# pollen-robotics/reachy2_symbolic_ik

Hardware: AMD Instinct MI355X
Metric: IK solves/sec (7-DoF r_arm, batched poses) (higher is better)
Workload: dtype f64

## Files before the change

### reachy2_symbolic_ik_amd/csrc/rsik_device.hpp

```cpp
#pragma once

#include <hip/hip_runtime.h>
#include <stdint.h>

#include "../../include/rsik.h"
#include "rsik_math.hpp"

namespace rsik {

#ifdef RSIK_HOT_ONLY
#define RSIK_RARE(c) (false)
#else
#define RSIK_RARE(c) (__builtin_expect(!!(c), 0))
#endif


#ifdef RSIK_ISA_MARKS
#define RSIK_MARK(name) asm volatile("; RSIK_MARK " name)
#else
#define RSIK_MARK(name)
#endif

constexpr double kPi = 3.141592653589793;
constexpr double kTwoPi = 2 * kPi;

struct ArmC {
    double v[RSIK_ARM_CONSTS_COUNT];
};

struct V3 {
    double x, y, z;
};
__device__ __forceinline__ V3 operator+(V3 a, V3 b) { return {a.x + b.x, a.y + b.y, a.z + b.z}; }
__device__ __forceinline__ V3 operator-(V3 a, V3 b) { return {a.x - b.x, a.y - b.y, a.z - b.z}; }
__device__ __forceinline__ V3 operator*(V3 a, double s) { return {a.x * s, a.y * s, a.z * s}; }
__device__ __forceinline__ double dot(V3 a, V3 b) { return fma(a.x, b.x, fma(a.y, b.y, a.z * b.z)); }
__device__ __forceinline__ V3 cross(V3 a, V3 b) {
    return {fma(a.y, b.z, -(a.z * b.y)), fma(a.z, b.x, -(a.x * b.z)), fma(a.x, b.y, -(a.y * b.x))};
}
__device__ __forceinline__ V3 madd(V3 a, double s, V3 b) { return {fma(a.x, s, b.x), fma(a.y, s, b.y), fma(a.z, s, b.z)}; }
__device__ __forceinline__ double dot_d(V3 a, V3 b) { return a.x * b.x + a.y * b.y + a.z * b.z; }
__device__ __forceinline__ double norm(V3 a) { return sqrt_cr(dot_d(a, a)); }
__device__ __forceinline__ V3 normalized(V3 a, double& len) {
    double rs;
    sqrt_rsqrt(dot(a, a), len, rs);
    return a * rs;
}
__device__ __forceinline__ V3 normalized(V3 a) {
    return a * rsqrt_fast(dot(a, a));
}

__device__ __forceinline__ bool np_isclose(double a, double b) { return fabs(a - b) <= (1e-8 + 1e-5 * fabs(b)); }
template <int N>
__device__ __forceinline__ bool all_finite(const double (&v)[N]) {
    bool ok = true;
#pragma unroll
    for (int k = 0; k < N; k++) ok = ok && (fabs(v[k]) < __builtin_inf());
    return ok;
}

__device__ __forceinline__ double pymod_2pi(double a) {
    double q = floor(a * 0.15915494309189535);
    double m = fma(-q, kTwoPi, a);
    if (RSIK_RARE(!(m >= 0 && m < kTwoPi))) {
        if (m < 0) m += kTwoPi;
        if (m >= kTwoPi) m -= kTwoPi;
    }
    return m;
// ... 180 lines not shown
    return g;
}
template <class Acc>
__device__ __forceinline__ Goal goal_from_euler_tipz(const Acc& A, double roll, double pitch, double yaw) {
    const double ang[3] = {roll, pitch, yaw};
    double sn[3], cs[3];
    fast_sincos_n<3>(ang, sn, cs);
    const double sa = sn[0], ca = cs[0], sb = sn[1], cb = cs[1], sc = sn[2], cc = cs[2];
    const double tz = A(RSIK_C_TIPL + 2);
    Goal g;
    g.woff = {fma(cc * sb, ca, sc * sa) * tz, fma(sc * sb, ca, -(cc * sa)) * tz, (cb * ca) * tz};
    g.toff = {0.0, 0.0, 0.0};
    g.xg = {cc * cb, sc * cb, -sb};
    g.tw = {-g.woff.x, -g.woff.y, -g.woff.z};
    return g;
}
__device__ __forceinline__ V3 wrist_position(const V3& woff, V3 pos) { return woff + pos; }

template <bool V>
struct BoolC {
    __device__ __forceinline__ constexpr operator bool() const { return V; }
};
template <bool KEEP, bool GEOM_ONLY, class NL, class Acc>
__device__ Reach reach_impl(const Acc& A, V3 pos_in, const V3 woff, const NL no_limits_v) {
    const bool NO_LIMITS = no_limits_v;
    Reach r;
    r.ok = false;
    r.i0 = r.i1 = __builtin_nan("");
    const V3 s = cvec(A, RSIK_C_SHOULDER);
    const double u = A(RSIK_C_UPPER_ARM), f = A(RSIK_C_FOREARM);
    const double bl = A(RSIK_C_BACKWARD), pm = A(RSIK_C_PROJ_MARGIN), upf = A(RSIK_C_UPF);

    V3 gp = pos_in;
    V3 dv = gp - s;
    const double ss0 = dot_d(dv, dv);
    int st = RSIK_STATE_REACHABLE;
    if (RSIK_RARE(ss0 > A(RSIK_C_MAX_LEN_SQ))) {
        double nd = sqrt_cr(ss0) + pm;
        gp = madd(dv * fast_rcp(nd), A(RSIK_C_MAX_LEN), s);
        st = RSIK_STATE_POSE_OUT_OF_REACH;
    }
    if (RSIK_RARE(gp.x < bl)) {
        gp.x = bl;
        st = RSIK_STATE_BACKWARD_POSE;
    }
    r.state = st;
    r.stage = 0;
    if (KEEP) { r.pos = gp; r.w = gp; r.c2 = gp; r.n2 = gp; r.a1 = gp; r.a2 = gp; r.r2 = 0.0; r.ct0 = 1.0; r.st0 = 0.0; r.ct1 = 1.0; r.st1 = 0.0; }
    if (!NO_LIMITS && st != RSIK_STATE_REACHABLE) return r;
    r.stage = 1;

    RSIK_MARK("reach_wrist");
    V3 w = wrist_position(woff, gp);
    if (RSIK_RARE(w.x < bl)) {
        double diff = bl - w.x;
        gp.x = gp.x + diff;
        if (NO_LIMITS) w = wrist_position(woff, gp);
        else w.x = w.x + diff;
    }
    V3 P = w - s;
    double dsw, inv_d;
    sqrt_rsqrt(dot_d(P, P), dsw, inv_d);
    double d = dsw;
    V3 self_pos = gp;
    if (NO_LIMITS) {
        if (RSIK_RARE(dsw > upf)) {
            double nd = fabs(dsw) + pm;
            V3 nw = madd((w - s) * fast_rcp(nd), upf, s);
            self_pos = gp + (nw - w);
            w = nw;
            P = w - s;
            sqrt_rsqrt(dot_d(P, P), d, inv_d);
        }
    } else {
        if (RSIK_RARE(dsw > upf)) {
            r.state = RSIK_STATE_WRIST_OUT_OF_RANGE;
            if (KEEP) { r.pos = gp; r.w = w; }
            return r;
        }
    }
    if (RSIK_RARE(dsw < A(RSIK_C_MIN_DIST))) {
        const double t = fabs(dsw) + pm;
        const double k = A(RSIK_C_MIN_DIST) * fast_rcp(t);
        const double km1 = k - 1.0;
        gp = madd(P, km1, gp);
        w = madd(P, km1, w);
        self_pos = gp;
        P = P * k;
        d = dsw * k;
        inv_d = inv_d * (t * A(RSIK_C_INV_MIN_DIST));
    }

    RSIK_MARK("reach_circle");
    if (RSIK_RARE(d > upf)) {
        r.state = RSIK_STATE_SHOULD_NOT_HAPPEN;
        if (KEEP) { r.pos = self_pos; r.w = w; }
        return r;
    }
    r.pos = self_pos;
    r.w = w;
    V3 n2 = P * inv_d;
    double r2, ir2;
    double kk;
    double fh;
    V3 c2;
    {
        double d2 = d * d, k = d2 - f * f + u * u;
        double rad = 4 * d2 * (u * u) - k * k;
        const double m = d + P.x;
        const double g = rad * (m * m);
        double irad, srad;
        if (RSIK_RARE(!(g > 0.0))) {
            irad = (rad != 0.0) ? rsqrt_fast(rad) : 0.0;
            srad = rad * irad;
            fh = fast_rcp(1.0 + n2.x);
        } else {
            const double z = rsqrt_fast(g);
            irad = z * m;
            srad = rad * irad;
            fh = d * (z * srad);
        }
        const double hid = 0.5 * inv_d;
        r2 = hid * srad;
        ir2 = (d + d) * irad;
        kk = k * hid;
        c2 = s + n2 * kk;
    }
    RSIK_MARK("reach_frame");
    Frame F2 = frame_from_unit(n2, fh);
    r.c2 = c2; r.r2 = r2; r.n2 = n2; r.a1 = F2.c1; r.a2 = F2.c2;
    r.stage = 2;
    if (NO_LIMITS || GEOM_ONLY) {
        r.ok = true; r.state = RSIK_STATE_REACHABLE; r.i0 = -kPi; r.i1 = kPi;
        r.ct0 = -1.0; r.st0 = -1.2246467991473532e-16;
// ... 130 lines not shown
    const bool inside = fma(r2, fma(cm, fa1, sm * fa2), side_val) > 0;
    const bool first = inside != (ang2 < ang1);
    r.i0 = first ? ang1 : ang2;
    r.i1 = first ? ang2 : ang1;
    r.ct0 = first ? ly1 : ly2;
    r.st0 = first ? lz1 : lz2;
    r.ct1 = first ? ly2 : ly1;
    r.st1 = first ? lz2 : lz1;
    return r;
}

template <bool NO_LIMITS, bool KEEP = true, class Acc>
__device__ __forceinline__ Reach reach_g(const Acc& A, V3 pos_in, const V3 woff) {
    return reach_impl<KEEP, false>(A, pos_in, woff, BoolC<NO_LIMITS>{});
}

template <bool NO_LIMITS, bool KEEP = true, class Acc>
__device__ __forceinline__ Reach reach(const Acc& A, V3 pos_in, const Rot& Rg) {
    return reach_g<NO_LIMITS, KEEP>(A, pos_in, make_goal(A, Rg).woff);
}

__device__ __forceinline__ V3 elbow_on_circle(const Reach& r, double ct, double st) {
    double y = r.r2 * ct, z = r.r2 * st;
    return madd(r.a1, y, madd(r.a2, z, r.c2));
}

template <bool EXACT = true, class Acc>
__device__ __forceinline__ bool above_singularity_plane(const Acc& A, V3 e) {
    if constexpr (EXACT) return e.z > (e.x - A(RSIK_C_ES)) * A(RSIK_C_SING_COEFF) + A(RSIK_C_ES + 2) - A(RSIK_C_SING_OFFSET);
    else return e.z > fma(e.x, A(RSIK_C_SING_COEFF), A(RSIK_C_PLANE_K));
}
template <bool PLANE = true, class Acc>
__device__ __forceinline__ bool is_elbow_ok(const Acc& A, V3 e) {
    bool ok = e.y * A(RSIK_C_SIDE) < -0.2;
    if constexpr (PLANE) ok = ok && (e.z < (e.x - A(RSIK_C_ES)) * A(RSIK_C_SING_COEFF) + A(RSIK_C_ES + 2) - A(RSIK_C_SING_OFFSET));
    return ok;
}

struct JointsOut {
    double j[7];
    V3 elbow;
    bool projected;
    bool sing;
    double c4, s4, c5, s5, c6, s6;
};

typedef const __attribute__((address_space(1))) double* GConst;
template <bool FRESH, bool TIPZ = false, class Acc, class Prev = const double*>
__device__ JointsOut joints_from_theta_g(const Acc& A, Reach& r, const Goal& G, double ct, double st, Prev prev) {
    RSIK_MARK("joints_elbow");
    JointsOut o;
    V3 e = elbow_on_circle(r, ct, st);
    o.projected = false;
    if (RSIK_RARE(above_singularity_plane<!FRESH>(A, e))) {
        const V3 v3 = cvec(A, RSIK_C_PLANE_N), pc = cvec(A, RSIK_C_PROJ_CENTER);
        const V3 d1 = e - pc;
        const V3 V = madd(v3, -dot(d1, v3), d1);
        const V3 ne = madd(V, A(RSIK_C_PROJ_RADIUS) * rsqrt_fast(dot(V, V)), pc);
        const V3 shift = ne - e;
        e = ne;
        if constexpr (FRESH) {
            r.w = r.w + shift;
        } else {
            r.pos = r.pos + shift;
            r.w = wrist_position(G.woff, r.pos);
        }
        o.projected = true;
    }
    RSIK_MARK("joints_shoulder");
    o.elbow = e;
    const double u = A(RSIK_C_UPPER_ARM), f = A(RSIK_C_FOREARM);
    auto to_shoulder = [&](V3 p) -> V3 {
        return {fma(A(RSIK_C_MST + 0), p.x, fma(A(RSIK_C_MST + 1), p.y, fma(A(RSIK_C_MST + 2), p.z, A(RSIK_C_TSH + 0)))),
                fma(A(RSIK_C_MST + 3), p.x, fma(A(RSIK_C_MST + 4), p.y, fma(A(RSIK_C_MST + 5), p.z, A(RSIK_C_TSH + 1)))),
                fma(A(RSIK_C_MST + 6), p.x, fma(A(RSIK_C_MST + 7), p.y, fma(A(RSIK_C_MST + 8), p.z, A(RSIK_C_TSH + 2))))};
    };
    V3 q = to_shoulder(e);
    double cphi, sphi, rho;
    const bool sing_sp = RSIK_RARE(q.x == 0 && q.z == 0);
    if (sing_sp) {
        double s_, c_;
        fast_sincos(prev[0], &s_, &c_);
        cphi = c_; sphi = -s_; rho = 0.0;
    } else {
        const double rho2 = fma(q.x, q.x, q.z * q.z);
        const double irho = rsqrt_fast(rho2);
        rho = rho2 * irho;
        cphi = q.x * irho; sphi = q.z * irho;
    }
    const double iL = A(RSIK_C_INV_U);
    double cr = rho * iL, srs = q.y * iL;
    V3 g0 = {cr * cphi, srs, cr * sphi};
    V3 g1 = {-srs * cphi, cr, -srs * sphi};
    V3 g2 = {-sphi, 0.0, cphi};
    auto rot_g = [&](V3 a) -> V3 { return {dot(g0, a), dot(g1, a), fma(g2.x, a.x, g2.z * a.z)}; };
    auto to_elbow = [&](V3 p) -> V3 {
        V3 a = rot_g(to_shoulder(p));
        a.x -= u;
        return a;
    };
    RSIK_MARK("joints_elbow_angles");
    V3 pw = to_elbow(r.w);
    double sigma, ca, sa;
    const bool sing_ey = RSIK_RARE(pw.y == 0 && pw.z == 0);
    if (sing_ey) {
        fast_sincos(prev[2], &sa, &ca);
        sigma = 0.0;
// ... 482 lines not shown
```

### reachy2_symbolic_ik_amd/csrc/rsik_kernel_continuous.hpp

```cpp
#pragma once

namespace rsik {

struct ContinuousArgs {
    int64_t n;
    const double* in[12];
    const double* cur_pose[12];
    const uint8_t* arm;
    const uint8_t* timed_out;
    int euler_roundtrip;
    int first_timed_out;
    double pref_arg[2];
    double pref_self[2];
    double pref_self_cs[2], pref_self_sn[2];
    double lim[2][2];
    double d_theta_max;
    const double* current_joints;
    double max_angle, cos_max, sin_max;
    double* st;
    double* joints;
    uint8_t* reachable;
    uint8_t* state;
    unsigned* started_word;
    unsigned started_seq;
// ... 21 lines not shown
    return disc;
}

struct ThetaTarget {
    bool ok_limits;
    bool found;
    double theta;
    int code;
};
template <bool PLANE, bool FALLBACK_GEOMETRY = true, class Acc>
__device__ __forceinline__ ThetaTarget continuous_target(const Acc& A, V3 pos, const V3 woff, double pref_self, double pref_cs,
                                                         double pref_sn, Reach& r) {
    ThetaTarget T;
    r = reach_g<false, false>(A, pos, woff);
    T.ok_limits = r.ok;
    T.found = false;
    T.theta = 0.0;
    T.code = RSIK_STATE_EMPTY;
    if (r.ok) {
        T.found = best_discrete_theta_lane<PLANE>(A, r, 10, pref_self, pref_cs, pref_sn, T.theta);
        if (!T.found) T.code = RSIK_STATE_LIMITED_BY_SHOULDER;
    } else {
        T.code = r.state;
        if constexpr (FALLBACK_GEOMETRY) r = reach_g<true>(A, pos, woff);
    }
    return T;
}
__device__ __forceinline__ double continuous_next_theta_goal(double goal, double prev_theta, double d_theta_max, double l0,
                                                            double l1, double dmax_v, double l1v) {
    const double ad = angle_diff_straight(goal, prev_theta);
    const double theta = (fabs(ad) < d_theta_max) ? goal : (prev_theta + copysign(dmax_v, ad));
    return limit_theta_to_interval_straight(theta, l0, l1, l1v);
}
__device__ __forceinline__ double continuous_next_theta_goal(double goal, double prev_theta, double d_theta_max, double l0,
                                                            double l1) {
    return continuous_next_theta_goal(goal, prev_theta, d_theta_max, l0, l1, d_theta_max, l1);
}
__device__ __forceinline__ double continuous_next_theta(bool ok_limits, bool found, double target, double pref_arg,
                                                        double prev_theta, double d_theta_max, double l0, double l1) {
    const double goal = ok_limits ? (found ? target : prev_theta) : pref_arg;
    return continuous_next_theta_goal(goal, prev_theta, d_theta_max, l0, l1);
}
template <bool MIXED, bool PLANE>
__global__ __launch_bounds__(kBlock) void control_continuous_kernel(const ContinuousArgs K) {
    __shared__ double lds_out[kBlock / 64][64 * 7];
    const int lane = threadIdx.x & 63;
    const int wave = threadIdx.x >> 6;
    const int64_t i = (int64_t)blockIdx.x * kBlock + threadIdx.x;
    const int64_t wave_base = (int64_t)blockIdx.x * kBlock + wave * 64;
    const bool live = i < K.n;
    const int64_t ii = live ? i : (K.n - 1);
    const int64_t n = K.n;

    __shared__ SharedTables lds_tab;
        stage_tables<MIXED, (int)offsetof(ContinuousArgs, arms) + (MIXED ? 0 : (int)sizeof(ArmC))>(lds_tab, K.arms);
    const Acc<MIXED> A = make_acc<MIXED>(K.arms, MIXED ? (K.arm[ii] != 0) : false, lds_tab);
    const int slot = MIXED ? (A.isl ? 1 : 0) : 0;

    double prev_theta = K.st[0 * n + ii];
    double prev_sol[7];
#pragma unroll
    for (int k = 0; k < 7; k++) prev_sol[k] = K.st[(1 + k) * n + ii];
    bool init = K.st[8 * n + ii] != 0.0;
    bool emergency = K.st[9 * n + ii] != 0.0;
    bool has_prev = K.st[10 * n + ii] != 0.0;

    double jv[7], rejected[7];
    int st_code = RSIK_STATE_EMPTY;
    int cause = 0;
    bool ok = false;
    if (emergency) {
#pragma unroll
        for (int k = 0; k < 7; k++) jv[k] = prev_sol[k];
        st_code = RSIK_STATE_EMERGENCY;
    } else {
        Rot Rg;
        V3 pos;
        double m[12];
#pragma unroll
        for (int k = 0; k < 12; k++) m[k] = K.in[k][ii];
        const bool invalid = !all_finite(m);
        goal_from_m12(m, Rg, pos, K.euler_roundtrip);
        if (K.first_timed_out || (K.timed_out && K.timed_out[ii])) { has_prev = false; init = true; }
        if (!has_prev) {
            has_prev = true;
            continuous_reinit(A, K, ii, K.pref_arg[slot], prev_theta, prev_sol);
        }
        const Goal G = make_goal(A, Rg);
        Reach r;
        const ThetaTarget T = continuous_target<PLANE>(A, pos, G.woff, K.pref_self[slot], K.pref_self_cs[slot], K.pref_self_sn[slot], r);
        if (RSIK_RARE(invalid)) {
#pragma unroll
            for (int k = 0; k < 7; k++) jv[k] = __builtin_nan("");
            st_code = RSIK_STATE_INVALID_INPUT;
            prev_theta = continuous_next_theta(true, false, 0.0, K.pref_arg[slot], prev_theta, K.d_theta_max, K.lim[slot][0], K.lim[slot][1]);
        } else if (RSIK_RARE(!T.ok_limits && !r.ok)) {
#pragma unroll
            for (int k = 0; k < 7; k++) jv[k] = __builtin_nan("");
            st_code = RSIK_STATE_NOT_REACHABLE_NO_LIMITS;
        } else {
        ok = T.ok_limits && T.found;
        st_code = T.code;
        const double theta = continuous_next_theta(T.ok_limits, T.found, T.theta, K.pref_arg[slot], prev_theta, K.d_theta_max,
                                                   K.lim[slot][0], K.lim[slot][1]);
        prev_theta = theta;
        double sn, cs;
        fast_sincos(theta, &sn, &cs);
        JointsOut o = joints_from_theta_g<true>(A, r, G, cs, sn, prev_sol);
#pragma unroll
        for (int k = 0; k < 7; k++) jv[k] = o.j[k];
        cause = safety_checks(A.utab, jv, o.c4, o.s4, o.c5, o.s5, o.c6, o.s6, prev_sol, K.max_angle, K.cos_max, K.sin_max);
        emergency = cause != 0;
        if (!init && joints_discontinuous(jv, prev_sol)) {
            cause |= RSIK_EMERGENCY_CONTINUITY;
            emergency = true;
#pragma unroll
            for (int k = 0; k < 7; k++) { rejected[k] = jv[k]; jv[k] = prev_sol[k]; }
        }
        init = false;
        if (!emergency) {
#pragma unroll
            for (int k = 0; k < 7; k++) prev_sol[k] = jv[k];
        }
        }
    }
    store_rows<7>(K.joints, wave_base, K.n, lane, lds_out[wave], jv);
    if (live) {
        if (K.reachable) K.reachable[i] = ok ? 1 : 0;
        if (K.state) K.state[i] = (uint8_t)st_code;
        K.st[0 * n + i] = prev_theta;
#pragma unroll
        for (int k = 0; k < 7; k++) K.st[(1 + k) * n + i] = prev_sol[k];
        K.st[8 * n + i] = init ? 1.0 : 0.0;
        K.st[9 * n + i] = emergency ? 1.0 : 0.0;
        K.st[10 * n + i] = has_prev ? 1.0 : 0.0;
        if (cause != 0) {
            K.st[11 * n + i] = (double)cause;
            if (cause & RSIK_EMERGENCY_CONTINUITY) {
#pragma unroll
                for (int k = 0; k < 7; k++) K.st[(12 + k) * n + i] = rejected[k];
            }
        }
    }
}

template <bool MIXED, bool PAIR>
__global__ __launch_bounds__(kBlock) void cont_init_kernel(const ContinuousArgs K) {
    __builtin_amdgcn_s_setprio(3);
    if (K.started_word != nullptr && blockIdx.x == gridDim.x - 1 && threadIdx.x == 0)
        __hip_atomic_store(K.started_word, K.started_seq, __ATOMIC_RELAXED, __HIP_MEMORY_SCOPE_SYSTEM);
    const int64_t gid = (int64_t)blockIdx.x * kBlock + threadIdx.x;
    const int64_t i = PAIR ? (gid >> 1) : gid;
    const int half = PAIR ? (int)(gid & 1) : 0;
    const bool live = i < K.n;
    const int64_t ii = live ? i : (K.n - 1);
    __shared__ SharedTables lds_tab;
        stage_tables<MIXED, (int)offsetof(ContinuousArgs, arms) + (MIXED ? 0 : (int)sizeof(ArmC))>(lds_tab, K.arms);
    const Acc<MIXED> A = make_acc<MIXED>(K.arms, MIXED ? (K.arm[ii] != 0) : false, lds_tab);
    const int slot = MIXED ? (A.isl ? 1 : 0) : 0;
    const int64_t n = K.n;
    if (!live || K.st[9 * n + i] != 0.0) return;
    const bool timed_out = K.first_timed_out || (K.timed_out && K.timed_out[i]);
    if (!timed_out && K.st[10 * n + i] != 0.0) return;
    double prev_theta = K.st[0 * n + i];
    double prev_sol[7];
#pragma unroll
    for (int k = 0; k < 7; k++) prev_sol[k] = K.st[(1 + k) * n + i];
    continuous_reinit<PAIR>(A, K, i, K.pref_arg[slot], prev_theta, prev_sol, half);
    if (half != 0) return;
    K.st[0 * n + i] = prev_theta;
#pragma unroll
    for (int k = 0; k < 7; k++) K.st[(1 + k) * n + i] = prev_sol[k];
    K.st[8 * n + i] = 1.0;
    K.st[10 * n + i] = 1.0;
}

}
```

### reachy2_symbolic_ik_amd/csrc/rsik_kernel_discrete.hpp

```cpp
#pragma once

namespace rsik {

struct DiscreteArgs {
    int64_t n;
    const double* in[12];
    const uint8_t* arm;
    int nb;
    int log2p;
    int sweep_mode;
    int euler_roundtrip;
    int stagger;
    double pref[2];
    double pref_cs[2], pref_sn[2];
    double lim[2][2];
    union {
        double prev_sol[2][7];
        const double* prev_rows;
    };
    double prev_cs[2][3], prev_sn[2][3];
    const double* current_joints;
    double max_angle, cos_max, sin_max;
    double* joints;
    uint8_t* reachable;
// ... 64 lines not shown
            double od = __shfl_xor(best_d, off);
            int ok = __shfl_xor(best_k, off);
            if (od < best_d || (od == best_d && ok < best_k)) { best_d = od; best_k = ok; }
        }
        if (p >= 0 && k0 == 0) {
            double th = __builtin_nan("");
            if (best_k != 0x7fffffff) th = (best_k == K.nb - 1) ? gb : ((double)best_k * gstep + ga);
            res[p] = th;
        }
    }
}

#ifndef RSIK_DISC_ATTR
#define RSIK_DISC_ATTR
#endif
#ifndef RSIK_DISC_MIN_WAVES
#define RSIK_DISC_MIN_WAVES 3
#endif
#define RSIK_DISC_PRIO(p) do { if (K.stagger) __builtin_amdgcn_s_setprio(p); } while (0)
#ifndef RSIK_DISC_BLOCK
#define RSIK_DISC_BLOCK 256
#endif
constexpr int kDiscBlock = RSIK_DISC_BLOCK;
struct PrevRowRegs { double v[7]; };
struct NoPrevRow {};
__device__ __forceinline__ const double* safety_prev(const PrevRowRegs& p, const double*) { return p.v; }
__device__ __forceinline__ const double* safety_prev(const NoPrevRow&, const double* uniform) { return uniform; }
template <bool MIXED, bool PLANE, bool PREV_ROWS = false>
__global__ __launch_bounds__(kDiscBlock, RSIK_DISC_MIN_WAVES) RSIK_DISC_ATTR void control_discrete_kernel(const DiscreteArgs K) {
    __shared__ double lds_slab[kDiscBlock / 64][kDiscRows][64];
    const int lane = threadIdx.x & 63;
    const int wave = threadIdx.x >> 6;
    const int64_t i = (int64_t)blockIdx.x * kDiscBlock + threadIdx.x;
    const int64_t wave_base = (int64_t)blockIdx.x * kDiscBlock + wave * 64;
    const bool live = i < K.n;
    const int64_t ii = live ? i : (K.n - 1);

#ifdef RSIK_TIMELINE_PROBE
    uint64_t probe_t[7];
    probe_t[0] = __builtin_amdgcn_s_memrealtime();
#define RSIK_DISC_PROBE(k) do { __builtin_amdgcn_sched_barrier(0); probe_t[k] = __builtin_amdgcn_s_memrealtime(); __builtin_amdgcn_sched_barrier(0); } while (0)
#else
#define RSIK_DISC_PROBE(k) do { } while (0)
#endif
    double m12[12];
#pragma unroll
    for (int k = 0; k < 12; k++) m12[k] = K.in[k][ii];
    const bool lane_isl = MIXED ? (K.arm[ii] != 0) : false;
    [[maybe_unused]] std::conditional_t<PREV_ROWS, PrevRowRegs, NoPrevRow> prow;
    if constexpr (PREV_ROWS) {
#pragma unroll
        for (int k = 0; k < 7; k++) prow.v[k] = K.prev_rows[ii * 7 + k];
    }
        __shared__ SharedTables lds_tab;
    stage_tables<MIXED, (int)offsetof(DiscreteArgs, arms) + (MIXED ? 0 : (int)sizeof(ArmC)), kDiscBlock>(lds_tab, K.arms);
#ifdef RSIK_TIMELINE_PROBE
    asm volatile("s_waitcnt vmcnt(0)" ::: "memory");
#endif
    RSIK_DISC_PROBE(1);
    const Acc<MIXED> A = make_acc<MIXED>(K.arms, lane_isl, lds_tab);
    const int slot = MIXED ? (A.isl ? 1 : 0) : 0;

    const bool invalid = !all_finite(m12);
    Rot Rg;
    V3 pos;
    goal_from_m12(m12, Rg, pos, K.euler_roundtrip);

    Goal G = make_goal(A, Rg);
    {
        const double pk[6] = {G.tw.x, G.tw.y, G.tw.z, G.xg.x, G.xg.y, G.xg.z};
#pragma unroll
        for (int k = 0; k < 6; k++) lds_slab[wave][k][lane] = pk[k];
    }
    RSIK_MARK("disc_reach");
    RSIK_DISC_PRIO(3);
    Reach r = reach_g<false, false>(A, pos, G.woff);
    if (RSIK_RARE(invalid)) { r.ok = false; r.state = RSIK_STATE_INVALID_INPUT; }
    RSIK_MARK("disc_shortcut");
    const double pref = K.pref[slot];
    bool found = false;
    double theta = 0.0;
    bool need = false;
    bool pref_valid = false;
    if (r.ok) {
        pref_valid = is_valid_angle(pref, r.i0, r.i1);
        if (pref_valid) {
            const double st = K.pref_sn[slot], ct = K.pref_cs[slot];
            if (is_elbow_ok<PLANE>(A, elbow_on_circle(r, ct, st))) { found = true; theta = pref; }
        }
        need = !found;
    }
    double ca = 1.0, sa = 0.0, cb = 1.0, sb = 0.0;
    bool pref_free = need && !pref_valid && fabs(pref) > kPi;
    if (need) {
        double a, b;
        if (fabs(fabs(r.i0) + fabs(r.i1) - kTwoPi) < 0.00001) {
            a = kPi / 2; b = kPi / 2 + kTwoPi;
            ca = 6.123233995736766e-17; sa = 1.0; cb = 3.061616997868383e-16; sb = 1.0;
            pref_free = pref_free || !pref_valid;
        } else {
            a = r.i0; b = (r.i0 < r.i1) ? r.i1 : r.i1 + kTwoPi;
            ca = r.ct0; sa = r.st0; cb = r.ct1; sb = r.st1;
        }
        double (*g)[64] = &lds_slab[wave][kGeoRow0];
        g[0][lane] = r.c2.x; g[1][lane] = r.c2.y; g[2][lane] = r.c2.z;
        g[3][lane] = r.r2 * r.a1.x; g[4][lane] = r.r2 * r.a1.y; g[5][lane] = r.r2 * r.a1.z;
        g[6][lane] = r.r2 * r.a2.x; g[7][lane] = r.r2 * r.a2.y; g[8][lane] = r.r2 * r.a2.z;
// ... 131 lines not shown
```

### reachy2_symbolic_ik_amd/csrc/rsik_kernel_nearest.hpp

```cpp
#pragma once

namespace rsik {

struct NearestArgs {
    int64_t n;
    const double* in[6];
    const uint8_t* arm;
    int theta_policy;
    int n_theta;
    int theta_per_pose;
    int skip_projected;
    const double* theta_in;
    union {
        double prev[7];
        const double* prev_rows;
    };
    const double* seed;
    double weights[7];
    int32_t* index;
    double* theta;
    double* joints;
    double* elbow;
    double* cost;
    uint8_t* projected;
    double* interval;
    uint8_t* reachable;
    uint8_t* state;
    ArmC arms[2];
};

template <int MIXED>
struct AccNearest : AccK<MIXED> {};

constexpr int kNoSample = 0x7fffffff;

__device__ __forceinline__ bool nearer(double c, int k, double bc, int bk) { return c < bc || (c == bc && k < bk); }

template <int L>
__device__ __forceinline__ void nearest_of_group(double& c, int& k) {
#pragma unroll
    for (int off = L / 2; off >= 1; off >>= 1) {
        const double oc = __shfl_xor(c, off, 64);
        const int ok = __shfl_xor(k, off, 64);
        if (nearer(oc, ok, c, k)) { c = oc; k = ok; }
    }
}

template <int W, int PW>
__device__ __forceinline__ void flush_pose_rows(double* __restrict__ out, int64_t wave_base, int nrows, int lane,
                                                const double* __restrict__ lds_rows) {
    __builtin_amdgcn_s_waitcnt(0xC07F);
    __builtin_amdgcn_wave_barrier();
    const int total = nrows * W;
    double* dst = out + wave_base * W;
#pragma unroll
    for (int k = 0; k < W; k++) {
        if (k * 64 < PW * W) {
            const int idx = k * 64 + lane;
            if (idx < total) st_stream(dst + idx, lds_rows[idx]);
        }
    }
    __builtin_amdgcn_wave_barrier();
}

#ifndef RSIK_NEAREST_MIN_WAVES
#define RSIK_NEAREST_MIN_WAVES 1
#endif
template <int MIXED, bool TIPZ, bool PREV_ROWS, int L>
__global__ __launch_bounds__(kBlock, RSIK_NEAREST_MIN_WAVES) void solve_nearest_kernel(const NearestArgs K) {
    static_assert(L == 1 || L == 8 || L == 64, "lanes per pose");
    constexpr int PW = 64 / L;
    constexpr int PB = kBlock / L;
    __shared__ SharedTables lds_tab;
    __shared__ double lds[kBlock / 64][64 * 10];
    const int lane = threadIdx.x & 63;
    const int wave = __builtin_amdgcn_readfirstlane(threadIdx.x >> 6);
    const int64_t tile0 = (int64_t)blockIdx.x * PB;
    const int64_t left = K.n - tile0;
    const unsigned rows = left < PB ? (unsigned)left : (unsigned)PB;
    const unsigned sub = (unsigned)lane & (L - 1);
    const unsigned pw = (unsigned)lane / L;
    const unsigned t = (unsigned)wave * PW + pw;
    const unsigned tt = (t < rows ? t : rows - 1) & (PB - 1);
    const bool lead = sub == 0;
    const bool live = t < rows && lead;

    double in[6];
#pragma unroll
    for (int k = 0; k < 6; k++) in[k] = ld_stream(K.in[k] + tile0 + tt);
    warm_and_stage_tables<MIXED>(K, lds_tab);
    const AccNearest<MIXED> A = kernarg_acc<AccNearest<MIXED>, NearestArgs>(lds_tab, (MIXED != 0 && K.arm[tile0 + tt] != 0) ? 1 : 0);
    double* lds_wave = lds[wave];

    const bool invalid = !all_finite(in);
    const V3 pos = {in[0], in[1], in[2]};
    Goal G;
    if constexpr (TIPZ) {
        G = goal_from_euler_tipz(A, in[3], in[4], in[5]);
    } else {
        const Rot Rg = rot_from_euler(in[3], in[4], in[5]);
        G = make_goal(A, Rg);
    }
    Reach r = reach_g<false, false>(A, pos, G.woff);
    if (RSIK_RARE(invalid)) reach_invalid_input(r);
    store_reach(K, live, tile0, t, r);
    if (rows <= (unsigned)(wave * PW)) return;

    const int wave_rows = rows - wave * PW < PW ? (int)(rows - wave * PW) : PW;
    const int64_t wave_base = tile0 + wave * PW;
    {
        const double* src = K.seed + wave_base * 7;
#pragma unroll
        for (int k = 0; k < 7; k++) {
            if (k * 64 < PW * 7) {
                const int idx = k * 64 + lane;
                if (idx < wave_rows * 7) lds_wave[idx] = ld_stream(src + idx);
            }
        }
        __builtin_amdgcn_s_waitcnt(0xC07F);
        __builtin_amdgcn_wave_barrier();
    }
    const double* seed = lds_wave + (tt - wave * PW) * 7;
    double* jrow = lds_wave + pw * 7;
    double* erow = lds_wave + 64 * 7 + pw * 3;

    const bool want_elbow = K.elbow != nullptr;
// ... 77 lines not shown
```

### reachy2_symbolic_ik_amd/csrc/rsik_kernel_pipeline.hpp

```cpp
#pragma once

namespace rsik {

#ifndef RSIK_THETA_BATCH
#define RSIK_THETA_BATCH 16
#endif
#ifndef RSIK_CHAIN_BATCH
#define RSIK_CHAIN_BATCH 16
#endif
constexpr int kThetaBatch = RSIK_THETA_BATCH, kChainBatch = RSIK_CHAIN_BATCH;
#ifdef RSIK_PHASED_OCC
#define RSIK_PHASED_OCC_ATTR __attribute__((amdgpu_waves_per_eu(RSIK_PHASED_OCC, RSIK_PHASED_OCC)))
#else
#define RSIK_PHASED_OCC_ATTR
#endif
#ifndef RSIK_JOINT_CHUNK
#define RSIK_JOINT_CHUNK 8
#endif
constexpr int kJointChunk = RSIK_JOINT_CHUNK;

#ifndef RSIK_THETA_BLOCK
#define RSIK_THETA_BLOCK 64
#endif
constexpr int kThetaBlock = RSIK_THETA_BLOCK;
// ... 48 lines not shown
    unsigned* run_turn_hint;
    uint8_t* slot_turn_hint;
    int first_block, last_block;
    unsigned* started_word;
    unsigned started_seq;
    const unsigned* wait_word;
    unsigned wait_seq;
    unsigned* timeout_word;
    unsigned* chain_started_word;
    double* st;
    double* joints;
    uint8_t* reachable;
    uint8_t* state;
    ArmC arms[2];
};
#define RSIK_WS(K, t, i) (K).ws[(int64_t)(t) * (K).n + (i)]
constexpr int kRowStoreAux = 17;
template <class T>
__device__ __forceinline__ void pipe_store(T* p, T v) { st_stream<kStoreThrough>(p, v); }

template <bool MIXED, bool PLANE>
__device__ __forceinline__ void cont_prepare_step(const ContRunArgs& K, const Acc<MIXED>& A, int slot, const double (&m)[12], int64_t t,
                                                  int64_t t_abs, int64_t i, bool live) {
    const bool invalid = !all_finite(m);
    Rot Rg;
    V3 pos;
    bool special;
    goal_from_m12(m, Rg, pos, K.euler_roundtrip, &special);
    const Goal G = make_goal(A, Rg);
    Reach r;
    ThetaTarget T = continuous_target<PLANE, false>(A, pos, G.woff, K.pref_self[slot], K.pref_self_cs[slot], K.pref_self_sn[slot], r);
    if (!live) return;
    if (RSIK_RARE(invalid)) { T.ok_limits = true; T.found = false; T.code = RSIK_STATE_INVALID_INPUT; }
    const double goal = T.ok_limits ? (T.found ? T.theta : __builtin_nan("")) : K.pref_arg[slot];
    pipe_store(&RSIK_WS(K, t, i), goal);
    pipe_store(&K.gw[t * K.n + i], wrap_theta_to_pi(goal));
    pipe_store(&K.flags[t * K.n + i], (uint8_t)((T.ok_limits ? 1 : 0) | (T.found ? 2 : 0) | (special ? 8 : 0) | (invalid ? 16 : 0)));
    if (K.state) pipe_store(&K.state[t_abs * K.n + i], (uint8_t)T.code);
    if (K.reachable) pipe_store(&K.reachable[t_abs * K.n + i], (uint8_t)((T.ok_limits && T.found) ? 1 : 0));
}

template <bool MIXED, bool PLANE>
__global__ __launch_bounds__(kBlock) RSIK_PHASED_OCC_ATTR void cont_prepare_kernel(const ContRunArgs K) {
    RSIK_PIPE_STAMP(K, 0);
    const int64_t i = (int64_t)blockIdx.x * kBlock + threadIdx.x;
    const int64_t t = blockIdx.y;
    const bool live = i < K.n;
    const int64_t ii = live ? i : (K.n - 1);
    double m[12];
    const double* src = K.m12_steps + (K.t0 + t) * 12 * K.n + ii;
#pragma unroll
    for (int k = 0; k < 12; k++) m[k] = src[k * K.n];
    const bool lane_isl = MIXED ? (K.arm[ii] != 0) : false;
    __shared__ SharedTables lds_tab;
        stage_tables<MIXED, (int)offsetof(ContRunArgs, arms) + (MIXED ? 0 : (int)sizeof(ArmC))>(lds_tab, K.arms);
    const Acc<MIXED> A = make_acc<MIXED>(K.arms, lane_isl, lds_tab);
    const int slot = MIXED ? (A.isl ? 1 : 0) : 0;
    cont_prepare_step<MIXED, PLANE>(K, A, slot, m, t, K.t0 + t, i, live);
}

typedef unsigned RowWords2 __attribute__((ext_vector_type(2)));
__device__ __forceinline__ __amdgpu_buffer_rsrc_t row_buffer(const void* base) {
    return __builtin_amdgcn_make_buffer_rsrc(const_cast<void*>(base), 0, 0x7fffffff, 0x00020000);
}
__device__ __forceinline__ double ld_row_f64(__amdgpu_buffer_rsrc_t buf, unsigned lane, unsigned row) {
    return __builtin_bit_cast(double, __builtin_amdgcn_raw_buffer_load_b64(buf, lane, row, 0));
}
__device__ __forceinline__ void st_row_f64(__amdgpu_buffer_rsrc_t buf, unsigned lane, unsigned row, double v) {
    __builtin_amdgcn_raw_buffer_store_b64(__builtin_bit_cast(RowWords2, v), buf, lane, row, kRowStoreAux);
}
__device__ __forceinline__ int ld_row_u8(__amdgpu_buffer_rsrc_t buf, unsigned lane, unsigned row) {
    return (int)__builtin_amdgcn_raw_buffer_load_b8(buf, lane, row, 0);
}

template <int KIND, int BATCH>
__device__ __forceinline__ double cont_theta_walk(const ContRunArgs& K, int64_t i, double l0, double l1, double* ws, double* gw, int64_t T,
                                                  bool first_generic, double prev_theta, double* scratch) {
    const int64_t n = K.n;
    const __amdgpu_buffer_rsrc_t wbuf = row_buffer(ws), gbuf = row_buffer(gw);
    const unsigned off = (unsigned)(i * sizeof(double)), stride = (unsigned)(n * sizeof(double));
    unsigned row = 0;
    const double dmax_v = opaque(K.d_theta_max), l0v = opaque(l0), l1v = opaque(l1), tdag_v = opaque(K.snap_tdag);
    auto generic = [&](double g) {
        return continuous_next_theta_goal((g != g) ? prev_theta : g, prev_theta, K.d_theta_max, l0, l1, dmax_v, l1v);
    };
    auto one = [&](double g, double gw_) {
        if constexpr (KIND == kSnapGeneric) prev_theta = generic(g);
        else prev_theta = continuous_next_theta_lean<KIND>(g, gw_, prev_theta, dmax_v, l0v, l1v, tdag_v);
        return prev_theta;
    };
    int64_t left = T;
    if (KIND != kSnapGeneric && first_generic && left > 0) {
        prev_theta = generic(ld_row_f64(wbuf, off, row));
        st_row_f64(wbuf, off, row, prev_theta);
        row += stride; left -= 1;
    }
    struct Operands { double g[BATCH], gw[BATCH]; };
    auto fetch = [&](Operands& o, int ahead, int valid) {
#pragma unroll
        for (int u = 0; u < BATCH; u++) {
            const unsigned at = row + (unsigned)(ahead + (u < valid ? u : valid - 1)) * stride;
            o.g[u] = ld_row_f64(wbuf, off, at);
            if constexpr (KIND != kSnapGeneric) o.gw[u] = ld_row_f64(gbuf, off, at);
        }
    };
    auto compute = [&](const Operands& o, auto partial, int valid) {
        constexpr bool kPartial = decltype(partial)::value;
// ... 178 lines not shown
            packed = fma(packed, 256.0, 8.0 - r);
        }
        if (k < 4) worst_a = __builtin_fmax(worst_a, fabs(x));
        else worst_b = __builtin_fmax(worst_b, fabs(x));
    }
    const unsigned long long sing_mask = __ballot(dead);
    const bool sing_below = sl > 0 && ((sing_mask >> (lane - 8)) & 1ull) != 0;
    const bool ev = dead || sing_below || !(worst_a <= 0.5 - 1e-9) || !(worst_b <= 1.0 - 1e-9) || !(fabs(packed) < 4.0e9);
    unsigned word = (unsigned)packed;
#pragma unroll
    for (int step = 1; step < 8; step *= 2) {
        const unsigned w = (unsigned)__builtin_amdgcn_ds_bpermute((lane - 8 * step) << 2, (int)word);
        if (sl >= step) word += w;
    }
#pragma unroll
    for (int k = 0; k < 7; k++) turn[k] = 0.0;
    {
        const int bias = 8 * (sl + 1) + 128;
        turn[0] = (double)((int)(word & 0xffu) + (int)(hint & 0xffu) - bias);
        turn[2] = (double)((int)((word >> 8) & 0xffu) + (int)((hint >> 8) & 0xffu) - bias);
        turn[4] = (double)((int)((word >> 16) & 0xffu) + (int)((hint >> 16) & 0xffu) - bias);
        turn[6] = (double)((int)(word >> 24) + (int)(hint >> 24) - bias);
    }
    double out[7];
#pragma unroll
    for (int k = 0; k < 7; k++) out[k] = (k == 0 || k == 2 || k == 4 || k == 6) ? fma(turn[k], kTwoPi, jv[k]) : jv[k];
    if (RSIK_RARE(sing_mask != 0)) {
#pragma unroll
        for (int k = 0; k < 7; k++) out[k] = dead ? __builtin_nan("") : out[k];
    }
    if (live && sing) K.flags[t * n + i] = (uint8_t)(flag | 4);
    const unsigned long long evm = __ballot(ev && live);
    if (live && sl == 0) pipe_store(&K.chunk_event[c * n + i], (uint8_t)(((evm >> tl) & 0x0101010101010101ull) != 0 ? 1 : 0));
#pragma unroll
    for (int k = 0; k < 7; k++) lw[lane * 7 + k] = out[k];
    __builtin_amdgcn_s_waitcnt(0xC07F);
    __builtin_amdgcn_wave_barrier();
    const int traj_left = (int)((n - grp * 8) < 8 ? (n - grp * 8) : 8);
    const int steps_left = (int)((K.T - c * kJointChunk) < kJointChunk ? (K.T - c * kJointChunk) : kJointChunk);
    const __amdgpu_buffer_rsrc_t obuf = row_buffer(K.joints + ((K.t0 + c * kJointChunk) * n + grp * 8) * 7);
    const unsigned row_bytes = (unsigned)(n * 7 * sizeof(double));
    if (lane < traj_left * 7) {
#pragma unroll
        for (int s_ = 0; s_ < kJointChunk; s_++)
            if (s_ < steps_left) st_row_f64(obuf, (unsigned)lane * 8u, (unsigned)s_ * row_bytes, lw[s_ * 56 + lane]);
    }
    __builtin_amdgcn_wave_barrier();
}

template <bool MIXED>
__global__ __launch_bounds__(kBlock) RSIK_PHASED_OCC_ATTR void cont_joints_kernel(const ContRunArgs K) {
    RSIK_PIPE_STAMP(K, 2);
    __shared__ double lds_out[kBlock / 64][64 * 7];
    __shared__ SharedTables lds_tab;
    const int wave = threadIdx.x >> 6;
    cont_joints_chunk<MIXED>(K, lds_tab, lds_out[wave], (int64_t)blockIdx.x * (kBlock / 64) + wave, (int64_t)blockIdx.y);
}

template <bool MIXED, int BATCH>
__device__ __forceinline__ void cont_chain_walk(const ContRunArgs& K, SharedTables& lds_tab, int64_t i, int j, int64_t tw0, int64_t t_abs0,
                                                int64_t T, bool last) {
    auto theta_at = [&](int64_t t_ws, int64_t ix) { return RSIK_WS(K, t_ws, ix); };
    const int lane = threadIdx.x & 63;
    const int gshift = lane & ~7;
    const bool live = i < K.n;
    const int64_t ii = live ? i : (K.n - 1);
    const int jj = j < 7 ? j : 6;
    const bool owner = live && j < 7;
    const Acc<MIXED> A = make_acc<MIXED>(K.arms, MIXED ? (K.arm[ii] != 0) : false, lds_tab);
    const int64_t n = K.n;
    const int64_t tm0 = t_abs0 - K.t0;
    double prev = K.st[(1 + jj) * n + ii];
    bool init = K.st[8 * n + ii] != 0.0;
    bool emergency = K.st[9 * n + ii] != 0.0;
    bool filled = false;
    const double thr = jj < 4 ? 0.5 : 1.0;
    const double lim = (jj == 0 || jj == 2 || jj == 6) ? 6 * kPi : __builtin_inf();
    const int hit_bit = jj == 0 ? RSIK_EMERGENCY_SHOULDER_PITCH : (jj == 2 ? RSIK_EMERGENCY_ELBOW_YAW : RSIK_EMERGENCY_WRIST_YAW);
    auto group_or = [](int v) -> int {
        v |= __builtin_amdgcn_update_dpp(0, v, 0xB1, 0xf, 0xf, true);
        v |= __builtin_amdgcn_update_dpp(0, v, 0x4E, 0xf, 0xf, true);
        v |= __builtin_amdgcn_update_dpp(0, v, 0x141, 0xf, 0xf, true);
        return v;
    };
    const __amdgpu_buffer_rsrc_t jbuf = row_buffer(K.joints + t_abs0 * n * 7), fbuf = row_buffer(K.flags + tw0 * n);
    const unsigned joff = (unsigned)((ii * 7 + jj) * sizeof(double)), foff = (unsigned)ii;
    const unsigned jstride = (unsigned)(n * 7 * sizeof(double)), fstride = (unsigned)n;
    int64_t t_abs = t_abs0;
    auto one = [&](double cur, int f, int64_t t, unsigned jrow) {
        const bool inv = (f & 16) != 0;
        if (RSIK_RARE((f & 4) != 0 && !emergency && !inv)) {
            double pv[7];
#pragma unroll
            for (int k = 0; k < 7; k++) pv[k] = __shfl(prev, gshift + k);
            Reach r;
            Goal G;
            double m[12];
            load_step_m12(K, tm0 + t, ii, m);
            step_geometry(A, m, K.euler_roundtrip, (f & 1) == 0, r, G);
            double jv[7];
            bool sing;
            step_joints(A, K, r, G, theta_at(tw0 + t, ii), pv, jv, sing);
            cur = jv[0];
#pragma unroll
            for (int k = 1; k < 7; k++) cur = (jj == k) ? jv[k] : cur;
        }
        const double turned = allow_multiturn_one_straight(cur, prev);
// ... 109 lines not shown
                                          (!limited || fabs(f2) <= clear_of_limit));
            const bool inside = c0 + u < n_chunks;
            const bool stands = !__any(!quiet) && inside;
            const bool taken = stop == BATCH && stands;
            if (stop == BATCH && !stands) stop = u;
            if (taken && !filled) prev = o.last[u] + sh;
            if (RSIK_RARE(taken && turns != 0.0 && !filled) && owner) add_turns(c0 + u, sh);
        }
        return stop;
    };
    {
        Operands oa, ob;
        int64_t c0 = 0;
        if (RSIK_RARE(__any(emergency && !filled))) fill_rest(0);
        fetch(oa, 0);
#pragma unroll 1
        while (c0 < n_chunks) {
            fetch(ob, c0 + BATCH);
            const int stop = walk(oa, c0);
            if (RSIK_RARE(c0 + stop < n_chunks && stop < BATCH)) {
                double sh, last_row;
                if (stands_alone(c0 + stop, sh, last_row)) {
                    if (!filled) prev = last_row + sh;
                    if (RSIK_RARE(sh != 0.0 && !filled) && owner) add_turns(c0 + stop, sh);
                } else {
                    stepwise((c0 + stop) * kJointChunk, chunk_len(c0 + stop));
                    if (RSIK_RARE(__any(emergency && !filled))) fill_rest((c0 + stop + 1) * kJointChunk);
                }
                c0 += stop + 1;
                if (c0 < n_chunks) fetch(oa, c0);
            } else {
                c0 += BATCH;
                oa = ob;
            }
        }
    }
    if (owner) K.st[(1 + j) * n + i] = prev;
    if (owner && (j & 1) == 0)
        K.slot_turn_hint[4 * i + (j >> 1)] = (uint8_t)((int)((fabs(prev) < 600.0 && !K.no_turn_hint) ? rint(prev * 0.15915494309189535) : 0.0) + 128);
    if (live && j == 7) {
        K.st[8 * n + i] = init ? 1.0 : 0.0;
        K.st[9 * n + i] = emergency ? 1.0 : 0.0;
        if (last && !emergency) K.st[0 * n + i] = theta_at(tw0 + T - 1, i);
    }
}

template <bool MIXED>
__global__ __launch_bounds__(kChainBlock) __attribute__((amdgpu_waves_per_eu(1, 1))) void cont_chain_kernel(const ContRunArgs K) {
    RSIK_PIPE_STAMP(K, 3);
    if (K.chain_started_word != nullptr && blockIdx.x == gridDim.x - 1 && threadIdx.x == 0)
        __hip_atomic_store(K.chain_started_word, K.started_seq, __ATOMIC_RELAXED, __HIP_MEMORY_SCOPE_SYSTEM);
    __builtin_amdgcn_s_setprio(2);
    const int64_t gid = (int64_t)blockIdx.x * kChainBlock + threadIdx.x;
    __shared__ SharedTables lds_tab;
        stage_tables<MIXED, (int)offsetof(ContRunArgs, arms) + (MIXED ? 0 : (int)sizeof(ArmC)), kChainBlock>(lds_tab, K.arms);
    cont_chain_walk<MIXED, kChainBatch>(K, lds_tab, gid >> 3, (int)(gid & 7), 0, K.t0, K.T, K.last_block != 0);
}

}
```

### reachy2_symbolic_ik_amd/csrc/rsik_kernel_solve.hpp

```cpp
#pragma once

namespace rsik {

#ifndef RSIK_BLOCK
#define RSIK_BLOCK 256
#endif
constexpr int kBlock = RSIK_BLOCK;

struct SolveArgs {
    int64_t n;
    const double* in[6];
    const uint8_t* arm;
    int theta_policy;
    const double* theta_in;
    union {
        double prev[7];
        const double* prev_rows;
    };
    double* joints;
    double* interval;
    double* elbow;
    uint8_t* reachable;
    uint8_t* state;
    ArmC arms[2];
};

typedef const __attribute__((address_space(3))) double* LdsConst;
template <bool MIXED>
struct Acc {
    const ArmC* a;
    bool isl;
    LdsConst lds;
    UnitAtanTab utab;
    __device__ __forceinline__ double operator()(int i) const {
        if constexpr (MIXED) return lds[i];
        else return a[0].v[i];
    }
};
typedef const __attribute__((address_space(4))) double* KConst;
__host__ __device__ constexpr bool arm_const_is_sided(int i) {
    return i == RSIK_C_SHOULDER + 1 || i == RSIK_C_TIPL + 1 || (i >= RSIK_C_MST && i < RSIK_C_TSH + 3) || i == RSIK_C_ES + 1 ||
           i == RSIK_C_SIDE || (i >= RSIK_C_PLANE_P && i < RSIK_C_PROJ_CENTER + 3);
}
template <int MIXED>
struct AccK {
    KConst k;
    LdsConst lds;
    UnitAtanTab utab;
    __device__ __forceinline__ double operator()(int i) const {
        if constexpr (MIXED == 1) return lds[i];
        else if constexpr (MIXED == 2) return arm_const_is_sided(i) ? lds[i] : k[i];
        else return k[i];
    }
};
struct SharedTables {
    double arm[2][RSIK_ARM_CONSTS_COUNT];
    double utab[3][kUnitAtanRows];
};
#ifndef RSIK_WARM_KERNARG
#define RSIK_WARM_KERNARG 1
#endif
template <int BYTES>
__device__ __forceinline__ void warm_kernarg() {
#if RSIK_WARM_KERNARG
    const unsigned long long ka = (unsigned long long)__builtin_amdgcn_kernarg_segment_ptr();
#define RSIK_TOUCH(off) if constexpr (BYTES > (off)) asm volatile("s_load_dword s90, %0, " #off ::"s"(ka) : "s90", "memory")
    RSIK_TOUCH(0x40); RSIK_TOUCH(0x80); RSIK_TOUCH(0xc0); RSIK_TOUCH(0x100); RSIK_TOUCH(0x140); RSIK_TOUCH(0x180);
    RSIK_TOUCH(0x1c0); RSIK_TOUCH(0x200); RSIK_TOUCH(0x240); RSIK_TOUCH(0x280); RSIK_TOUCH(0x2c0); RSIK_TOUCH(0x300);
    RSIK_TOUCH(0x340); RSIK_TOUCH(0x380); RSIK_TOUCH(0x3c0); RSIK_TOUCH(0x400); RSIK_TOUCH(0x440); RSIK_TOUCH(0x480);
    RSIK_TOUCH(0x4c0); RSIK_TOUCH(0x500); RSIK_TOUCH(0x540); RSIK_TOUCH(0x580); RSIK_TOUCH(0x5c0); RSIK_TOUCH(0x600);
#undef RSIK_TOUCH
    asm volatile("s_waitcnt lgkmcnt(0)" ::: "s90", "memory");
#endif
}

template <bool MIXED, int WARM = 0, int NB = kBlock>
__device__ __forceinline__ void stage_tables(SharedTables& S, const ArmC* arms) {
    constexpr int NA = kUnitAtanRows * 3, NS = kSinCosRows * 2, NC = 2 * RSIK_ARM_CONSTS_COUNT;
    constexpr int RA = (NA + NB - 1) / NB, RS = (NS + NB - 1) / NB, RC = (NC + NB - 1) / NB;
    const unsigned t = threadIdx.x & (NB - 1);
    const double* ga = &c_unit_atan_tab[0][0];
    const double* gs = &c_sincos_tab[0][0];
    double va[RA], vs[RS], vc[RC];
#pragma unroll
    for (int r = 0; r < RA; r++) va[r] = ((r + 1) * NB <= NA || t + r * NB < NA) ? ga[t + r * NB] : 0.0;
#pragma unroll
    for (int r = 0; r < RS; r++) vs[r] = ((r + 1) * NB <= NS || t + r * NB < NS) ? gs[t + r * NB] : 0.0;
    if constexpr (MIXED) {
#pragma unroll
        for (int r = 0; r < RC; r++) {
            const unsigned k = t + r * NB;
            vc[r] = ((r + 1) * NB <= NC || k < NC) ? arms[k / RSIK_ARM_CONSTS_COUNT].v[k % RSIK_ARM_CONSTS_COUNT] : 0.0;
        }
    }
    double* la = &S.utab[0][0];
    double* ls = &g_sincos_tab[0][0];
#pragma unroll
    for (int r = 0; r < RA; r++)
        if ((r + 1) * NB <= NA || t + r * NB < NA) la[t + r * NB] = va[r];
#pragma unroll
    for (int r = 0; r < RS; r++)
        if ((r + 1) * NB <= NS || t + r * NB < NS) ls[t + r * NB] = vs[r];
    if constexpr (MIXED) {
        double* lc = &S.arm[0][0];
#pragma unroll
        for (int r = 0; r < RC; r++)
            if ((r + 1) * NB <= NC || t + r * NB < NC) lc[t + r * NB] = vc[r];
    }
    __syncthreads();
}
template <bool MIXED>
__device__ __forceinline__ Acc<MIXED> make_acc(const ArmC* arms, bool isl, SharedTables& S) {
    Acc<MIXED> A{arms, isl, (LdsConst)S.arm[isl ? 1 : 0], (UnitAtanTab)&S.utab[0][0]};
    return A;
}

#ifndef RSIK_NT_STORE
#define RSIK_NT_STORE 1
#endif
#ifndef RSIK_NT_LOAD
#define RSIK_NT_LOAD 0
#endif
typedef double f64x2 __attribute__((ext_vector_type(2)));
constexpr int kStoreStream = 1, kStoreThrough = 2;
template <int POLICY = kStoreStream, class T>
__device__ __forceinline__ void st_stream(T* p, T v) {
#if RSIK_NT_STORE
    if constexpr (POLICY == kStoreThrough && sizeof(T) <= 8) __hip_atomic_store(p, v, __ATOMIC_RELAXED, __HIP_MEMORY_SCOPE_SYSTEM);
    else __builtin_nontemporal_store(v, p);
#else
    *p = v;
#endif
}
template <class T>
__device__ __forceinline__ T ld_stream(const T* p) {
#if RSIK_NT_LOAD
    return __builtin_nontemporal_load(p);
#else
    return *p;
#endif
}

template <int W, int POLICY = kStoreStream>
__device__ __forceinline__ void store_rows(double* __restrict__ out, int64_t wave_base, int64_t n, int lane,
                                           double* __restrict__ lds_wave, const double (&vals)[W]) {
#pragma unroll
    for (int k = 0; k < W; k++) lds_wave[lane * W + k] = vals[k];
    __builtin_amdgcn_s_waitcnt(0xC07F);
    __builtin_amdgcn_wave_barrier();
    int64_t rows = n - wave_base;
    if (rows > 64) rows = 64;
    double* dst = out + wave_base * W;
    if (__builtin_amdgcn_readfirstlane((int)rows) == 64) {
        double v[W];
#pragma unroll
        for (int k = 0; k < W; k++) v[k] = lds_wave[k * 64 + lane];
#pragma unroll
        for (int k = 0; k < W; k++) st_stream<POLICY>(dst + k * 64 + lane, v[k]);
    } else {
        const int64_t total = rows * W;
#pragma unroll
        for (int k = 0; k < W; k++) {
            int idx = k * 64 + lane;
            if (idx < total) st_stream<POLICY>(dst + idx, lds_wave[idx]);
        }
    }
    __builtin_amdgcn_wave_barrier();
}

template <int W>
__device__ __forceinline__ void flush_rows_full(double* __restrict__ out, int64_t wave_base, int lane,
                                                const double* __restrict__ lds_rows) {
    __builtin_amdgcn_s_waitcnt(0xC07F);
    __builtin_amdgcn_wave_barrier();
    double v[W];
#pragma unroll
    for (int k = 0; k < W; k++) v[k] = lds_rows[k * 64 + lane];
    double* dst = out + wave_base * W + lane;
#pragma unroll
    for (int k = 0; k < W; k++) st_stream(dst + k * 64, v[k]);
    __builtin_amdgcn_wave_barrier();
}

template <int W>
__device__ __forceinline__ void flush_rows(double* __restrict__ out, int64_t wave_base, int64_t n, int lane,
                                           const double* __restrict__ lds_rows) {
    __builtin_amdgcn_s_waitcnt(0xC07F);
    __builtin_amdgcn_wave_barrier();
    int64_t rows = n - wave_base;
    if (rows > 64) rows = 64;
    const int64_t total = rows * W;
    double* dst = out + wave_base * W;
#pragma unroll
    for (int k = 0; k < W; k++) {
        int idx = k * 64 + lane;
        if (idx < total) st_stream(dst + idx, lds_rows[idx]);
    }
    __builtin_amdgcn_wave_barrier();
}

__device__ __forceinline__ void branch_stores_stay() { asm volatile("" ::: "memory"); }

#ifndef RSIK_SOLVE_MIN_WAVES
#define RSIK_SOLVE_MIN_WAVES 1
#endif

template <int MIXED, class ARGS>
__device__ __forceinline__ void warm_and_stage_tables(const ARGS& K, SharedTables& S) {
    warm_kernarg<(MIXED == 1 ? 0 : (int)offsetof(ARGS, arms) + (int)sizeof(ArmC))>();
    stage_tables<(MIXED != 0)>(S, K.arms);
}
template <class ACC, class ARGS>
__device__ __forceinline__ ACC kernarg_acc(SharedTables& S, int slot) {
    ACC A;
    A.k = (KConst)&((const __attribute__((address_space(4))) ARGS*)__builtin_amdgcn_kernarg_segment_ptr())->arms[0].v[0];
    A.lds = (LdsConst)S.arm[slot]; A.utab = (UnitAtanTab)&S.utab[0][0];
    return A;
}
__device__ __forceinline__ void reach_invalid_input(Reach& r) {
    r.ok = false; r.state = RSIK_STATE_INVALID_INPUT; r.i0 = r.i1 = __builtin_nan("");
}
template <class ARGS>
__device__ __forceinline__ void store_reach(const ARGS& K, bool live, int64_t tile0, unsigned t, const Reach& r) {
    if (!live) return;
    if (K.interval) {
        const f64x2 iv = {r.i0, r.i1};
        st_stream(reinterpret_cast<f64x2*>(K.interval + 2 * tile0) + t, iv);
    }
    if (K.reachable) st_stream(K.reachable + tile0 + t, (uint8_t)(r.ok ? 1 : 0));
    if (K.state) st_stream(K.state + tile0 + t, (uint8_t)r.state);
}

template <int MIXED, bool TIPZ, bool PREV_ROWS = false>
__global__ __launch_bounds__(kBlock, RSIK_SOLVE_MIN_WAVES) void solve_kernel(const SolveArgs K) {
    __shared__ SharedTables lds_tab;
    __shared__ double lds[kBlock / 64][64 * 10];
    const int lane = threadIdx.x & 63;
    const int wave = __builtin_amdgcn_readfirstlane(threadIdx.x >> 6);
    const int64_t tile0 = (int64_t)blockIdx.x * kBlock;
    const int64_t left = K.n - tile0;
    const unsigned rows = left < kBlock ? (unsigned)left : (unsigned)kBlock;
    const unsigned t = threadIdx.x & (kBlock - 1);
    const unsigned tt = (t < rows ? t : rows - 1) & (kBlock - 1);
    const bool live = t < rows;

#ifdef RSIK_CLOCK_PROBE
    const uint64_t probe_c0 = __builtin_readcyclecounter(), probe_r0 = __builtin_amdgcn_s_memrealtime();
#endif
#ifdef RSIK_TIMELINE_PROBE
    const uint64_t probe_t0 = __builtin_amdgcn_s_memrealtime();
#endif
    double in[6];
#pragma unroll
    for (int k = 0; k < 6; k++) in[k] = ld_stream(K.in[k] + tile0 + tt);
    warm_and_stage_tables<MIXED>(K, lds_tab);
#ifdef RSIK_TIMELINE_PROBE
    const uint64_t probe_t1 = __builtin_amdgcn_s_memrealtime();
    uint64_t probe_mid = 0, probe_goal = 0, probe_reach = 0;
#define RSIK_SOLVE_PROBE(v) do { __builtin_amdgcn_sched_barrier(0); v = __builtin_amdgcn_s_memrealtime(); __builtin_amdgcn_sched_barrier(0); } while (0)
#else
#define RSIK_SOLVE_PROBE(v) do { } while (0)
#endif
    const AccK<MIXED> A = kernarg_acc<AccK<MIXED>, SolveArgs>(lds_tab, (MIXED != 0 && K.arm[tile0 + tt] != 0) ? 1 : 0);
    double* lds_wave = lds[wave];

    const bool invalid = !all_finite(in);
    const V3 pos = {in[0], in[1], in[2]};
    Goal G;
    if constexpr (TIPZ) {
        G = goal_from_euler_tipz(A, in[3], in[4], in[5]);
    } else {
        RSIK_MARK("euler");
        const Rot Rg = rot_from_euler(in[3], in[4], in[5]);
        RSIK_MARK("goal");
        G = make_goal(A, Rg);
    }
    RSIK_MARK("reach_start");
    RSIK_SOLVE_PROBE(probe_goal);
    Reach r = reach_g<false, false>(A, pos, G.woff);
    RSIK_SOLVE_PROBE(probe_reach);
    if (RSIK_RARE(invalid)) reach_invalid_input(r);
    RSIK_MARK("after_reach");

    const bool want_elbow = K.elbow != nullptr;
    if (K.theta_policy != RSIK_THETA_NONE) {
        double* jrow = lds_wave + lane * 7;
        double* erow = lds_wave + 64 * 7 + lane * 3;
        if (r.ok) {
// ... 127 lines not shown
```

### reachy2_symbolic_ik_amd/csrc/rsik_kernel_stages.hpp

```cpp
#pragma once

namespace rsik {

struct StageArgs {
    int64_t n;
    int op;
    const double* in;
    double* out;
    int in_stride, out_stride;
    ArmC arms[2];
};

__device__ __forceinline__ V3 cross_d(V3 a, V3 b) {
    return {a.y * b.z - a.z * b.y, a.z * b.x - a.x * b.z, a.x * b.y - a.y * b.x};
}
__device__ __forceinline__ V3 div_d(V3 a, double s) { return {a.x / s, a.y / s, a.z / s}; }

__device__ inline void rotation_from_vector_ref(V3 vect, double (&R)[9]) {
    const V3 u = div_d(vect, sqrt(dot_d(vect, vect)));
    if (np_isclose(1.0, u.x) && np_isclose(0.0, u.y) && np_isclose(0.0, u.z)) {
        R[0] = 1; R[1] = 0; R[2] = 0; R[3] = 0; R[4] = 1; R[5] = 0; R[6] = 0; R[7] = 0; R[8] = 1;
        return;
    }
    if (np_isclose(1.0, -u.x) && np_isclose(0.0, -u.y) && np_isclose(0.0, -u.z)) {
// ... 98 lines not shown
    const double sq = sqrt(disc);
    const double t1 = (-b + sq) / (2 * a), t2 = (-b - sq) / (2 * a);
    pa = {point.x + t1 * dir.x, point.y + t1 * dir.y, point.z + t1 * dir.z};
    pb = {point.x + t2 * dir.x, point.y + t2 * dir.y, point.z + t2 * dir.z};
    return 2;
}

__device__ inline int circles_linked_ref(double normal_margin, V3 wrist, V3 c2, double r2, V3 n2, V3 c1, double r1, V3 n1, double& i0, double& i1) {
    i0 = i1 = __builtin_nan("");
    const V3 p1 = c1 - wrist, p2 = c2 - wrist;
    double R2[9], R1[9];
    rotation_from_vector_ref(n2, R2);
    rotation_from_vector_ref(n1, R1);
    auto colT = [](const double (&R)[9], int k, V3 a) { return R[k] * a.x + R[3 + k] * a.y + R[6 + k] * a.z; };
    auto lim_x = [&](V3 p) { return colT(R1, 0, p) + (-colT(R1, 0, p1)); };
    const bool side = lim_x(p2) > 0;
    auto whole_or_nothing = [&]() -> int {
        if (!side) return 0;
        i0 = -kPi; i1 = kPi;
        return 2;
    };
    V3 N1 = n1, N2 = n2;
    if (N1.x != 0 || N1.y != 0 || N1.z != 0) N1 = div_d(N1, sqrt(dot_d(N1, N1)));
    if (N2.x != 0 || N2.y != 0 || N2.z != 0) N2 = div_d(N2, sqrt(dot_d(N2, N2)));
    const double mg = normal_margin;
    if ((fabs(N2.x - N1.x) < mg && fabs(N2.y - N1.y) < mg && fabs(N2.z - N1.z) < mg) ||
        (fabs(N2.x + N1.x) < mg && fabs(N2.y + N1.y) < mg && fabs(N2.z + N1.z) < mg))
        return whole_or_nothing();
    V3 q, v;
    if (!nearest_approach_ref(p1, N1, p2, N2, q, v)) return whole_or_nothing();
    V3 pa, pb;
    const int np_ = circle_line_ref(p1, r1, v, q, pa, pb);
    if (np_ == 0) return whole_or_nothing();
    auto angle_of = [&](V3 p) {
        const double y = colT(R2, 1, p) + (-colT(R2, 1, p2)), z = colT(R2, 2, p) + (-colT(R2, 2, p2));
        return atan2(z, y);
    };
    if (np_ == 1) {
        i0 = i1 = angle_of(pa);
        return 2;
    }
    double a1 = angle_of(pa), a2 = angle_of(pb);
    if (a2 < a1) { const double t = a1; a1 = a2; a2 = t; }
    const double at = (a1 + a2) / 2;
    const double ly = cos(at) * r2, lz = sin(at) * r2;
    const V3 tp = {R2[1] * ly + R2[2] * lz + p2.x, R2[4] * ly + R2[5] * lz + p2.y, R2[7] * ly + R2[8] * lz + p2.z};
    if (lim_x(tp) > 0) { i0 = a1; i1 = a2; }
    else { i0 = a2; i1 = a1; }
    return 2;
}

__global__ __launch_bounds__(kBlock) void stage_kernel(const StageArgs K) {
    const int64_t i = (int64_t)blockIdx.x * kBlock + threadIdx.x;
    __shared__ SharedTables lds_tab;
        stage_tables<false, (int)offsetof(StageArgs, arms) + (int)sizeof(ArmC)>(lds_tab, K.arms);
    if (i >= K.n) return;
    const Acc<false> A = make_acc<false>(K.arms, false, lds_tab);
    const double* x = K.in + i * K.in_stride;
    double* o = K.out + i * K.out_stride;
    const V3 s = cvec(A, RSIK_C_SHOULDER);
    const double u = A(RSIK_C_UPPER_ARM), f = A(RSIK_C_FOREARM);
    auto put = [&](int at, V3 a) { o[at] = a.x; o[at + 1] = a.y; o[at + 2] = a.z; };
    switch (K.op) {
    case RSIK_STAGE_POSE_IN_REACH: {
        V3 gp = {x[0], x[1], x[2]};
        const V3 dv = gp - s;
        const double d = sqrt(dot_d(dv, dv));
        int st = RSIK_STATE_EMPTY;
        if (d > A(RSIK_C_MAX_LEN)) {
            const V3 dir = div_d(dv, d + A(RSIK_C_PROJ_MARGIN));
            gp = {s.x + dir.x * A(RSIK_C_MAX_LEN), s.y + dir.y * A(RSIK_C_MAX_LEN), s.z + dir.z * A(RSIK_C_MAX_LEN)};
            st = RSIK_STATE_POSE_OUT_OF_REACH;
        }
        if (gp.x < A(RSIK_C_BACKWARD)) { gp.x = A(RSIK_C_BACKWARD); st = RSIK_STATE_BACKWARD_POSE; }
        o[0] = st == RSIK_STATE_EMPTY ? 1.0 : 0.0;
        put(1, gp);
        o[4] = (double)st;
        break;
    }
    case RSIK_STAGE_WRIST_POSITION: {
        const Rot Rg = rot_from_euler(x[3], x[4], x[5]);
        put(0, wrist_position(make_goal(A, Rg).woff, V3{x[0], x[1], x[2]}));
        break;
    }
    case RSIK_STAGE_LIMITATION_CIRCLE: {
        const V3 w = {x[0], x[1], x[2]};
        const V3 nv = w - V3{x[3], x[4], x[5]};
        const V3 vec = div_d(nv, sqrt(dot_d(nv, nv))) * A(RSIK_C_WRIST_AX);
        put(0, w + vec);
        o[3] = A(RSIK_C_WRIST_R);
        put(4, nv);
        break;
    }
    case RSIK_STAGE_INTERSECTION_CIRCLE: {
        const V3 P = V3{x[0], x[1], x[2]} - s;
        const double d = sqrt(P.x * P.x + P.y * P.y + P.z * P.z);
        if (d > u + f) {
            o[0] = 0.0;
            for (int k = 1; k < 8; k++) o[k] = __builtin_nan("");
            break;
        }
        const V3 dir = div_d(P, d);
        const double kq = d * d - f * f + u * u;
        o[0] = 1.0;
        put(1, s + dir * (kq / (2 * d)));
        o[4] = 1 / (2 * d) * sqrt(4 * (d * d) * (u * u) - kq * kq);
        put(5, dir);
// ... 91 lines not shown
```

### reachy2_symbolic_ik_amd/csrc/rsik_kernel_state.hpp

```cpp
#pragma once

namespace rsik {

struct StateArgs {
    int64_t n;
    const double* in[6];
    const uint8_t* arm;
    int no_limits;
    double* solver_state;
    const double* theta;
    const double* prev;
    double* joints;
    double* interval;
    double* elbow;
    uint8_t* reachable;
    uint8_t* state;
    ArmC arms[2];
};

template <bool MIXED>
__global__ __launch_bounds__(kBlock) void reach_state_kernel(const StateArgs K) {
    const int64_t i = (int64_t)blockIdx.x * kBlock + threadIdx.x;
    __shared__ SharedTables lds_tab;
    stage_tables<MIXED, (int)offsetof(StateArgs, arms) + (MIXED ? 0 : (int)sizeof(ArmC))>(lds_tab, K.arms);
    if (i >= K.n) return;
    const Acc<MIXED> A = make_acc<MIXED>(K.arms, MIXED ? (K.arm[i] != 0) : false, lds_tab);
    V3 pos = {K.in[0][i], K.in[1][i], K.in[2][i]};
    double e0 = K.in[3][i], e1 = K.in[4][i], e2 = K.in[5][i];
    const double in6[6] = {pos.x, pos.y, pos.z, e0, e1, e2};
    const bool invalid = !all_finite(in6);
    Rot Rg = rot_from_euler(e0, e1, e2);
    Reach r = K.no_limits ? reach<true>(A, pos, Rg) : reach<false>(A, pos, Rg);
    if (RSIK_RARE(invalid)) { reach_invalid_input(r); r.stage = 0; }
    double* S = K.solver_state + i * RSIK_SOLVER_STATE_STRIDE;
    if (r.stage >= 1) {
        S[0] = r.pos.x; S[1] = r.pos.y; S[2] = r.pos.z; S[3] = e0; S[4] = e1; S[5] = e2;
        S[6] = r.w.x; S[7] = r.w.y; S[8] = r.w.z;
    }
    if (r.stage >= 2) {
        S[9] = r.c2.x; S[10] = r.c2.y; S[11] = r.c2.z; S[12] = r.r2;
        S[13] = r.n2.x; S[14] = r.n2.y; S[15] = r.n2.z;
    }
    S[20] = r.i0; S[21] = r.i1; S[22] = r.ok ? 1.0 : 0.0; S[23] = (double)r.state;
    if (K.interval) { K.interval[2 * i] = r.i0; K.interval[2 * i + 1] = r.i1; }
    if (K.reachable) K.reachable[i] = r.ok ? 1 : 0;
    if (K.state) K.state[i] = (uint8_t)r.state;
}

__device__ __forceinline__ Reach reach_from_state(const double* S) {
    Reach r;
    r.ok = true; r.state = RSIK_STATE_REACHABLE; r.stage = 2; r.i0 = -kPi; r.i1 = kPi;
    r.pos = {S[0], S[1], S[2]};
    r.w = {S[6], S[7], S[8]};
    r.c2 = {S[9], S[10], S[11]};
    r.r2 = S[12];
    r.n2 = {S[13], S[14], S[15]};
    Frame F = frame_from_unit(normalized(r.n2));
    r.a1 = F.c1; r.a2 = F.c2;
    return r;
}

template <bool MIXED>
__global__ __launch_bounds__(kBlock) void joints_state_kernel(const StateArgs K) {
    const int64_t i = (int64_t)blockIdx.x * kBlock + threadIdx.x;
    __shared__ SharedTables lds_tab;
    stage_tables<MIXED, (int)offsetof(StateArgs, arms) + (MIXED ? 0 : (int)sizeof(ArmC))>(lds_tab, K.arms);
    if (i >= K.n) return;
    const Acc<MIXED> A = make_acc<MIXED>(K.arms, MIXED ? (K.arm[i] != 0) : false, lds_tab);
    double* S = K.solver_state + i * RSIK_SOLVER_STATE_STRIDE;
    Reach r = reach_from_state(S);
    Rot Rg = rot_from_euler(S[3], S[4], S[5]);
    double prev[7];
#pragma unroll
    for (int k = 0; k < 7; k++) prev[k] = K.prev ? K.prev[i * 7 + k] : 0.0;
    double st, ct;
    fast_sincos(K.theta[i], &st, &ct);
    JointsOut o = joints_from_theta<false>(A, r, Rg, ct, st, prev);
    if (K.joints) {
#pragma unroll
        for (int k = 0; k < 7; k++) K.joints[i * 7 + k] = o.j[k];
    }
#pragma unroll
    for (int k = 0; k < 7; k++) S[24 + k] = o.j[k];
    S[0] = r.pos.x; S[1] = r.pos.y; S[2] = r.pos.z;
    S[6] = r.w.x; S[7] = r.w.y; S[8] = r.w.z;
    S[16] = o.elbow.x; S[17] = o.elbow.y; S[18] = o.elbow.z;
    S[19] = o.projected ? 1.0 : 0.0;
    if (K.elbow) { K.elbow[3 * i] = o.elbow.x; K.elbow[3 * i + 1] = o.elbow.y; K.elbow[3 * i + 2] = o.elbow.z; }
}

__global__ __launch_bounds__(kBlock) void elbow_state_kernel(const StateArgs K) {
    const int64_t i = (int64_t)blockIdx.x * kBlock + threadIdx.x;
    stage_sincos_tab();
    __syncthreads();
    if (i >= K.n) return;
    const double* S = K.solver_state + i * RSIK_SOLVER_STATE_STRIDE;
    Reach r = reach_from_state(S);
    double st, ct;
    fast_sincos(K.theta[i], &st, &ct);
    V3 e = elbow_on_circle(r, ct, st);
    K.elbow[3 * i] = e.x; K.elbow[3 * i + 1] = e.y; K.elbow[3 * i + 2] = e.z;
}

struct FkArgs {
    int64_t n;
    const double* joints;
    const uint8_t* arm;
    int goal_kind;
    const double* goal[12];
    double* pos;
    double* rot;
    double* err;
    ArmC arms[2];
};

template <bool MIXED>
__global__ __launch_bounds__(kBlock) void fk_kernel(const FkArgs K) {
    const int64_t i = (int64_t)blockIdx.x * kBlock + threadIdx.x;
    __shared__ SharedTables lds_tab;
    stage_tables<MIXED>(lds_tab, K.arms);
    if (i >= K.n) return;
    const Acc<MIXED> A = make_acc<MIXED>(K.arms, MIXED ? (K.arm[i] != 0) : false, lds_tab);
    double j[7];
#pragma unroll
    for (int k = 0; k < 7; k++) j[k] = K.joints[i * 7 + k];
    const FkOut o = forward_kinematics(A, j);
    if (K.pos) { K.pos[3 * i] = o.pos.x; K.pos[3 * i + 1] = o.pos.y; K.pos[3 * i + 2] = o.pos.z; }
    if (K.rot) {
#pragma unroll
        for (int k = 0; k < 9; k++) K.rot[9 * i + k] = o.R[k];
    }
    if (K.err) {
        V3 gp;
        Rot Rg;
        if (K.goal_kind == RSIK_GOAL_M12) {
#pragma unroll
            for (int k = 0; k < 9; k++) Rg.m[k] = K.goal[k][i];
            gp = {K.goal[9][i], K.goal[10][i], K.goal[11][i]};
        } else {
            gp = {K.goal[0][i], K.goal[1][i], K.goal[2][i]};
            Rg = rot_from_euler(K.goal[3][i], K.goal[4][i], K.goal[5][i]);
        }
        const V3 d = o.pos - gp;
        double fro = 0.0;
#pragma unroll
        for (int k = 0; k < 9; k++) { const double e = o.R[k] - Rg.m[k]; fro = fma(e, e, fro); }
        K.err[2 * i] = sqrt(dot(d, d));
        K.err[2 * i + 1] = sqrt(0.5 * fro);
    }
}

__global__ void debug_math_kernel(int op, int64_t n, const double* a, const double* b, double* o0, double* o1) {
    const int64_t i = (int64_t)blockIdx.x * blockDim.x + threadIdx.x;
    __shared__ double utab[3][kUnitAtanRows];
    stage_sincos_tab();
    stage_unit_atan_tab(utab);
    __syncthreads();
    if (i >= n) return;
    double x = a[i], r0 = 0.0, r1 = 0.0;
    switch (op) {
        case 7: {
            const double ss[1] = {x}, cc[1] = {b[i]};
            double o[1];
            unit_atan2_n<1>((UnitAtanTab)&utab[0][0], ss, cc, o);
            r0 = o[0];
            break;
        }
        case 0: r0 = fast_rcp(x); break;
        case 1: sqrt_rsqrt(x, r0, r1); r1 = sqrt_cr(x); break;
        case 2: r0 = rsqrt_fast(x); break;
        case 3: r0 = fast_atan2(x, b[i]); break;
        case 4: fast_sincos(x, &r0, &r1); break;
        case 5: r0 = pymod_2pi(x); r1 = angle_diff(x, b[i]); break;
        case 6: {
            double c[8];
#pragma unroll
            for (int k = 0; k < 8; k++) c[k] = x + k;
            const double m = b[i];
#pragma unroll 1
            for (int it = 0; it < 2048; ++it) {
#pragma unroll
                for (int k = 0; k < 8; k++) c[k] = fma(c[k], m, x);
            }
            r0 = ((c[0] + c[1]) + (c[2] + c[3])) + ((c[4] + c[5]) + (c[6] + c[7]));
            break;
        }
        default: break;
    }
    o0[i] = r0;
    if (o1) o1[i] = r1;
}

__global__ void clock_monitor_kernel(const double* ticks, int64_t n_waves, double* core_ticks, double* real_ticks) {
    const int64_t w = ((int64_t)blockIdx.x * blockDim.x + threadIdx.x) >> 6;
    if (w >= n_waves) return;
    double want = ticks[0];
    want = want < 0.0 ? 0.0 : (want > 5.0e8 ? 5.0e8 : want);
    const uint64_t dur = (uint64_t)want;
    const uint64_t r0 = __builtin_amdgcn_s_memrealtime(), c0 = __builtin_readcyclecounter();
    uint64_t r = r0;
    for (int guard = 0; guard < 4000000 && r - r0 < dur; ++guard) {
        __builtin_amdgcn_s_sleep(127);
        r = __builtin_amdgcn_s_memrealtime();
    }
    const uint64_t c1 = __builtin_readcyclecounter();
    if ((threadIdx.x & 63) == 0) {
        core_ticks[w] = (double)(c1 - c0);
        real_ticks[w] = (double)(r - r0);
    }
}

}
```

### reachy2_symbolic_ik_amd/csrc/rsik_kernel_sweep.hpp

```cpp
#pragma once

namespace rsik {

struct SweepArgs {
    int64_t n;
    const double* in[6];
    const uint8_t* arm;
    int theta_policy;
    int n_theta;
    int theta_per_pose;
    const double* theta_in;
    union {
        double prev[7];
        const double* prev_rows;
    };
    double* joints;
    double* elbow;
    uint8_t* projected;
    double* theta;
    double* interval;
    uint8_t* reachable;
    uint8_t* state;
    ArmC arms[2];
};

template <int MIXED>
struct AccSweep : AccK<MIXED> {};

#ifndef RSIK_SWEEP_MIN_WAVES
#define RSIK_SWEEP_MIN_WAVES 1
#endif
template <int MIXED, bool TIPZ, bool PREV_ROWS>
__global__ __launch_bounds__(kBlock, RSIK_SWEEP_MIN_WAVES) void solve_sweep_kernel(const SweepArgs K) {
    __shared__ SharedTables lds_tab;
    __shared__ double lds[kBlock / 64][64 * 10];
    const int lane = threadIdx.x & 63;
    const int wave = __builtin_amdgcn_readfirstlane(threadIdx.x >> 6);
    const int64_t tile0 = (int64_t)blockIdx.x * kBlock;
    const int64_t left = K.n - tile0;
    const unsigned rows = left < kBlock ? (unsigned)left : (unsigned)kBlock;
    const unsigned t = threadIdx.x & (kBlock - 1);
    const unsigned tt = (t < rows ? t : rows - 1) & (kBlock - 1);
    const bool live = t < rows;

    double in[6];
#pragma unroll
    for (int k = 0; k < 6; k++) in[k] = ld_stream(K.in[k] + tile0 + tt);
    warm_and_stage_tables<MIXED>(K, lds_tab);
    const AccSweep<MIXED> A = kernarg_acc<AccSweep<MIXED>, SweepArgs>(lds_tab, (MIXED != 0 && K.arm[tile0 + tt] != 0) ? 1 : 0);
    double* lds_wave = lds[wave];

    const bool invalid = !all_finite(in);
    const V3 pos = {in[0], in[1], in[2]};
    Goal G;
    if constexpr (TIPZ) {
        G = goal_from_euler_tipz(A, in[3], in[4], in[5]);
    } else {
        const Rot Rg = rot_from_euler(in[3], in[4], in[5]);
        G = make_goal(A, Rg);
    }
    Reach r = reach_g<false, false>(A, pos, G.woff);
    if (RSIK_RARE(invalid)) reach_invalid_input(r);
    store_reach(K, live, tile0, t, r);
    if (rows <= (unsigned)(wave * 64)) return;

    const bool want_elbow = K.elbow != nullptr;
    const bool full = rows >= (unsigned)(wave * 64 + 64);
    const bool fraction = K.theta_policy != RSIK_THETA_EXPLICIT;
    const bool per_pose = K.theta_per_pose != 0;
    const int64_t wave_base = tile0 + wave * 64;
    double* jrow = lds_wave + lane * 7;
    double* erow = lds_wave + 64 * 7 + lane * 3;
    const double fa = r.i0;
    double fb = r.i1;
    if (fa > fb) fb += kTwoPi;
    const double fspan = fb - fa;
    const V3 wrist = r.w;
    if (!r.ok) {
        const double nan = opaque(__builtin_nan(""));
#pragma unroll
        for (int k = 0; k < 7; k++) jrow[k] = nan;
        erow[0] = nan; erow[1] = nan; erow[2] = nan;
        branch_stores_stay();
    }
    const __attribute__((address_space(4))) double* grid = (const __attribute__((address_space(4))) double*)K.theta_in;
    const double* th_col = K.theta_in + tile0 + tt;
    double* jout = K.joints;
// ... 52 lines not shown
```

### reachy2_symbolic_ik_amd/csrc/rsik_kernel_theta_from_joints.hpp

```cpp
#pragma once

namespace rsik {

struct ThetaSearchOut {
    double theta, low, high, distance;
    double j[7];
    V3 elbow;
    bool projected;
};

template <class Acc>
__device__ __forceinline__ ThetaSearchOut theta_search(const Acc& A, Reach& r, const Goal& G, const double* cur, bool n14, double pref) {
    const double zeros[7] = {0, 0, 0, 0, 0, 0, 0};
    const double tolerance = 0.01;
    ThetaSearchOut S;
    auto eval = [&](double th, bool keep) -> double {
        double st, ct;
        fast_sincos(th, &st, &ct);
        const JointsOut o = joints_from_theta_g<false>(A, r, G, ct, st, zeros);
        double acc = 0.0;
        if (RSIK_RARE(n14)) {
#pragma unroll
            for (int q = 0; q < 2; q++)
#pragma unroll
// ... 3 lines not shown
            for (int k = 0; k < 7; k++) { const double d = angle_diff(o.j[k], cur[k]); acc += d * d; }
        }
        const double dist = sqrt(acc);
        if (keep) {
#pragma unroll
            for (int k = 0; k < 7; k++) S.j[k] = o.j[k];
            S.elbow = o.elbow; S.projected = o.projected; S.distance = dist; S.theta = th;
        }
        return dist;
    };
    double low = -kPi, high = kPi;
    if (A(RSIK_C_SIDE) < 0) { low = 0; high = kTwoPi; }
    S.low = S.high = __builtin_nan("");
    if (eval(pref, true) < tolerance) return S;
    while ((high - low) > tolerance) {
        const double mid1 = low + (high - low) / 3;
        const double mid2 = high - (high - low) / 3;
        const double f1 = eval(mid1, false);
        const double f2 = eval(mid2, false);
        if (f1 < f2) high = mid2; else low = mid1;
    }
    (void)eval((low + high) / 2, true);
    S.low = low; S.high = high;
    return S;
}

struct ThetaFromJointsArgs {
    int64_t n;
    const double* goal[12];
    const uint8_t* arm;
    int euler_roundtrip;
    const double* current_joints;
    int n_current;
    double pref[2];
    double* solver_state;
    double* theta;
    double* joints;
    double* bracket;
    double* distance;
    uint8_t* state;
    ArmC arms[2];
};

template <int MIXED, bool M12>
__global__ __launch_bounds__(kBlock) void theta_from_joints_kernel(const ThetaFromJointsArgs K) {
    __shared__ double lds_out[kBlock / 64][64 * 7];
    const int lane = threadIdx.x & 63;
    const int wave = threadIdx.x >> 6;
    const int64_t i = (int64_t)blockIdx.x * kBlock + threadIdx.x;
    const int64_t wave_base = (int64_t)blockIdx.x * kBlock + wave * 64;
    const bool live = i < K.n;
    const int64_t ii = live ? i : (K.n - 1);

    __shared__ SharedTables lds_tab;
    stage_tables<(MIXED != 0), (MIXED == 1 ? 0 : (int)offsetof(ThetaFromJointsArgs, arms) + (int)sizeof(ArmC))>(lds_tab, K.arms);
    const int slot = (MIXED != 0 && K.arm[ii] != 0) ? 1 : 0;
    const AccK<MIXED> A = kernarg_acc<AccK<MIXED>, ThetaFromJointsArgs>(lds_tab, slot);

    double cur[7];
#pragma unroll
    for (int k = 0; k < 7; k++) cur[k] = K.current_joints[ii * 7 + k];
    Rot Rg;
    V3 pos;
    bool invalid = !all_finite(cur);
    if constexpr (M12) {
        double m[12];
#pragma unroll
        for (int k = 0; k < 12; k++) m[k] = K.goal[k][ii];
        invalid = invalid || !all_finite(m);
        goal_from_m12(m, Rg, pos, K.euler_roundtrip);
    } else {
        double p[6];
#pragma unroll
        for (int k = 0; k < 6; k++) p[k] = K.goal[k][ii];
        invalid = invalid || !all_finite(p);
        pos = {p[0], p[1], p[2]};
        Rg = rot_from_euler(p[3], p[4], p[5]);
    }
    const Goal G = make_goal(A, Rg);
    Reach r = reach_g<true>(A, pos, G.woff);
    ThetaSearchOut S = theta_search(A, r, G, cur, false, K.pref[slot]);
    int code = RSIK_STATE_REACHABLE;
    if (RSIK_RARE(invalid || !r.ok)) {
        code = invalid ? RSIK_STATE_INVALID_INPUT : RSIK_STATE_NOT_REACHABLE_NO_LIMITS;
        const double nan = __builtin_nan("");
        S.theta = S.low = S.high = S.distance = nan;
#pragma unroll
        for (int k = 0; k < 7; k++) S.j[k] = nan;
    }
    if (K.joints) store_rows<7>(K.joints, wave_base, K.n, lane, lds_out[wave], S.j);
    if (live) {
        K.theta[i] = S.theta;
        if (K.bracket) { K.bracket[2 * i] = S.low; K.bracket[2 * i + 1] = S.high; }
        if (K.distance) K.distance[i] = S.distance;
        if (K.state) K.state[i] = (uint8_t)code;
    }
}

template <bool MIXED>
__global__ __launch_bounds__(kBlock) void theta_from_joints_state_kernel(const ThetaFromJointsArgs K) {
    const int64_t i = (int64_t)blockIdx.x * kBlock + threadIdx.x;
    __shared__ SharedTables lds_tab;
    stage_tables<MIXED, (int)offsetof(ThetaFromJointsArgs, arms) + (MIXED ? 0 : (int)sizeof(ArmC))>(lds_tab, K.arms);
    if (i >= K.n) return;
    const Acc<MIXED> A = make_acc<MIXED>(K.arms, MIXED ? (K.arm[i] != 0) : false, lds_tab);
    const int slot = MIXED ? (A.isl ? 1 : 0) : 0;
    double* Sr = K.solver_state + i * RSIK_SOLVER_STATE_STRIDE;
    Reach r = reach_from_state(Sr);
    const Goal G = make_goal(A, rot_from_euler(Sr[3], Sr[4], Sr[5]));
    const bool n14 = K.n_current == 14;
    double cur[14];
#pragma unroll
    for (int k = 0; k < 14; k++) cur[k] = (k < 7 || n14) ? K.current_joints[i * K.n_current + k] : 0.0;
    const ThetaSearchOut S = theta_search(A, r, G, cur, n14, K.pref[slot]);
    K.theta[i] = S.theta;
    if (K.bracket) { K.bracket[2 * i] = S.low; K.bracket[2 * i + 1] = S.high; }
#pragma unroll
    for (int k = 0; k < 7; k++) Sr[24 + k] = S.j[k];
    Sr[0] = r.pos.x; Sr[1] = r.pos.y; Sr[2] = r.pos.z;
    Sr[6] = r.w.x; Sr[7] = r.w.y; Sr[8] = r.w.z;
    Sr[16] = S.elbow.x; Sr[17] = S.elbow.y; Sr[18] = S.elbow.z;
    Sr[19] = S.projected ? 1.0 : 0.0;
}

__device__ __forceinline__ bool tend_to_theta_ref(double previous_theta, double d_theta_max, double goal, double& theta) {
    const double ad = angle_diff(goal, previous_theta);
    if (fabs(ad) < d_theta_max) { theta = goal; return true; }
    const double sign = ad / fabs(ad);
    theta = previous_theta + sign * d_theta_max;
    return false;
}
__global__ __launch_bounds__(kBlock) void stage_limiter_kernel(const StageArgs K) {
    const int64_t i = (int64_t)blockIdx.x * kBlock + threadIdx.x;
    if (i >= K.n) return;
    const double* x = K.in + i * K.in_stride;
    double* o = K.out + i * K.out_stride;
    if (K.op == RSIK_STAGE_TEND_TO_PREFERRED_THETA) {
        double th;
        const bool reached = tend_to_theta_ref(x[0], x[1], x[2], th);
        o[0] = reached ? 1.0 : 0.0; o[1] = th;
    } else {
        double in[19];
        for (int k = 0; k < 19; k++) in[k] = x[k];
        double goal = in[0], th = in[0];
        bool worked = false;
        const int nb = (in[3] >= 0.0 && in[3] <= 1048576.0) ? (int)in[3] : 0;
        const bool found = best_discrete_theta_ref(in[0], in[1], in[2], nb, in[4], in[5], in[6], in[7], V3{in[8], in[9], in[10]},
                                                   V3{in[11], in[12], in[13]}, in[14], V3{in[15], in[16], in[17]}, goal, worked);
        double which = 0.0;
        if (found) which = tend_to_theta_ref(in[0], in[18], goal, th) ? 1.0 : 2.0;
        o[0] = found ? 1.0 : 0.0; o[1] = found ? th : in[0]; o[2] = which; o[3] = worked ? 1.0 : 0.0;
    }
}

}
// ... 1 lines not shown
```

### reachy2_symbolic_ik_amd/csrc/rsik_math.hpp

```cpp
#pragma once

#include <hip/hip_runtime.h>

namespace rsik {

__device__ __forceinline__ double fast_rcp(double d) {
    double r = __builtin_amdgcn_rcp(d);
    double e = fma(-d, r, 1.0);
    double p = fma(e, e, e);
    return fma(r, p, r);
}

__device__ __forceinline__ double sqrt_cr(double x) {
    double y = __builtin_amdgcn_rsq(x);
    double g = x * y, h = 0.5 * y;
    double r = fma(-h, g, 0.5);
    g = fma(g, r, g);
    h = fma(h, r, h);
    double d = fma(-g, g, x);
    g = fma(d, h, g);
    d = fma(-g, g, x);
    g = fma(d, h, g);
    return g;
}
// ... 4 lines not shown
    double r = fma(-h, g, 0.5);
    g = fma(g, r, g);
    h = fma(h, r, h);
    double d = fma(-g, g, x);
    g = fma(d, h, g);
    r = fma(-h, g, 0.5);
    h = fma(h, r, h);
    d = fma(-g, g, x);
    g = fma(d, h, g);
    s = g;
    rs = h + h;
}

__device__ __forceinline__ double rsqrt_fast(double x) {
    double y = __builtin_amdgcn_rsq(x);
    double e = fma(-(x * y), y, 1.0);
    double p = fma(0.375, e, 0.5);
    return fma(y, e * p, y);
}

#include "rsik_poly_gen.hpp"

template <int N>
__device__ __forceinline__ void fast_atan2_n(const double (&y)[N], const double (&x)[N], double (&out)[N]) {
    double a[N], s[N], q[N];
    unsigned oct[N];
#pragma unroll
    for (int i = 0; i < N; i++) {
        const double ax = fabs(x[i]), ay = fabs(y[i]);
        const double mx = fmax(ax, ay), mn = fmin(ax, ay);
        double t = mn * fast_rcp(mx);
        a[i] = (mx == 0.0) ? 0.0 : t;
        s[i] = a[i] * a[i];
        oct[i] = (ay > ax ? 1u : 0u) | (__builtin_signbit(x[i]) ? 2u : 0u) |
                 ((unsigned)(__builtin_bit_cast(unsigned long long, y[i]) >> 32) & 0x80000000u);
    }
    horner_atan_q<N>(q, s);
#pragma unroll
    for (int i = 0; i < N; i++) {
        double r = fma(a[i] * s[i], q[i], a[i]);
        r = (oct[i] & 1u) ? (1.5707963267948966 - r) : r;
        r = (oct[i] & 2u) ? (3.141592653589793 - r) : r;
        unsigned long long bits = __builtin_bit_cast(unsigned long long, r) | ((unsigned long long)(oct[i] & 0x80000000u) << 32);
        out[i] = __builtin_bit_cast(double, bits);
    }
}
__device__ __forceinline__ double fast_atan2(double y, double x) {
    const double yy[1] = {y}, xx[1] = {x};
    double o[1];
    fast_atan2_n<1>(yy, xx, o);
    return o[0];
}

typedef const __attribute__((address_space(3))) double* UnitAtanTab;
__device__ __forceinline__ void stage_unit_atan_tab(double (*lds_tab)[kUnitAtanRows]) {
    for (int k = threadIdx.x; k < kUnitAtanRows * 3; k += blockDim.x) (&lds_tab[0][0])[k] = (&c_unit_atan_tab[0][0])[k];
}
template <int N>
__device__ __forceinline__ void unit_atan2_n(UnitAtanTab T, const double (&s)[N], const double (&c)[N], double (&out)[N]) {
    double x[N], x2[N], p[N], phi[N];
#pragma unroll
    for (int i = 0; i < N; i++) {
        const double ac = fabs(c[i]), as = fabs(s[i]);
        const double mx = fmax(ac, as), mn = fmin(ac, as);
        const unsigned idx = (unsigned)(int)fma(mn, (double)kUnitAtanSteps, 0.5);
        const unsigned cneg = (unsigned)(__builtin_bit_cast(unsigned long long, c[i]) >> 63);
        typedef const __attribute__((address_space(3))) char* LdsBytes;
        const unsigned tb = (unsigned)(size_t)(LdsBytes)T;
        const unsigned addr = ((idx + (unsigned)kUnitAtanHalf * cneg) << 4) + (as > ac ? tb + 8u : tb);
        const LdsBytes Tb = (LdsBytes)(size_t)addr;
        const double ci = *(UnitAtanTab)Tb, si = *(UnitAtanTab)(Tb + kUnitAtanRows * 8);
        phi[i] = *(UnitAtanTab)(Tb + 2 * kUnitAtanRows * 8);
        x[i] = fma(mn, ci, -(mx * si));
        x2[i] = x[i] * x[i];
    }
    horner_asin_p<N>(p, x2);
#pragma unroll
    for (int i = 0; i < N; i++) {
        const double r = phi[i] + fma(x[i] * x2[i], p[i], x[i]);
        out[i] = __builtin_copysign(r, s[i]);
    }
}

__shared__ __attribute__((aligned(512))) double g_sincos_tab[2][kSinCosRows];
__device__ __forceinline__ void stage_sincos_tab() {
    for (int k = threadIdx.x; k < kSinCosRows * 2; k += blockDim.x) (&g_sincos_tab[0][0])[k] = (&c_sincos_tab[0][0])[k];
}
template <int N>
__device__ __forceinline__ void fast_sincos_n(const double (&x)[N], double (&sn)[N], double (&cs)[N]) {
    double r[N], z[N], ps[N], pc[N], ck[N], sk[N];
#pragma unroll
    for (int i = 0; i < N; i++) {
        const double k = __builtin_rint(x[i] * 10.185916357881302);
        const double t = fma(-k, 0.09817477042088285, x[i]);
        r[i] = fma(-k, 3.79818781656637e-12, t);
        const int idx = (int)k & (kSinCosRows - 1);
        ck[i] = g_sincos_tab[0][idx]; sk[i] = g_sincos_tab[1][idx];
        z[i] = r[i] * r[i];
    }
    horner_sin3<N>(ps, z);
    horner_cos4<N>(pc, z);
#pragma unroll
    for (int i = 0; i < N; i++) {
        const double sr = fma(r[i] * z[i], ps[i], r[i]);
        const double cm1 = z[i] * pc[i];
        sn[i] = sk[i] + fma(sk[i], cm1, ck[i] * sr);
        cs[i] = ck[i] + fma(ck[i], cm1, -(sk[i] * sr));
    }
}
__device__ __forceinline__ void fast_sincos(double x, double* sn, double* cs) {
    const double xx[1] = {x};
    double s[1], c[1];
    fast_sincos_n<1>(xx, s, c);
    *sn = s[0];
    *cs = c[0];
}

}
```

### reachy2_symbolic_ik_amd/csrc/rsik_poly_gen.hpp

```cpp
template <int N> __device__ __forceinline__ void horner_atan_q(double (&q)[N], const double (&s)[N]);
template <int N> __device__ __forceinline__ void horner_sin_s(double (&q)[N], const double (&s)[N]);
template <int N> __device__ __forceinline__ void horner_cos_c(double (&q)[N], const double (&s)[N]);
template <> __device__ __forceinline__ void horner_atan_q<1>(double (&q)[1], const double (&s)[1]) {
    asm("s_mov_b32 s94, 0xf1d17f2c\n\ts_mov_b32 s95, 0x3eea7d4f\n\tv_mov_b64 %0, s[94:95]\n\ts_mov_b32 s94, 0x5000addb\n\ts_mov_b32 s95, 0xbf2328ae\n\tv_fma_f64 %0, %0, %1, s[94:95]\n\ts_mov_b32 s94, 0x5c884a6d\n\ts_mov_b32 s95, 0x3f4a5313\n\tv_fma_f64 %0, %0, %1, s[94:95]\n\ts_mov_b32 s94, 0x0a5cad37\n\ts_mov_b32 s95, 0xbf66fa05\n\tv_fma_f64 %0, %0, %1, s[94:95]\n\ts_mov_b32 s94, 0x33ffd1ae\n\ts_mov_b32 s95, 0x3f7cd48e\n\tv_fma_f64 %0, %0, %1, s[94:95]\n\ts_mov_b32 s94, 0xe85b6413\n\ts_mov_b32 s95, 0xbf8c012f\n\tv_fma_f64 %0, %0, %1, s[94:95]\n\ts_mov_b32 s94, 0x0da5054f\n\ts_mov_b32 s95, 0x3f964311\n\tv_fma_f64 %0, %0, %1, s[94:95]\n\ts_mov_b32 s94, 0x6d612131\n\ts_mov_b32 s95, 0xbf9e69dd\n\tv_fma_f64 %0, %0, %1, s[94:95]\n\ts_mov_b32 s94, 0x9c197546\n\ts_mov_b32 s95, 0x3fa2b18b\n\tv_fma_f64 %0, %0, %1, s[94:95]\n\ts_mov_b32 s94, 0xbd7d7b67\n\ts_mov_b32 s95, 0xbfa59180\n\tv_fma_f64 %0, %0, %1, s[94:95]\n\ts_mov_b32 s94, 0x93dd0230\n\ts_mov_b32 s95, 0x3fa82a3c\n\tv_fma_f64 %0, %0, %1, s[94:95]\n\ts_mov_b32 s94, 0x39abd8c9\n\ts_mov_b32 s95, 0xbfaae4da\n\tv_fma_f64 %0, %0, %1, s[94:95]\n\ts_mov_b32 s94, 0x5bcacd55\n\ts_mov_b32 s95, 0x3fae1b7b\n\tv_fma_f64 %0, %0, %1, s[94:95]\n\ts_mov_b32 s94, 0x7e57b3d8\n\ts_mov_b32 s95, 0xbfb110df\n\tv_fma_f64 %0, %0, %1, s[94:95]\n\ts_mov_b32 s94, 0xaf6a0e88\n\ts_mov_b32 s95, 0x3fb3b135\n\tv_fma_f64 %0, %0, %1, s[94:95]\n\ts_mov_b32 s94, 0x099f743e\n\ts_mov_b32 s95, 0xbfb745d1\n\tv_fma_f64 %0, %0, %1, s[94:95]\n\ts_mov_b32 s94, 0x16e724e1\n\ts_mov_b32 s95, 0x3fbc71c7\n\tv_fma_f64 %0, %0, %1, s[94:95]\n\ts_mov_b32 s94, 0x92327bf2\n\ts_mov_b32 s95, 0xbfc24924\n\tv_fma_f64 %0, %0, %1, s[94:95]\n\ts_mov_b32 s94, 0x99993702\n\ts_mov_b32 s95, 0x3fc99999\n\tv_fma_f64 %0, %0, %1, s[94:95]\n\ts_mov_b32 s94, 0x55555500\n\ts_mov_b32 s95, 0xbfd55555\n\tv_fma_f64 %0, %0, %1, s[94:95]"
        : "=&v"(q[0])
        : "v"(s[0])
        : "s94", "s95");
}
template <> __device__ __forceinline__ void horner_atan_q<2>(double (&q)[2], const double (&s)[2]) {
    asm("s_mov_b32 s94, 0xf1d17f2c\n\ts_mov_b32 s95, 0x3eea7d4f\n\tv_mov_b64 %0, s[94:95]\n\ts_mov_b32 s94, 0x5000addb\n\ts_mov_b32 s95, 0xbf2328ae\n\tv_fma_f64 %1, %0, %3, s[94:95]\n\tv_fma_f64 %0, %0, %2, s[94:95]\n\ts_mov_b32 s94, 0x5c884a6d\n\ts_mov_b32 s95, 0x3f4a5313\n\tv_fma_f64 %0, %0, %2, s[94:95]\n\tv_fma_f64 %1, %1, %3, s[94:95]\n\ts_mov_b32 s94, 0x0a5cad37\n\ts_mov_b32 s95, 0xbf66fa05\n\tv_fma_f64 %0, %0, %2, s[94:95]\n\tv_fma_f64 %1, %1, %3, s[94:95]\n\ts_mov_b32 s94, 0x33ffd1ae\n\ts_mov_b32 s95, 0x3f7cd48e\n\tv_fma_f64 %0, %0, %2, s[94:95]\n\tv_fma_f64 %1, %1, %3, s[94:95]\n\ts_mov_b32 s94, 0xe85b6413\n\ts_mov_b32 s95, 0xbf8c012f\n\tv_fma_f64 %0, %0, %2, s[94:95]\n\tv_fma_f64 %1, %1, %3, s[94:95]\n\ts_mov_b32 s94, 0x0da5054f\n\ts_mov_b32 s95, 0x3f964311\n\tv_fma_f64 %0, %0, %2, s[94:95]\n\tv_fma_f64 %1, %1, %3, s[94:95]\n\ts_mov_b32 s94, 0x6d612131\n\ts_mov_b32 s95, 0xbf9e69dd\n\tv_fma_f64 %0, %0, %2, s[94:95]\n\tv_fma_f64 %1, %1, %3, s[94:95]\n\ts_mov_b32 s94, 0x9c197546\n\ts_mov_b32 s95, 0x3fa2b18b\n\tv_fma_f64 %0, %0, %2, s[94:95]\n\tv_fma_f64 %1, %1, %3, s[94:95]\n\ts_mov_b32 s94, 0xbd7d7b67\n\ts_mov_b32 s95, 0xbfa59180\n\tv_fma_f64 %0, %0, %2, s[94:95]\n\tv_fma_f64 %1, %1, %3, s[94:95]\n\ts_mov_b32 s94, 0x93dd0230\n\ts_mov_b32 s95, 0x3fa82a3c\n\tv_fma_f64 %0, %0, %2, s[94:95]\n\tv_fma_f64 %1, %1, %3, s[94:95]\n\ts_mov_b32 s94, 0x39abd8c9\n\ts_mov_b32 s95, 0xbfaae4da\n\tv_fma_f64 %0, %0, %2, s[94:95]\n\tv_fma_f64 %1, %1, %3, s[94:95]\n\ts_mov_b32 s94, 0x5bcacd55\n\ts_mov_b32 s95, 0x3fae1b7b\n\tv_fma_f64 %0, %0, %2, s[94:95]\n\tv_fma_f64 %1, %1, %3, s[94:95]\n\ts_mov_b32 s94, 0x7e57b3d8\n\ts_mov_b32 s95, 0xbfb110df\n\tv_fma_f64 %0, %0, %2, s[94:95]\n\tv_fma_f64 %1, %1, %3, s[94:95]\n\ts_mov_b32 s94, 0xaf6a0e88\n\ts_mov_b32 s95, 0x3fb3b135\n\tv_fma_f64 %0, %0, %2, s[94:95]\n\tv_fma_f64 %1, %1, %3, s[94:95]\n\ts_mov_b32 s94, 0x099f743e\n\ts_mov_b32 s95, 0xbfb745d1\n\tv_fma_f64 %0, %0, %2, s[94:95]\n\tv_fma_f64 %1, %1, %3, s[94:95]\n\ts_mov_b32 s94, 0x16e724e1\n\ts_mov_b32 s95, 0x3fbc71c7\n\tv_fma_f64 %0, %0, %2, s[94:95]\n\tv_fma_f64 %1, %1, %3, s[94:95]\n\ts_mov_b32 s94, 0x92327bf2\n\ts_mov_b32 s95, 0xbfc24924\n\tv_fma_f64 %0, %0, %2, s[94:95]\n\tv_fma_f64 %1, %1, %3, s[94:95]\n\ts_mov_b32 s94, 0x99993702\n\ts_mov_b32 s95, 0x3fc99999\n\tv_fma_f64 %0, %0, %2, s[94:95]\n\tv_fma_f64 %1, %1, %3, s[94:95]\n\ts_mov_b32 s94, 0x55555500\n\ts_mov_b32 s95, 0xbfd55555\n\tv_fma_f64 %0, %0, %2, s[94:95]\n\tv_fma_f64 %1, %1, %3, s[94:95]"
        : "=&v"(q[0]), "=&v"(q[1])
        : "v"(s[0]), "v"(s[1])
        : "s94", "s95");
}
template <> __device__ __forceinline__ void horner_atan_q<3>(double (&q)[3], const double (&s)[3]) {
    asm("s_mov_b32 s94, 0xf1d17f2c\n\ts_mov_b32 s95, 0x3eea7d4f\n\tv_mov_b64 %0, s[94:95]\n\ts_mov_b32 s94, 0x5000addb\n\ts_mov_b32 s95, 0xbf2328ae\n\tv_fma_f64 %2, %0, %5, s[94:95]\n\tv_fma_f64 %1, %0, %4, s[94:95]\n\tv_fma_f64 %0, %0, %3, s[94:95]\n\ts_mov_b32 s94, 0x5c884a6d\n\ts_mov_b32 s95, 0x3f4a5313\n\tv_fma_f64 %0, %0, %3, s[94:95]\n\tv_fma_f64 %1, %1, %4, s[94:95]\n\tv_fma_f64 %2, %2, %5, s[94:95]\n\ts_mov_b32 s94, 0x0a5cad37\n\ts_mov_b32 s95, 0xbf66fa05\n\tv_fma_f64 %0, %0, %3, s[94:95]\n\tv_fma_f64 %1, %1, %4, s[94:95]\n\tv_fma_f64 %2, %2, %5, s[94:95]\n\ts_mov_b32 s94, 0x33ffd1ae\n\ts_mov_b32 s95, 0x3f7cd48e\n\tv_fma_f64 %0, %0, %3, s[94:95]\n\tv_fma_f64 %1, %1, %4, s[94:95]\n\tv_fma_f64 %2, %2, %5, s[94:95]\n\ts_mov_b32 s94, 0xe85b6413\n\ts_mov_b32 s95, 0xbf8c012f\n\tv_fma_f64 %0, %0, %3, s[94:95]\n\tv_fma_f64 %1, %1, %4, s[94:95]\n\tv_fma_f64 %2, %2, %5, s[94:95]\n\ts_mov_b32 s94, 0x0da5054f\n\ts_mov_b32 s95, 0x3f964311\n\tv_fma_f64 %0, %0, %3, s[94:95]\n\tv_fma_f64 %1, %1, %4, s[94:95]\n\tv_fma_f64 %2, %2, %5, s[94:95]\n\ts_mov_b32 s94, 0x6d612131\n\ts_mov_b32 s95, 0xbf9e69dd\n\tv_fma_f64 %0, %0, %3, s[94:95]\n\tv_fma_f64 %1, %1, %4, s[94:95]\n\tv_fma_f64 %2, %2, %5, s[94:95]\n\ts_mov_b32 s94, 0x9c197546\n\ts_mov_b32 s95, 0x3fa2b18b\n\tv_fma_f64 %0, %0, %3, s[94:95]\n\tv_fma_f64 %1, %1, %4, s[94:95]\n\tv_fma_f64 %2, %2, %5, s[94:95]\n\ts_mov_b32 s94, 0xbd7d7b67\n\ts_mov_b32 s95, 0xbfa59180\n\tv_fma_f64 %0, %0, %3, s[94:95]\n\tv_fma_f64 %1, %1, %4, s[94:95]\n\tv_fma_f64 %2, %2, %5, s[94:95]\n\ts_mov_b32 s94, 0x93dd0230\n\ts_mov_b32 s95, 0x3fa82a3c\n\tv_fma_f64 %0, %0, %3, s[94:95]\n\tv_fma_f64 %1, %1, %4, s[94:95]\n\tv_fma_f64 %2, %2, %5, s[94:95]\n\ts_mov_b32 s94, 0x39abd8c9\n\ts_mov_b32 s95, 0xbfaae4da\n\tv_fma_f64 %0, %0, %3, s[94:95]\n\tv_fma_f64 %1, %1, %4, s[94:95]\n\tv_fma_f64 %2, %2, %5, s[94:95]\n\ts_mov_b32 s94, 0x5bcacd55\n\ts_mov_b32 s95, 0x3fae1b7b\n\tv_fma_f64 %0, %0, %3, s[94:95]\n\tv_fma_f64 %1, %1, %4, s[94:95]\n\tv_fma_f64 %2, %2, %5, s[94:95]\n\ts_mov_b32 s94, 0x7e57b3d8\n\ts_mov_b32 s95, 0xbfb110df\n\tv_fma_f64 %0, %0, %3, s[94:95]\n\tv_fma_f64 %1, %1, %4, s[94:95]\n\tv_fma_f64 %2, %2, %5, s[94:95]\n\ts_mov_b32 s94, 0xaf6a0e88\n\ts_mov_b32 s95, 0x3fb3b135\n\tv_fma_f64 %0, %0, %3, s[94:95]\n\tv_fma_f64 %1, %1, %4, s[94:95]\n\tv_fma_f64 %2, %2, %5, s[94:95]\n\ts_mov_b32 s94, 0x099f743e\n\ts_mov_b32 s95, 0xbfb745d1\n\tv_fma_f64 %0, %0, %3, s[94:95]\n\tv_fma_f64 %1, %1, %4, s[94:95]\n\tv_fma_f64 %2, %2, %5, s[94:95]\n\ts_mov_b32 s94, 0x16e724e1\n\ts_mov_b32 s95, 0x3fbc71c7\n\tv_fma_f64 %0, %0, %3, s[94:95]\n\tv_fma_f64 %1, %1, %4, s[94:95]\n\tv_fma_f64 %2, %2, %5, s[94:95]\n\ts_mov_b32 s94, 0x92327bf2\n\ts_mov_b32 s95, 0xbfc24924\n\tv_fma_f64 %0, %0, %3, s[94:95]\n\tv_fma_f64 %1, %1, %4, s[94:95]\n\tv_fma_f64 %2, %2, %5, s[94:95]\n\ts_mov_b32 s94, 0x99993702\n\ts_mov_b32 s95, 0x3fc99999\n\tv_fma_f64 %0, %0, %3, s[94:95]\n\tv_fma_f64 %1, %1, %4, s[94:95]\n\tv_fma_f64 %2, %2, %5, s[94:95]\n\ts_mov_b32 s94, 0x55555500\n\ts_mov_b32 s95, 0xbfd55555\n\tv_fma_f64 %0, %0, %3, s[94:95]\n\tv_fma_f64 %1, %1, %4, s[94:95]\n\tv_fma_f64 %2, %2, %5, s[94:95]"
        : "=&v"(q[0]), "=&v"(q[1]), "=&v"(q[2])
        : "v"(s[0]), "v"(s[1]), "v"(s[2])
        : "s94", "s95");
}
template <> __device__ __forceinline__ void horner_atan_q<4>(double (&q)[4], const double (&s)[4]) {
    asm("s_mov_b32 s94, 0xf1d17f2c\n\ts_mov_b32 s95, 0x3eea7d4f\n\tv_mov_b64 %0, s[94:95]\n\ts_mov_b32 s94, 0x5000addb\n\ts_mov_b32 s95, 0xbf2328ae\n\tv_fma_f64 %3, %0, %7, s[94:95]\n\tv_fma_f64 %2, %0, %6, s[94:95]\n\tv_fma_f64 %1, %0, %5, s[94:95]\n\tv_fma_f64 %0, %0, %4, s[94:95]\n\ts_mov_b32 s94, 0x5c884a6d\n\ts_mov_b32 s95, 0x3f4a5313\n\tv_fma_f64 %0, %0, %4, s[94:95]\n\tv_fma_f64 %1, %1, %5, s[94:95]\n\tv_fma_f64 %2, %2, %6, s[94:95]\n\tv_fma_f64 %3, %3, %7, s[94:95]\n\ts_mov_b32 s94, 0x0a5cad37\n\ts_mov_b32 s95, 0xbf66fa05\n\tv_fma_f64 %0, %0, %4, s[94:95]\n\tv_fma_f64 %1, %1, %5, s[94:95]\n\tv_fma_f64 %2, %2, %6, s[94:95]\n\tv_fma_f64 %3, %3, %7, s[94:95]\n\ts_mov_b32 s94, 0x33ffd1ae\n\ts_mov_b32 s95, 0x3f7cd48e\n\tv_fma_f64 %0, %0, %4, s[94:95]\n\tv_fma_f64 %1, %1, %5, s[94:95]\n\tv_fma_f64 %2, %2, %6, s[94:95]\n\tv_fma_f64 %3, %3, %7, s[94:95]\n\ts_mov_b32 s94, 0xe85b6413\n\ts_mov_b32 s95, 0xbf8c012f\n\tv_fma_f64 %0, %0, %4, s[94:95]\n\tv_fma_f64 %1, %1, %5, s[94:95]\n\tv_fma_f64 %2, %2, %6, s[94:95]\n\tv_fma_f64 %3, %3, %7, s[94:95]\n\ts_mov_b32 s94, 0x0da5054f\n\ts_mov_b32 s95, 0x3f964311\n\tv_fma_f64 %0, %0, %4, s[94:95]\n\tv_fma_f64 %1, %1, %5, s[94:95]\n\tv_fma_f64 %2, %2, %6, s[94:95]\n\tv_fma_f64 %3, %3, %7, s[94:95]\n\ts_mov_b32 s94, 0x6d612131\n\ts_mov_b32 s95, 0xbf9e69dd\n\tv_fma_f64 %0, %0, %4, s[94:95]\n\tv_fma_f64 %1, %1, %5, s[94:95]\n\tv_fma_f64 %2, %2, %6, s[94:95]\n\tv_fma_f64 %3, %3, %7, s[94:95]\n\ts_mov_b32 s94, 0x9c197546\n\ts_mov_b32 s95, 0x3fa2b18b\n\tv_fma_f64 %0, %0, %4, s[94:95]\n\tv_fma_f64 %1, %1, %5, s[94:95]\n\tv_fma_f64 %2, %2, %6, s[94:95]\n\tv_fma_f64 %3, %3, %7, s[94:95]\n\ts_mov_b32 s94, 0xbd7d7b67\n\ts_mov_b32 s95, 0xbfa59180\n\tv_fma_f64 %0, %0, %4, s[94:95]\n\tv_fma_f64 %1, %1, %5, s[94:95]\n\tv_fma_f64 %2, %2, %6, s[94:95]\n\tv_fma_f64 %3, %3, %7, s[94:95]\n\ts_mov_b32 s94, 0x93dd0230\n\ts_mov_b32 s95, 0x3fa82a3c\n\tv_fma_f64 %0, %0, %4, s[94:95]\n\tv_fma_f64 %1, %1, %5, s[94:95]\n\tv_fma_f64 %2, %2, %6, s[94:95]\n\tv_fma_f64 %3, %3, %7, s[94:95]\n\ts_mov_b32 s94, 0x39abd8c9\n\ts_mov_b32 s95, 0xbfaae4da\n\tv_fma_f64 %0, %0, %4, s[94:95]\n\tv_fma_f64 %1, %1, %5, s[94:95]\n\tv_fma_f64 %2, %2, %6, s[94:95]\n\tv_fma_f64 %3, %3, %7, s[94:95]\n\ts_mov_b32 s94, 0x5bcacd55\n\ts_mov_b32 s95, 0x3fae1b7b\n\tv_fma_f64 %0, %0, %4, s[94:95]\n\tv_fma_f64 %1, %1, %5, s[94:95]\n\tv_fma_f64 %2, %2, %6, s[94:95]\n\tv_fma_f64 %3, %3, %7, s[94:95]\n\ts_mov_b32 s94, 0x7e57b3d8\n\ts_mov_b32 s95, 0xbfb110df\n\tv_fma_f64 %0, %0, %4, s[94:95]\n\tv_fma_f64 %1, %1, %5, s[94:95]\n\tv_fma_f64 %2, %2, %6, s[94:95]\n\tv_fma_f64 %3, %3, %7, s[94:95]\n\ts_mov_b32 s94, 0xaf6a0e88\n\ts_mov_b32 s95, 0x3fb3b135\n\tv_fma_f64 %0, %0, %4, s[94:95]\n\tv_fma_f64 %1, %1, %5, s[94:95]\n\tv_fma_f64 %2, %2, %6, s[94:95]\n\tv_fma_f64 %3, %3, %7, s[94:95]\n\ts_mov_b32 s94, 0x099f743e\n\ts_mov_b32 s95, 0xbfb745d1\n\tv_fma_f64 %0, %0, %4, s[94:95]\n\tv_fma_f64 %1, %1, %5, s[94:95]\n\tv_fma_f64 %2, %2, %6, s[94:95]\n\tv_fma_f64 %3, %3, %7, s[94:95]\n\ts_mov_b32 s94, 0x16e724e1\n\ts_mov_b32 s95, 0x3fbc71c7\n\tv_fma_f64 %0, %0, %4, s[94:95]\n\tv_fma_f64 %1, %1, %5, s[94:95]\n\tv_fma_f64 %2, %2, %6, s[94:95]\n\tv_fma_f64 %3, %3, %7, s[94:95]\n\ts_mov_b32 s94, 0x92327bf2\n\ts_mov_b32 s95, 0xbfc24924\n\tv_fma_f64 %0, %0, %4, s[94:95]\n\tv_fma_f64 %1, %1, %5, s[94:95]\n\tv_fma_f64 %2, %2, %6, s[94:95]\n\tv_fma_f64 %3, %3, %7, s[94:95]\n\ts_mov_b32 s94, 0x99993702\n\ts_mov_b32 s95, 0x3fc99999\n\tv_fma_f64 %0, %0, %4, s[94:95]\n\tv_fma_f64 %1, %1, %5, s[94:95]\n\tv_fma_f64 %2, %2, %6, s[94:95]\n\tv_fma_f64 %3, %3, %7, s[94:95]\n\ts_mov_b32 s94, 0x55555500\n\ts_mov_b32 s95, 0xbfd55555\n\tv_fma_f64 %0, %0, %4, s[94:95]\n\tv_fma_f64 %1, %1, %5, s[94:95]\n\tv_fma_f64 %2, %2, %6, s[94:95]\n\tv_fma_f64 %3, %3, %7, s[94:95]"
        : "=&v"(q[0]), "=&v"(q[1]), "=&v"(q[2]), "=&v"(q[3])
        : "v"(s[0]), "v"(s[1]), "v"(s[2]), "v"(s[3])
// ... 15 lines not shown
    asm("s_mov_b32 s94, 0x9f8b1451\n\ts_mov_b32 s95, 0x3de5e0b1\n\tv_mov_b64 %0, s[94:95]\n\ts_mov_b32 s94, 0xb02b6262\n\ts_mov_b32 s95, 0xbe5ae600\n\tv_fma_f64 %1, %0, %3, s[94:95]\n\tv_fma_f64 %0, %0, %2, s[94:95]\n\ts_mov_b32 s94, 0x7968a100\n\ts_mov_b32 s95, 0x3ec71de3\n\tv_fma_f64 %0, %0, %2, s[94:95]\n\tv_fma_f64 %1, %1, %3, s[94:95]\n\ts_mov_b32 s94, 0x19e83aae\n\ts_mov_b32 s95, 0xbf2a01a0\n\tv_fma_f64 %0, %0, %2, s[94:95]\n\tv_fma_f64 %1, %1, %3, s[94:95]\n\ts_mov_b32 s94, 0x11110bb2\n\ts_mov_b32 s95, 0x3f811111\n\tv_fma_f64 %0, %0, %2, s[94:95]\n\tv_fma_f64 %1, %1, %3, s[94:95]\n\ts_mov_b32 s94, 0x55555555\n\ts_mov_b32 s95, 0xbfc55555\n\tv_fma_f64 %0, %0, %2, s[94:95]\n\tv_fma_f64 %1, %1, %3, s[94:95]"
        : "=&v"(q[0]), "=&v"(q[1])
        : "v"(s[0]), "v"(s[1])
        : "s94", "s95");
}
template <> __device__ __forceinline__ void horner_sin_s<3>(double (&q)[3], const double (&s)[3]) {
    asm("s_mov_b32 s94, 0x9f8b1451\n\ts_mov_b32 s95, 0x3de5e0b1\n\tv_mov_b64 %0, s[94:95]\n\ts_mov_b32 s94, 0xb02b6262\n\ts_mov_b32 s95, 0xbe5ae600\n\tv_fma_f64 %2, %0, %5, s[94:95]\n\tv_fma_f64 %1, %0, %4, s[94:95]\n\tv_fma_f64 %0, %0, %3, s[94:95]\n\ts_mov_b32 s94, 0x7968a100\n\ts_mov_b32 s95, 0x3ec71de3\n\tv_fma_f64 %0, %0, %3, s[94:95]\n\tv_fma_f64 %1, %1, %4, s[94:95]\n\tv_fma_f64 %2, %2, %5, s[94:95]\n\ts_mov_b32 s94, 0x19e83aae\n\ts_mov_b32 s95, 0xbf2a01a0\n\tv_fma_f64 %0, %0, %3, s[94:95]\n\tv_fma_f64 %1, %1, %4, s[94:95]\n\tv_fma_f64 %2, %2, %5, s[94:95]\n\ts_mov_b32 s94, 0x11110bb2\n\ts_mov_b32 s95, 0x3f811111\n\tv_fma_f64 %0, %0, %3, s[94:95]\n\tv_fma_f64 %1, %1, %4, s[94:95]\n\tv_fma_f64 %2, %2, %5, s[94:95]\n\ts_mov_b32 s94, 0x55555555\n\ts_mov_b32 s95, 0xbfc55555\n\tv_fma_f64 %0, %0, %3, s[94:95]\n\tv_fma_f64 %1, %1, %4, s[94:95]\n\tv_fma_f64 %2, %2, %5, s[94:95]"
        : "=&v"(q[0]), "=&v"(q[1]), "=&v"(q[2])
        : "v"(s[0]), "v"(s[1]), "v"(s[2])
        : "s94", "s95");
}
template <> __device__ __forceinline__ void horner_sin_s<4>(double (&q)[4], const double (&s)[4]) {
    asm("s_mov_b32 s94, 0x9f8b1451\n\ts_mov_b32 s95, 0x3de5e0b1\n\tv_mov_b64 %0, s[94:95]\n\ts_mov_b32 s94, 0xb02b6262\n\ts_mov_b32 s95, 0xbe5ae600\n\tv_fma_f64 %3, %0, %7, s[94:95]\n\tv_fma_f64 %2, %0, %6, s[94:95]\n\tv_fma_f64 %1, %0, %5, s[94:95]\n\tv_fma_f64 %0, %0, %4, s[94:95]\n\ts_mov_b32 s94, 0x7968a100\n\ts_mov_b32 s95, 0x3ec71de3\n\tv_fma_f64 %0, %0, %4, s[94:95]\n\tv_fma_f64 %1, %1, %5, s[94:95]\n\tv_fma_f64 %2, %2, %6, s[94:95]\n\tv_fma_f64 %3, %3, %7, s[94:95]\n\ts_mov_b32 s94, 0x19e83aae\n\ts_mov_b32 s95, 0xbf2a01a0\n\tv_fma_f64 %0, %0, %4, s[94:95]\n\tv_fma_f64 %1, %1, %5, s[94:95]\n\tv_fma_f64 %2, %2, %6, s[94:95]\n\tv_fma_f64 %3, %3, %7, s[94:95]\n\ts_mov_b32 s94, 0x11110bb2\n\ts_mov_b32 s95, 0x3f811111\n\tv_fma_f64 %0, %0, %4, s[94:95]\n\tv_fma_f64 %1, %1, %5, s[94:95]\n\tv_fma_f64 %2, %2, %6, s[94:95]\n\tv_fma_f64 %3, %3, %7, s[94:95]\n\ts_mov_b32 s94, 0x55555555\n\ts_mov_b32 s95, 0xbfc55555\n\tv_fma_f64 %0, %0, %4, s[94:95]\n\tv_fma_f64 %1, %1, %5, s[94:95]\n\tv_fma_f64 %2, %2, %6, s[94:95]\n\tv_fma_f64 %3, %3, %7, s[94:95]"
        : "=&v"(q[0]), "=&v"(q[1]), "=&v"(q[2]), "=&v"(q[3])
        : "v"(s[0]), "v"(s[1]), "v"(s[2]), "v"(s[3])
        : "s94", "s95");
}
template <> __device__ __forceinline__ void horner_sin_s<7>(double (&q)[7], const double (&s)[7]) {
    asm("s_mov_b32 s94, 0x9f8b1451\n\ts_mov_b32 s95, 0x3de5e0b1\n\tv_mov_b64 %0, s[94:95]\n\ts_mov_b32 s94, 0xb02b6262\n\ts_mov_b32 s95, 0xbe5ae600\n\tv_fma_f64 %6, %0, %13, s[94:95]\n\tv_fma_f64 %5, %0, %12, s[94:95]\n\tv_fma_f64 %4, %0, %11, s[94:95]\n\tv_fma_f64 %3, %0, %10, s[94:95]\n\tv_fma_f64 %2, %0, %9, s[94:95]\n\tv_fma_f64 %1, %0, %8, s[94:95]\n\tv_fma_f64 %0, %0, %7, s[94:95]\n\ts_mov_b32 s94, 0x7968a100\n\ts_mov_b32 s95, 0x3ec71de3\n\tv_fma_f64 %0, %0, %7, s[94:95]\n\tv_fma_f64 %1, %1, %8, s[94:95]\n\tv_fma_f64 %2, %2, %9, s[94:95]\n\tv_fma_f64 %3, %3, %10, s[94:95]\n\tv_fma_f64 %4, %4, %11, s[94:95]\n\tv_fma_f64 %5, %5, %12, s[94:95]\n\tv_fma_f64 %6, %6, %13, s[94:95]\n\ts_mov_b32 s94, 0x19e83aae\n\ts_mov_b32 s95, 0xbf2a01a0\n\tv_fma_f64 %0, %0, %7, s[94:95]\n\tv_fma_f64 %1, %1, %8, s[94:95]\n\tv_fma_f64 %2, %2, %9, s[94:95]\n\tv_fma_f64 %3, %3, %10, s[94:95]\n\tv_fma_f64 %4, %4, %11, s[94:95]\n\tv_fma_f64 %5, %5, %12, s[94:95]\n\tv_fma_f64 %6, %6, %13, s[94:95]\n\ts_mov_b32 s94, 0x11110bb2\n\ts_mov_b32 s95, 0x3f811111\n\tv_fma_f64 %0, %0, %7, s[94:95]\n\tv_fma_f64 %1, %1, %8, s[94:95]\n\tv_fma_f64 %2, %2, %9, s[94:95]\n\tv_fma_f64 %3, %3, %10, s[94:95]\n\tv_fma_f64 %4, %4, %11, s[94:95]\n\tv_fma_f64 %5, %5, %12, s[94:95]\n\tv_fma_f64 %6, %6, %13, s[94:95]\n\ts_mov_b32 s94, 0x55555555\n\ts_mov_b32 s95, 0xbfc55555\n\tv_fma_f64 %0, %0, %7, s[94:95]\n\tv_fma_f64 %1, %1, %8, s[94:95]\n\tv_fma_f64 %2, %2, %9, s[94:95]\n\tv_fma_f64 %3, %3, %10, s[94:95]\n\tv_fma_f64 %4, %4, %11, s[94:95]\n\tv_fma_f64 %5, %5, %12, s[94:95]\n\tv_fma_f64 %6, %6, %13, s[94:95]"
        : "=&v"(q[0]), "=&v"(q[1]), "=&v"(q[2]), "=&v"(q[3]), "=&v"(q[4]), "=&v"(q[5]), "=&v"(q[6])
        : "v"(s[0]), "v"(s[1]), "v"(s[2]), "v"(s[3]), "v"(s[4]), "v"(s[5]), "v"(s[6])
        : "s94", "s95");
}
template <> __device__ __forceinline__ void horner_cos_c<1>(double (&q)[1], const double (&s)[1]) {
    asm("s_mov_b32 s94, 0x367a37cb\n\ts_mov_b32 s95, 0xbda907da\n\tv_mov_b64 %0, s[94:95]\n\ts_mov_b32 s94, 0x8e93b64c\n\ts_mov_b32 s95, 0x3e21eeb6\n\tv_fma_f64 %0, %0, %1, s[94:95]\n\ts_mov_b32 s94, 0xa17da09e\n\ts_mov_b32 s95, 0xbe927e4f\n\tv_fma_f64 %0, %0, %1, s[94:95]\n\ts_mov_b32 s94, 0x19f4eb01\n\ts_mov_b32 s95, 0x3efa01a0\n\tv_fma_f64 %0, %0, %1, s[94:95]\n\ts_mov_b32 s94, 0x16c16967\n\ts_mov_b32 s95, 0xbf56c16c\n\tv_fma_f64 %0, %0, %1, s[94:95]\n\ts_mov_b32 s94, 0x55555555\n\ts_mov_b32 s95, 0x3fa55555\n\tv_fma_f64 %0, %0, %1, s[94:95]"
        : "=&v"(q[0])
        : "v"(s[0])
        : "s94", "s95");
}
template <> __device__ __forceinline__ void horner_cos_c<2>(double (&q)[2], const double (&s)[2]) {
    asm("s_mov_b32 s94, 0x367a37cb\n\ts_mov_b32 s95, 0xbda907da\n\tv_mov_b64 %0, s[94:95]\n\ts_mov_b32 s94, 0x8e93b64c\n\ts_mov_b32 s95, 0x3e21eeb6\n\tv_fma_f64 %1, %0, %3, s[94:95]\n\tv_fma_f64 %0, %0, %2, s[94:95]\n\ts_mov_b32 s94, 0xa17da09e\n\ts_mov_b32 s95, 0xbe927e4f\n\tv_fma_f64 %0, %0, %2, s[94:95]\n\tv_fma_f64 %1, %1, %3, s[94:95]\n\ts_mov_b32 s94, 0x19f4eb01\n\ts_mov_b32 s95, 0x3efa01a0\n\tv_fma_f64 %0, %0, %2, s[94:95]\n\tv_fma_f64 %1, %1, %3, s[94:95]\n\ts_mov_b32 s94, 0x16c16967\n\ts_mov_b32 s95, 0xbf56c16c\n\tv_fma_f64 %0, %0, %2, s[94:95]\n\tv_fma_f64 %1, %1, %3, s[94:95]\n\ts_mov_b32 s94, 0x55555555\n\ts_mov_b32 s95, 0x3fa55555\n\tv_fma_f64 %0, %0, %2, s[94:95]\n\tv_fma_f64 %1, %1, %3, s[94:95]"
        : "=&v"(q[0]), "=&v"(q[1])
        : "v"(s[0]), "v"(s[1])
        : "s94", "s95");
}
template <> __device__ __forceinline__ void horner_cos_c<3>(double (&q)[3], const double (&s)[3]) {
    asm("s_mov_b32 s94, 0x367a37cb\n\ts_mov_b32 s95, 0xbda907da\n\tv_mov_b64 %0, s[94:95]\n\ts_mov_b32 s94, 0x8e93b64c\n\ts_mov_b32 s95, 0x3e21eeb6\n\tv_fma_f64 %2, %0, %5, s[94:95]\n\tv_fma_f64 %1, %0, %4, s[94:95]\n\tv_fma_f64 %0, %0, %3, s[94:95]\n\ts_mov_b32 s94, 0xa17da09e\n\ts_mov_b32 s95, 0xbe927e4f\n\tv_fma_f64 %0, %0, %3, s[94:95]\n\tv_fma_f64 %1, %1, %4, s[94:95]\n\tv_fma_f64 %2, %2, %5, s[94:95]\n\ts_mov_b32 s94, 0x19f4eb01\n\ts_mov_b32 s95, 0x3efa01a0\n\tv_fma_f64 %0, %0, %3, s[94:95]\n\tv_fma_f64 %1, %1, %4, s[94:95]\n\tv_fma_f64 %2, %2, %5, s[94:95]\n\ts_mov_b32 s94, 0x16c16967\n\ts_mov_b32 s95, 0xbf56c16c\n\tv_fma_f64 %0, %0, %3, s[94:95]\n\tv_fma_f64 %1, %1, %4, s[94:95]\n\tv_fma_f64 %2, %2, %5, s[94:95]\n\ts_mov_b32 s94, 0x55555555\n\ts_mov_b32 s95, 0x3fa55555\n\tv_fma_f64 %0, %0, %3, s[94:95]\n\tv_fma_f64 %1, %1, %4, s[94:95]\n\tv_fma_f64 %2, %2, %5, s[94:95]"
        : "=&v"(q[0]), "=&v"(q[1]), "=&v"(q[2])
        : "v"(s[0]), "v"(s[1]), "v"(s[2])
        : "s94", "s95");
}
template <> __device__ __forceinline__ void horner_cos_c<4>(double (&q)[4], const double (&s)[4]) {
    asm("s_mov_b32 s94, 0x367a37cb\n\ts_mov_b32 s95, 0xbda907da\n\tv_mov_b64 %0, s[94:95]\n\ts_mov_b32 s94, 0x8e93b64c\n\ts_mov_b32 s95, 0x3e21eeb6\n\tv_fma_f64 %3, %0, %7, s[94:95]\n\tv_fma_f64 %2, %0, %6, s[94:95]\n\tv_fma_f64 %1, %0, %5, s[94:95]\n\tv_fma_f64 %0, %0, %4, s[94:95]\n\ts_mov_b32 s94, 0xa17da09e\n\ts_mov_b32 s95, 0xbe927e4f\n\tv_fma_f64 %0, %0, %4, s[94:95]\n\tv_fma_f64 %1, %1, %5, s[94:95]\n\tv_fma_f64 %2, %2, %6, s[94:95]\n\tv_fma_f64 %3, %3, %7, s[94:95]\n\ts_mov_b32 s94, 0x19f4eb01\n\ts_mov_b32 s95, 0x3efa01a0\n\tv_fma_f64 %0, %0, %4, s[94:95]\n\tv_fma_f64 %1, %1, %5, s[94:95]\n\tv_fma_f64 %2, %2, %6, s[94:95]\n\tv_fma_f64 %3, %3, %7, s[94:95]\n\ts_mov_b32 s94, 0x16c16967\n\ts_mov_b32 s95, 0xbf56c16c\n\tv_fma_f64 %0, %0, %4, s[94:95]\n\tv_fma_f64 %1, %1, %5, s[94:95]\n\tv_fma_f64 %2, %2, %6, s[94:95]\n\tv_fma_f64 %3, %3, %7, s[94:95]\n\ts_mov_b32 s94, 0x55555555\n\ts_mov_b32 s95, 0x3fa55555\n\tv_fma_f64 %0, %0, %4, s[94:95]\n\tv_fma_f64 %1, %1, %5, s[94:95]\n\tv_fma_f64 %2, %2, %6, s[94:95]\n\tv_fma_f64 %3, %3, %7, s[94:95]"
        : "=&v"(q[0]), "=&v"(q[1]), "=&v"(q[2]), "=&v"(q[3])
        : "v"(s[0]), "v"(s[1]), "v"(s[2]), "v"(s[3])
        : "s94", "s95");
}
template <> __device__ __forceinline__ void horner_cos_c<7>(double (&q)[7], const double (&s)[7]) {
    asm("s_mov_b32 s94, 0x367a37cb\n\ts_mov_b32 s95, 0xbda907da\n\tv_mov_b64 %0, s[94:95]\n\ts_mov_b32 s94, 0x8e93b64c\n\ts_mov_b32 s95, 0x3e21eeb6\n\tv_fma_f64 %6, %0, %13, s[94:95]\n\tv_fma_f64 %5, %0, %12, s[94:95]\n\tv_fma_f64 %4, %0, %11, s[94:95]\n\tv_fma_f64 %3, %0, %10, s[94:95]\n\tv_fma_f64 %2, %0, %9, s[94:95]\n\tv_fma_f64 %1, %0, %8, s[94:95]\n\tv_fma_f64 %0, %0, %7, s[94:95]\n\ts_mov_b32 s94, 0xa17da09e\n\ts_mov_b32 s95, 0xbe927e4f\n\tv_fma_f64 %0, %0, %7, s[94:95]\n\tv_fma_f64 %1, %1, %8, s[94:95]\n\tv_fma_f64 %2, %2, %9, s[94:95]\n\tv_fma_f64 %3, %3, %10, s[94:95]\n\tv_fma_f64 %4, %4, %11, s[94:95]\n\tv_fma_f64 %5, %5, %12, s[94:95]\n\tv_fma_f64 %6, %6, %13, s[94:95]\n\ts_mov_b32 s94, 0x19f4eb01\n\ts_mov_b32 s95, 0x3efa01a0\n\tv_fma_f64 %0, %0, %7, s[94:95]\n\tv_fma_f64 %1, %1, %8, s[94:95]\n\tv_fma_f64 %2, %2, %9, s[94:95]\n\tv_fma_f64 %3, %3, %10, s[94:95]\n\tv_fma_f64 %4, %4, %11, s[94:95]\n\tv_fma_f64 %5, %5, %12, s[94:95]\n\tv_fma_f64 %6, %6, %13, s[94:95]\n\ts_mov_b32 s94, 0x16c16967\n\ts_mov_b32 s95, 0xbf56c16c\n\tv_fma_f64 %0, %0, %7, s[94:95]\n\tv_fma_f64 %1, %1, %8, s[94:95]\n\tv_fma_f64 %2, %2, %9, s[94:95]\n\tv_fma_f64 %3, %3, %10, s[94:95]\n\tv_fma_f64 %4, %4, %11, s[94:95]\n\tv_fma_f64 %5, %5, %12, s[94:95]\n\tv_fma_f64 %6, %6, %13, s[94:95]\n\ts_mov_b32 s94, 0x55555555\n\ts_mov_b32 s95, 0x3fa55555\n\tv_fma_f64 %0, %0, %7, s[94:95]\n\tv_fma_f64 %1, %1, %8, s[94:95]\n\tv_fma_f64 %2, %2, %9, s[94:95]\n\tv_fma_f64 %3, %3, %10, s[94:95]\n\tv_fma_f64 %4, %4, %11, s[94:95]\n\tv_fma_f64 %5, %5, %12, s[94:95]\n\tv_fma_f64 %6, %6, %13, s[94:95]"
        : "=&v"(q[0]), "=&v"(q[1]), "=&v"(q[2]), "=&v"(q[3]), "=&v"(q[4]), "=&v"(q[5]), "=&v"(q[6])
        : "v"(s[0]), "v"(s[1]), "v"(s[2]), "v"(s[3]), "v"(s[4]), "v"(s[5]), "v"(s[6])
        : "s94", "s95");
}
constexpr int kUnitAtanSteps = 24;
constexpr int kUnitAtanHalf = 18;
constexpr int kUnitAtanRows = 4 * kUnitAtanHalf;
__constant__ double c_unit_atan_tab[3][kUnitAtanRows] = {
    {1.0, -1.0, 0.9991315673568165, -0.9991315673568165, 0.9965217285917831, -0.9965217285917831, 0.9921567416492215, -0.9921567416492215, 0.9860132971832694, -0.9860132971832694, 0.9780578828587919, -0.9780578828587919, 0.9682458365518543, -0.9682458365518543, 0.9565200236040831, -0.9565200236040831, 0.9428090415820634, -0.9428090415820634, 0.9270248108869579, -0.9270248108869579, 0.9090593428863095, -0.9090593428863095, 0.8887803753208976, -0.8887803753208976, 0.8660254037844386, -0.8660254037844386, 0.8405933750763339, -0.8405933750763339, 0.8122328620674136, -0.8122328620674136, 0.7806247497997998, -0.7806247497997998, 0.7453559924999299, -0.7453559924999299, 0.705878097754059, -0.705878097754059, -1.0, 1.0, -0.9991315673568165, 0.9991315673568165, -0.9965217285917831, 0.9965217285917831, -0.9921567416492215, 0.9921567416492215, -0.9860132971832694, 0.9860132971832694, -0.9780578828587919, 0.9780578828587919, -0.9682458365518543, 0.9682458365518543, -0.9565200236040831, 0.9565200236040831, -0.9428090415820634, 0.9428090415820634, -0.9270248108869579, 0.9270248108869579, -0.9090593428863095, 0.9090593428863095, -0.8887803753208976, 0.8887803753208976, -0.8660254037844386, 0.8660254037844386, -0.8405933750763339, 0.8405933750763339, -0.8122328620674136, 0.8122328620674136, -0.7806247497997998, 0.7806247497997998, -0.7453559924999299, 0.7453559924999299, -0.705878097754059, 0.705878097754059},
    {0.0, 0.0, 0.041666666666666664, -0.041666666666666664, 0.08333333333333333, -0.08333333333333333, 0.125, -0.125, 0.16666666666666666, -0.16666666666666666, 0.20833333333333334, -0.20833333333333334, 0.25, -0.25, 0.2916666666666667, -0.2916666666666667, 0.3333333333333333, -0.3333333333333333, 0.375, -0.375, 0.4166666666666667, -0.4166666666666667, 0.4583333333333333, -0.4583333333333333, 0.5, -0.5, 0.5416666666666666, -0.5416666666666666, 0.5833333333333334, -0.5833333333333334, 0.625, -0.625, 0.6666666666666666, -0.6666666666666666, 0.7083333333333334, -0.7083333333333334, 0.0, 0.0, -0.041666666666666664, 0.041666666666666664, -0.08333333333333333, 0.08333333333333333, -0.125, 0.125, -0.16666666666666666, 0.16666666666666666, -0.20833333333333334, 0.20833333333333334, -0.25, 0.25, -0.2916666666666667, 0.2916666666666667, -0.3333333333333333, 0.3333333333333333, -0.375, 0.375, -0.4166666666666667, 0.4166666666666667, -0.4583333333333333, 0.4583333333333333, -0.5, 0.5, -0.5416666666666666, 0.5416666666666666, -0.5833333333333334, 0.5833333333333334, -0.625, 0.625, -0.6666666666666666, 0.6666666666666666, -0.7083333333333334, 0.7083333333333334},
    {0.0, 1.5707963267948966, 0.041678732422577865, 1.5291175943723188, 0.083430086610615, 1.4873662401842815, 0.1253278311680654, 1.4454684956268313, 0.16744807921968932, 1.4033482475752073, 0.20987059226273777, 1.3609257345321588, 0.25268025514207865, 1.318116071652818, 0.2959688033589313, 1.2748275234359654, 0.3398369094541219, 1.2309594173407747, 0.3843967744956391, 1.1863995522992576, 0.42977543130452767, 1.141020895490369, 0.47611906091179634, 1.0946772658831003, 0.5235987755982989, 1.0471975511965979, 0.5724185720928202, 0.9983777547020763, 0.622826585412003, 0.9479697413828937, 0.6751315329370317, 0.895664793857865, 0.7297276562269663, 0.8410686705679302, 0.7871342779970989, 0.7836620487977977, 3.141592653589793, 1.5707963267948966, 3.0999139211672153, 1.6124750592174746, 3.058162566979178, 1.6542264134055116, 3.0162648224217277, 1.696124157962962, 2.974144574370104, 1.7382444060145859, 2.9317220613270556, 1.7806669190576343, 2.8889123984477147, 1.8234765819369754, 2.845623850230862, 1.866765130153828, 2.8017557441356713, 1.9106332362490186, 2.757195879094154, 1.9551931012905357, 2.7118172222852657, 2.0005717580994244, 2.665473592677997, 2.046915387706693, 2.6179938779914944, 2.0943951023931957, 2.569174081496973, 2.1432148988877167, 2.5187660681777904, 2.1936229122068998, 2.466461120652762, 2.2459278597319283, 2.411864997362827, 2.300523983021863, 2.3544583755926944, 2.3579306047919957},
};
template <int N> __device__ __forceinline__ void horner_asin_p(double (&q)[N], const double (&s)[N]);
template <> __device__ __forceinline__ void horner_asin_p<1>(double (&q)[1], const double (&s)[1]) {
    asm("s_mov_b32 s94, 0xb6db6db7\n\ts_mov_b32 s95, 0x3fa6db6d\n\tv_mov_b64 %0, s[94:95]\n\ts_mov_b32 s94, 0x33333333\n\ts_mov_b32 s95, 0x3fb33333\n\tv_fma_f64 %0, %0, %1, s[94:95]\n\ts_mov_b32 s94, 0x55555555\n\ts_mov_b32 s95, 0x3fc55555\n\tv_fma_f64 %0, %0, %1, s[94:95]"
        : "=&v"(q[0])
        : "v"(s[0])
        : "s94", "s95");
}
template <> __device__ __forceinline__ void horner_asin_p<2>(double (&q)[2], const double (&s)[2]) {
    asm("s_mov_b32 s94, 0xb6db6db7\n\ts_mov_b32 s95, 0x3fa6db6d\n\tv_mov_b64 %0, s[94:95]\n\ts_mov_b32 s94, 0x33333333\n\ts_mov_b32 s95, 0x3fb33333\n\tv_fma_f64 %1, %0, %3, s[94:95]\n\tv_fma_f64 %0, %0, %2, s[94:95]\n\ts_mov_b32 s94, 0x55555555\n\ts_mov_b32 s95, 0x3fc55555\n\tv_fma_f64 %0, %0, %2, s[94:95]\n\tv_fma_f64 %1, %1, %3, s[94:95]"
        : "=&v"(q[0]), "=&v"(q[1])
        : "v"(s[0]), "v"(s[1])
        : "s94", "s95");
}
template <> __device__ __forceinline__ void horner_asin_p<3>(double (&q)[3], const double (&s)[3]) {
    asm("s_mov_b32 s94, 0xb6db6db7\n\ts_mov_b32 s95, 0x3fa6db6d\n\tv_mov_b64 %0, s[94:95]\n\ts_mov_b32 s94, 0x33333333\n\ts_mov_b32 s95, 0x3fb33333\n\tv_fma_f64 %2, %0, %5, s[94:95]\n\tv_fma_f64 %1, %0, %4, s[94:95]\n\tv_fma_f64 %0, %0, %3, s[94:95]\n\ts_mov_b32 s94, 0x55555555\n\ts_mov_b32 s95, 0x3fc55555\n\tv_fma_f64 %0, %0, %3, s[94:95]\n\tv_fma_f64 %1, %1, %4, s[94:95]\n\tv_fma_f64 %2, %2, %5, s[94:95]"
        : "=&v"(q[0]), "=&v"(q[1]), "=&v"(q[2])
        : "v"(s[0]), "v"(s[1]), "v"(s[2])
        : "s94", "s95");
}
template <> __device__ __forceinline__ void horner_asin_p<4>(double (&q)[4], const double (&s)[4]) {
    asm("s_mov_b32 s94, 0xb6db6db7\n\ts_mov_b32 s95, 0x3fa6db6d\n\tv_mov_b64 %0, s[94:95]\n\ts_mov_b32 s94, 0x33333333\n\ts_mov_b32 s95, 0x3fb33333\n\tv_fma_f64 %3, %0, %7, s[94:95]\n\tv_fma_f64 %2, %0, %6, s[94:95]\n\tv_fma_f64 %1, %0, %5, s[94:95]\n\tv_fma_f64 %0, %0, %4, s[94:95]\n\ts_mov_b32 s94, 0x55555555\n\ts_mov_b32 s95, 0x3fc55555\n\tv_fma_f64 %0, %0, %4, s[94:95]\n\tv_fma_f64 %1, %1, %5, s[94:95]\n\tv_fma_f64 %2, %2, %6, s[94:95]\n\tv_fma_f64 %3, %3, %7, s[94:95]"
        : "=&v"(q[0]), "=&v"(q[1]), "=&v"(q[2]), "=&v"(q[3])
        : "v"(s[0]), "v"(s[1]), "v"(s[2]), "v"(s[3])
        : "s94", "s95");
}
template <> __device__ __forceinline__ void horner_asin_p<7>(double (&q)[7], const double (&s)[7]) {
    asm("s_mov_b32 s94, 0xb6db6db7\n\ts_mov_b32 s95, 0x3fa6db6d\n\tv_mov_b64 %0, s[94:95]\n\ts_mov_b32 s94, 0x33333333\n\ts_mov_b32 s95, 0x3fb33333\n\tv_fma_f64 %6, %0, %13, s[94:95]\n\tv_fma_f64 %5, %0, %12, s[94:95]\n\tv_fma_f64 %4, %0, %11, s[94:95]\n\tv_fma_f64 %3, %0, %10, s[94:95]\n\tv_fma_f64 %2, %0, %9, s[94:95]\n\tv_fma_f64 %1, %0, %8, s[94:95]\n\tv_fma_f64 %0, %0, %7, s[94:95]\n\ts_mov_b32 s94, 0x55555555\n\ts_mov_b32 s95, 0x3fc55555\n\tv_fma_f64 %0, %0, %7, s[94:95]\n\tv_fma_f64 %1, %1, %8, s[94:95]\n\tv_fma_f64 %2, %2, %9, s[94:95]\n\tv_fma_f64 %3, %3, %10, s[94:95]\n\tv_fma_f64 %4, %4, %11, s[94:95]\n\tv_fma_f64 %5, %5, %12, s[94:95]\n\tv_fma_f64 %6, %6, %13, s[94:95]"
        : "=&v"(q[0]), "=&v"(q[1]), "=&v"(q[2]), "=&v"(q[3]), "=&v"(q[4]), "=&v"(q[5]), "=&v"(q[6])
        : "v"(s[0]), "v"(s[1]), "v"(s[2]), "v"(s[3]), "v"(s[4]), "v"(s[5]), "v"(s[6])
        : "s94", "s95");
}
constexpr int kSinCosRows = 64;
__constant__ double c_sincos_tab[2][kSinCosRows] = {
    {1.0, 0.9951847266721969, 0.9807852804032304, 0.9569403357322088, 0.9238795325112867, 0.881921264348355, 0.8314696123025452, 0.773010453362737, 0.7071067811865476, 0.6343932841636455, 0.5555702330196022, 0.47139673682599764, 0.3826834323650898, 0.2902846772544624, 0.19509032201612828, 0.0980171403295606, 0.0, -0.0980171403295606, -0.19509032201612828, -0.2902846772544624, -0.3826834323650898, -0.47139673682599764, -0.5555702330196022, -0.6343932841636455, -0.7071067811865476, -0.773010453362737, -0.8314696123025452, -0.881921264348355, -0.9238795325112867, -0.9569403357322088, -0.9807852804032304, -0.9951847266721969, -1.0, -0.9951847266721969, -0.9807852804032304, -0.9569403357322088, -0.9238795325112867, -0.881921264348355, -0.8314696123025452, -0.773010453362737, -0.7071067811865476, -0.6343932841636455, -0.5555702330196022, -0.47139673682599764, -0.3826834323650898, -0.2902846772544624, -0.19509032201612828, -0.0980171403295606, 0.0, 0.0980171403295606, 0.19509032201612828, 0.2902846772544624, 0.3826834323650898, 0.47139673682599764, 0.5555702330196022, 0.6343932841636455, 0.7071067811865476, 0.773010453362737, 0.8314696123025452, 0.881921264348355, 0.9238795325112867, 0.9569403357322088, 0.9807852804032304, 0.9951847266721969},
    {0.0, 0.0980171403295606, 0.19509032201612828, 0.2902846772544624, 0.3826834323650898, 0.47139673682599764, 0.5555702330196022, 0.6343932841636455, 0.7071067811865476, 0.773010453362737, 0.8314696123025452, 0.881921264348355, 0.9238795325112867, 0.9569403357322088, 0.9807852804032304, 0.9951847266721969, 1.0, 0.9951847266721969, 0.9807852804032304, 0.9569403357322088, 0.9238795325112867, 0.881921264348355, 0.8314696123025452, 0.773010453362737, 0.7071067811865476, 0.6343932841636455, 0.5555702330196022, 0.47139673682599764, 0.3826834323650898, 0.2902846772544624, 0.19509032201612828, 0.0980171403295606, 0.0, -0.0980171403295606, -0.19509032201612828, -0.2902846772544624, -0.3826834323650898, -0.47139673682599764, -0.5555702330196022, -0.6343932841636455, -0.7071067811865476, -0.773010453362737, -0.8314696123025452, -0.881921264348355, -0.9238795325112867, -0.9569403357322088, -0.9807852804032304, -0.9951847266721969, -1.0, -0.9951847266721969, -0.9807852804032304, -0.9569403357322088, -0.9238795325112867, -0.881921264348355, -0.8314696123025452, -0.773010453362737, -0.7071067811865476, -0.6343932841636455, -0.5555702330196022, -0.47139673682599764, -0.3826834323650898, -0.2902846772544624, -0.19509032201612828, -0.0980171403295606},
};
template <int N> __device__ __forceinline__ void horner_sin3(double (&q)[N], const double (&s)[N]);
template <int N> __device__ __forceinline__ void horner_cos4(double (&q)[N], const double (&s)[N]);
template <> __device__ __forceinline__ void horner_sin3<1>(double (&q)[1], const double (&s)[1]) {
    asm("s_mov_b32 s94, 0x1a01a01a\n\ts_mov_b32 s95, 0xbf2a01a0\n\tv_mov_b64 %0, s[94:95]\n\ts_mov_b32 s94, 0x11111111\n\ts_mov_b32 s95, 0x3f811111\n\tv_fma_f64 %0, %0, %1, s[94:95]\n\ts_mov_b32 s94, 0x55555555\n\ts_mov_b32 s95, 0xbfc55555\n\tv_fma_f64 %0, %0, %1, s[94:95]"
        : "=&v"(q[0])
        : "v"(s[0])
        : "s94", "s95");
}
template <> __device__ __forceinline__ void horner_sin3<2>(double (&q)[2], const double (&s)[2]) {
    asm("s_mov_b32 s94, 0x1a01a01a\n\ts_mov_b32 s95, 0xbf2a01a0\n\tv_mov_b64 %0, s[94:95]\n\ts_mov_b32 s94, 0x11111111\n\ts_mov_b32 s95, 0x3f811111\n\tv_fma_f64 %1, %0, %3, s[94:95]\n\tv_fma_f64 %0, %0, %2, s[94:95]\n\ts_mov_b32 s94, 0x55555555\n\ts_mov_b32 s95, 0xbfc55555\n\tv_fma_f64 %0, %0, %2, s[94:95]\n\tv_fma_f64 %1, %1, %3, s[94:95]"
        : "=&v"(q[0]), "=&v"(q[1])
        : "v"(s[0]), "v"(s[1])
        : "s94", "s95");
}
template <> __device__ __forceinline__ void horner_sin3<3>(double (&q)[3], const double (&s)[3]) {
    asm("s_mov_b32 s94, 0x1a01a01a\n\ts_mov_b32 s95, 0xbf2a01a0\n\tv_mov_b64 %0, s[94:95]\n\ts_mov_b32 s94, 0x11111111\n\ts_mov_b32 s95, 0x3f811111\n\tv_fma_f64 %2, %0, %5, s[94:95]\n\tv_fma_f64 %1, %0, %4, s[94:95]\n\tv_fma_f64 %0, %0, %3, s[94:95]\n\ts_mov_b32 s94, 0x55555555\n\ts_mov_b32 s95, 0xbfc55555\n\tv_fma_f64 %0, %0, %3, s[94:95]\n\tv_fma_f64 %1, %1, %4, s[94:95]\n\tv_fma_f64 %2, %2, %5, s[94:95]"
        : "=&v"(q[0]), "=&v"(q[1]), "=&v"(q[2])
        : "v"(s[0]), "v"(s[1]), "v"(s[2])
        : "s94", "s95");
}
template <> __device__ __forceinline__ void horner_sin3<4>(double (&q)[4], const double (&s)[4]) {
    asm("s_mov_b32 s94, 0x1a01a01a\n\ts_mov_b32 s95, 0xbf2a01a0\n\tv_mov_b64 %0, s[94:95]\n\ts_mov_b32 s94, 0x11111111\n\ts_mov_b32 s95, 0x3f811111\n\tv_fma_f64 %3, %0, %7, s[94:95]\n\tv_fma_f64 %2, %0, %6, s[94:95]\n\tv_fma_f64 %1, %0, %5, s[94:95]\n\tv_fma_f64 %0, %0, %4, s[94:95]\n\ts_mov_b32 s94, 0x55555555\n\ts_mov_b32 s95, 0xbfc55555\n\tv_fma_f64 %0, %0, %4, s[94:95]\n\tv_fma_f64 %1, %1, %5, s[94:95]\n\tv_fma_f64 %2, %2, %6, s[94:95]\n\tv_fma_f64 %3, %3, %7, s[94:95]"
        : "=&v"(q[0]), "=&v"(q[1]), "=&v"(q[2]), "=&v"(q[3])
        : "v"(s[0]), "v"(s[1]), "v"(s[2]), "v"(s[3])
        : "s94", "s95");
}
template <> __device__ __forceinline__ void horner_cos4<1>(double (&q)[1], const double (&s)[1]) {
    asm("s_mov_b32 s94, 0x1a01a01a\n\ts_mov_b32 s95, 0x3efa01a0\n\tv_mov_b64 %0, s[94:95]\n\ts_mov_b32 s94, 0x16c16c17\n\ts_mov_b32 s95, 0xbf56c16c\n\tv_fma_f64 %0, %0, %1, s[94:95]\n\ts_mov_b32 s94, 0x55555555\n\ts_mov_b32 s95, 0x3fa55555\n\tv_fma_f64 %0, %0, %1, s[94:95]\n\ts_mov_b32 s94, 0x00000000\n\ts_mov_b32 s95, 0xbfe00000\n\tv_fma_f64 %0, %0, %1, s[94:95]"
        : "=&v"(q[0])
        : "v"(s[0])
        : "s94", "s95");
}
template <> __device__ __forceinline__ void horner_cos4<2>(double (&q)[2], const double (&s)[2]) {
    asm("s_mov_b32 s94, 0x1a01a01a\n\ts_mov_b32 s95, 0x3efa01a0\n\tv_mov_b64 %0, s[94:95]\n\ts_mov_b32 s94, 0x16c16c17\n\ts_mov_b32 s95, 0xbf56c16c\n\tv_fma_f64 %1, %0, %3, s[94:95]\n\tv_fma_f64 %0, %0, %2, s[94:95]\n\ts_mov_b32 s94, 0x55555555\n\ts_mov_b32 s95, 0x3fa55555\n\tv_fma_f64 %0, %0, %2, s[94:95]\n\tv_fma_f64 %1, %1, %3, s[94:95]\n\ts_mov_b32 s94, 0x00000000\n\ts_mov_b32 s95, 0xbfe00000\n\tv_fma_f64 %0, %0, %2, s[94:95]\n\tv_fma_f64 %1, %1, %3, s[94:95]"
        : "=&v"(q[0]), "=&v"(q[1])
        : "v"(s[0]), "v"(s[1])
        : "s94", "s95");
}
template <> __device__ __forceinline__ void horner_cos4<3>(double (&q)[3], const double (&s)[3]) {
    asm("s_mov_b32 s94, 0x1a01a01a\n\ts_mov_b32 s95, 0x3efa01a0\n\tv_mov_b64 %0, s[94:95]\n\ts_mov_b32 s94, 0x16c16c17\n\ts_mov_b32 s95, 0xbf56c16c\n\tv_fma_f64 %2, %0, %5, s[94:95]\n\tv_fma_f64 %1, %0, %4, s[94:95]\n\tv_fma_f64 %0, %0, %3, s[94:95]\n\ts_mov_b32 s94, 0x55555555\n\ts_mov_b32 s95, 0x3fa55555\n\tv_fma_f64 %0, %0, %3, s[94:95]\n\tv_fma_f64 %1, %1, %4, s[94:95]\n\tv_fma_f64 %2, %2, %5, s[94:95]\n\ts_mov_b32 s94, 0x00000000\n\ts_mov_b32 s95, 0xbfe00000\n\tv_fma_f64 %0, %0, %3, s[94:95]\n\tv_fma_f64 %1, %1, %4, s[94:95]\n\tv_fma_f64 %2, %2, %5, s[94:95]"
        : "=&v"(q[0]), "=&v"(q[1]), "=&v"(q[2])
        : "v"(s[0]), "v"(s[1]), "v"(s[2])
        : "s94", "s95");
}
template <> __device__ __forceinline__ void horner_cos4<4>(double (&q)[4], const double (&s)[4]) {
    asm("s_mov_b32 s94, 0x1a01a01a\n\ts_mov_b32 s95, 0x3efa01a0\n\tv_mov_b64 %0, s[94:95]\n\ts_mov_b32 s94, 0x16c16c17\n\ts_mov_b32 s95, 0xbf56c16c\n\tv_fma_f64 %3, %0, %7, s[94:95]\n\tv_fma_f64 %2, %0, %6, s[94:95]\n\tv_fma_f64 %1, %0, %5, s[94:95]\n\tv_fma_f64 %0, %0, %4, s[94:95]\n\ts_mov_b32 s94, 0x55555555\n\ts_mov_b32 s95, 0x3fa55555\n\tv_fma_f64 %0, %0, %4, s[94:95]\n\tv_fma_f64 %1, %1, %5, s[94:95]\n\tv_fma_f64 %2, %2, %6, s[94:95]\n\tv_fma_f64 %3, %3, %7, s[94:95]\n\ts_mov_b32 s94, 0x00000000\n\ts_mov_b32 s95, 0xbfe00000\n\tv_fma_f64 %0, %0, %4, s[94:95]\n\tv_fma_f64 %1, %1, %5, s[94:95]\n\tv_fma_f64 %2, %2, %6, s[94:95]\n\tv_fma_f64 %3, %3, %7, s[94:95]"
        : "=&v"(q[0]), "=&v"(q[1]), "=&v"(q[2]), "=&v"(q[3])
        : "v"(s[0]), "v"(s[1]), "v"(s[2]), "v"(s[3])
        : "s94", "s95");
}
```

Measured before the change: 35.14 billion.

## Unify LDS lookup tables into one interleaved shared buffer with faster index math

Replaces the per-kernel SharedTables struct and separate sincos table with a single global LDS buffer, placing the table columns at offsets chosen so two columns fall within reach of one two-address LDS read. The unit-atan table's phi column is reordered so the row index and cosine sign can be formed with one alignbit, and the table indices are computed with a magic-constant FMA instead of a float-to-int conversion. Sincos reduction gets similar inline-asm helpers, and branch hints on per-lane rare paths become configurable. The intent is fewer ALU and LDS instructions per table lookup, at the cost of hand-tuned offsets and more inline asm.

```diff
diff --git a/reachy2_symbolic_ik_amd/csrc/rsik_device.hpp b/reachy2_symbolic_ik_amd/csrc/rsik_device.hpp
--- a/reachy2_symbolic_ik_amd/csrc/rsik_device.hpp
+++ b/reachy2_symbolic_ik_amd/csrc/rsik_device.hpp
@@ -13,7 +13,14 @@
 #else
 #define RSIK_RARE(c) (__builtin_expect(!!(c), 0))
 #endif
-
+#ifndef RSIK_WAVE_COMMON_HINT
+#define RSIK_WAVE_COMMON_HINT 1
+#endif
+#if defined(RSIK_HOT_ONLY) || RSIK_WAVE_COMMON_HINT
+#define RSIK_RARE_LANE(c) RSIK_RARE(c)
+#else
+#define RSIK_RARE_LANE(c) (c)
+#endif
 
 #ifdef RSIK_ISA_MARKS
 #define RSIK_MARK(name) asm volatile("; RSIK_MARK " name)
@@ -300,7 +307,7 @@
 
     RSIK_MARK("reach_wrist");
     V3 w = wrist_position(woff, gp);
-    if (RSIK_RARE(w.x < bl)) {
+    if (RSIK_RARE_LANE(w.x < bl)) {
         double diff = bl - w.x;
         gp.x = gp.x + diff;
         if (NO_LIMITS) w = wrist_position(woff, gp);
@@ -327,7 +334,7 @@
             return r;
         }
     }
-    if (RSIK_RARE(dsw < A(RSIK_C_MIN_DIST))) {
+    if (RSIK_RARE_LANE(dsw < A(RSIK_C_MIN_DIST))) {
         const double t = fabs(dsw) + pm;
         const double k = A(RSIK_C_MIN_DIST) * fast_rcp(t);
         const double km1 = k - 1.0;
@@ -564,7 +571,7 @@
     JointsOut o;
     V3 e = elbow_on_circle(r, ct, st);
     o.projected = false;
-    if (RSIK_RARE(above_singularity_plane<!FRESH>(A, e))) {
+    if (RSIK_RARE_LANE(above_singularity_plane<!FRESH>(A, e))) {
         const V3 v3 = cvec(A, RSIK_C_PLANE_N), pc = cvec(A, RSIK_C_PROJ_CENTER);
         const V3 d1 = e - pc;
         const V3 V = madd(v3, -dot(d1, v3), d1);
diff --git a/reachy2_symbolic_ik_amd/csrc/rsik_kernel_continuous.hpp b/reachy2_symbolic_ik_amd/csrc/rsik_kernel_continuous.hpp
--- a/reachy2_symbolic_ik_amd/csrc/rsik_kernel_continuous.hpp
+++ b/reachy2_symbolic_ik_amd/csrc/rsik_kernel_continuous.hpp
@@ -97,7 +97,7 @@
     const int64_t ii = live ? i : (K.n - 1);
     const int64_t n = K.n;
 
-    __shared__ SharedTables lds_tab;
+    SharedTables lds_tab;
         stage_tables<MIXED, (int)offsetof(ContinuousArgs, arms) + (MIXED ? 0 : (int)sizeof(ArmC))>(lds_tab, K.arms);
     const Acc<MIXED> A = make_acc<MIXED>(K.arms, MIXED ? (K.arm[ii] != 0) : false, lds_tab);
     const int slot = MIXED ? (A.isl ? 1 : 0) : 0;
@@ -199,7 +199,7 @@
     const int half = PAIR ? (int)(gid & 1) : 0;
     const bool live = i < K.n;
     const int64_t ii = live ? i : (K.n - 1);
-    __shared__ SharedTables lds_tab;
+    SharedTables lds_tab;
         stage_tables<MIXED, (int)offsetof(ContinuousArgs, arms) + (MIXED ? 0 : (int)sizeof(ArmC))>(lds_tab, K.arms);
     const Acc<MIXED> A = make_acc<MIXED>(K.arms, MIXED ? (K.arm[ii] != 0) : false, lds_tab);
     const int slot = MIXED ? (A.isl ? 1 : 0) : 0;
diff --git a/reachy2_symbolic_ik_amd/csrc/rsik_kernel_discrete.hpp b/reachy2_symbolic_ik_amd/csrc/rsik_kernel_discrete.hpp
--- a/reachy2_symbolic_ik_amd/csrc/rsik_kernel_discrete.hpp
+++ b/reachy2_symbolic_ik_amd/csrc/rsik_kernel_discrete.hpp
@@ -140,7 +140,7 @@
 #pragma unroll
         for (int k = 0; k < 7; k++) prow.v[k] = K.prev_rows[ii * 7 + k];
     }
-        __shared__ SharedTables lds_tab;
+        SharedTables lds_tab;
     stage_tables<MIXED, (int)offsetof(DiscreteArgs, arms) + (MIXED ? 0 : (int)sizeof(ArmC)), kDiscBlock>(lds_tab, K.arms);
 #ifdef RSIK_TIMELINE_PROBE
     asm volatile("s_waitcnt vmcnt(0)" ::: "memory");
diff --git a/reachy2_symbolic_ik_amd/csrc/rsik_kernel_nearest.hpp b/reachy2_symbolic_ik_amd/csrc/rsik_kernel_nearest.hpp
--- a/reachy2_symbolic_ik_amd/csrc/rsik_kernel_nearest.hpp
+++ b/reachy2_symbolic_ik_amd/csrc/rsik_kernel_nearest.hpp
@@ -71,7 +71,7 @@
     static_assert(L == 1 || L == 8 || L == 64, "lanes per pose");
     constexpr int PW = 64 / L;
     constexpr int PB = kBlock / L;
-    __shared__ SharedTables lds_tab;
+    SharedTables lds_tab;
     __shared__ double lds[kBlock / 64][64 * 10];
     const int lane = threadIdx.x & 63;
     const int wave = __builtin_amdgcn_readfirstlane(threadIdx.x >> 6);
diff --git a/reachy2_symbolic_ik_amd/csrc/rsik_kernel_pipeline.hpp b/reachy2_symbolic_ik_amd/csrc/rsik_kernel_pipeline.hpp
--- a/reachy2_symbolic_ik_amd/csrc/rsik_kernel_pipeline.hpp
+++ b/reachy2_symbolic_ik_amd/csrc/rsik_kernel_pipeline.hpp
@@ -124,7 +124,7 @@
 #pragma unroll
     for (int k = 0; k < 12; k++) m[k] = src[k * K.n];
     const bool lane_isl = MIXED ? (K.arm[ii] != 0) : false;
-    __shared__ SharedTables lds_tab;
+    SharedTables lds_tab;
         stage_tables<MIXED, (int)offsetof(ContRunArgs, arms) + (MIXED ? 0 : (int)sizeof(ArmC))>(lds_tab, K.arms);
     const Acc<MIXED> A = make_acc<MIXED>(K.arms, lane_isl, lds_tab);
     const int slot = MIXED ? (A.isl ? 1 : 0) : 0;
@@ -409,7 +409,7 @@
 __global__ __launch_bounds__(kBlock) RSIK_PHASED_OCC_ATTR void cont_joints_kernel(const ContRunArgs K) {
     RSIK_PIPE_STAMP(K, 2);
     __shared__ double lds_out[kBlock / 64][64 * 7];
-    __shared__ SharedTables lds_tab;
+    SharedTables lds_tab;
     const int wave = threadIdx.x >> 6;
     cont_joints_chunk<MIXED>(K, lds_tab, lds_out[wave], (int64_t)blockIdx.x * (kBlock / 64) + wave, (int64_t)blockIdx.y);
 }
@@ -625,7 +625,7 @@
         __hip_atomic_store(K.chain_started_word, K.started_seq, __ATOMIC_RELAXED, __HIP_MEMORY_SCOPE_SYSTEM);
     __builtin_amdgcn_s_setprio(2);
     const int64_t gid = (int64_t)blockIdx.x * kChainBlock + threadIdx.x;
-    __shared__ SharedTables lds_tab;
+    SharedTables lds_tab;
         stage_tables<MIXED, (int)offsetof(ContRunArgs, arms) + (MIXED ? 0 : (int)sizeof(ArmC)), kChainBlock>(lds_tab, K.arms);
     cont_chain_walk<MIXED, kChainBatch>(K, lds_tab, gid >> 3, (int)(gid & 7), 0, K.t0, K.T, K.last_block != 0);
 }
diff --git a/reachy2_symbolic_ik_amd/csrc/rsik_kernel_solve.hpp b/reachy2_symbolic_ik_amd/csrc/rsik_kernel_solve.hpp
--- a/reachy2_symbolic_ik_amd/csrc/rsik_kernel_solve.hpp
+++ b/reachy2_symbolic_ik_amd/csrc/rsik_kernel_solve.hpp
@@ -53,9 +53,10 @@
         else return k[i];
     }
 };
+static_assert(2 * RSIK_ARM_CONSTS_COUNT * 8 <= kLdsArmBytes, "the two per-arm blocks do not fit between the tables' columns");
 struct SharedTables {
-    double arm[2][RSIK_ARM_CONSTS_COUNT];
-    double utab[3][kUnitAtanRows];
+    __device__ __forceinline__ double* arm(int slot) const { return &g_lds_tab[kLdsArm / 8 + slot * RSIK_ARM_CONSTS_COUNT]; }
+    __device__ __forceinline__ UnitAtanTab utab() const { return (UnitAtanTab)&g_lds_tab[0]; }
 };
 #ifndef RSIK_WARM_KERNARG
 #define RSIK_WARM_KERNARG 1
@@ -93,16 +94,14 @@
             vc[r] = ((r + 1) * NB <= NC || k < NC) ? arms[k / RSIK_ARM_CONSTS_COUNT].v[k % RSIK_ARM_CONSTS_COUNT] : 0.0;
         }
     }
-    double* la = &S.utab[0][0];
-    double* ls = &g_sincos_tab[0][0];
 #pragma unroll
     for (int r = 0; r < RA; r++)
-        if ((r + 1) * NB <= NA || t + r * NB < NA) la[t + r * NB] = va[r];
+        if ((r + 1) * NB <= NA || t + r * NB < NA) g_lds_tab[lds_slot_unit_atan(t + r * NB)] = va[r];
 #pragma unroll
     for (int r = 0; r < RS; r++)
-        if ((r + 1) * NB <= NS || t + r * NB < NS) ls[t + r * NB] = vs[r];
+        if ((r + 1) * NB <= NS || t + r * NB < NS) g_lds_tab[lds_slot_sincos(t + r * NB)] = vs[r];
     if constexpr (MIXED) {
-        double* lc = &S.arm[0][0];
+        double* lc = S.arm(0);
 #pragma unroll
         for (int r = 0; r < RC; r++)
             if ((r + 1) * NB <= NC || t + r * NB < NC) lc[t + r * NB] = vc[r];
@@ -111,7 +110,7 @@
 }
 template <bool MIXED>
 __device__ __forceinline__ Acc<MIXED> make_acc(const ArmC* arms, bool isl, SharedTables& S) {
-    Acc<MIXED> A{arms, isl, (LdsConst)S.arm[isl ? 1 : 0], (UnitAtanTab)&S.utab[0][0]};
+    Acc<MIXED> A{arms, isl, (LdsConst)S.arm(isl ? 1 : 0), S.utab()};
     return A;
 }
 
@@ -214,7 +213,7 @@
 __device__ __forceinline__ ACC kernarg_acc(SharedTables& S, int slot) {
     ACC A;
     A.k = (KConst)&((const __attribute__((address_space(4))) ARGS*)__builtin_amdgcn_kernarg_segment_ptr())->arms[0].v[0];
-    A.lds = (LdsConst)S.arm[slot]; A.utab = (UnitAtanTab)&S.utab[0][0];
+    A.lds = (LdsConst)S.arm(slot); A.utab = S.utab();
     return A;
 }
 __device__ __forceinline__ void reach_invalid_input(Reach& r) {
@@ -233,7 +232,7 @@
 
 template <int MIXED, bool TIPZ, bool PREV_ROWS = false>
 __global__ __launch_bounds__(kBlock, RSIK_SOLVE_MIN_WAVES) void solve_kernel(const SolveArgs K) {
-    __shared__ SharedTables lds_tab;
+    SharedTables lds_tab;
     __shared__ double lds[kBlock / 64][64 * 10];
     const int lane = threadIdx.x & 63;
     const int wave = __builtin_amdgcn_readfirstlane(threadIdx.x >> 6);
diff --git a/reachy2_symbolic_ik_amd/csrc/rsik_kernel_stages.hpp b/reachy2_symbolic_ik_amd/csrc/rsik_kernel_stages.hpp
--- a/reachy2_symbolic_ik_amd/csrc/rsik_kernel_stages.hpp
+++ b/reachy2_symbolic_ik_amd/csrc/rsik_kernel_stages.hpp
@@ -174,7 +174,7 @@
 
 __global__ __launch_bounds__(kBlock) void stage_kernel(const StageArgs K) {
     const int64_t i = (int64_t)blockIdx.x * kBlock + threadIdx.x;
-    __shared__ SharedTables lds_tab;
+    SharedTables lds_tab;
         stage_tables<false, (int)offsetof(StageArgs, arms) + (int)sizeof(ArmC)>(lds_tab, K.arms);
     if (i >= K.n) return;
     const Acc<false> A = make_acc<false>(K.arms, false, lds_tab);
diff --git a/reachy2_symbolic_ik_amd/csrc/rsik_kernel_state.hpp b/reachy2_symbolic_ik_amd/csrc/rsik_kernel_state.hpp
--- a/reachy2_symbolic_ik_amd/csrc/rsik_kernel_state.hpp
+++ b/reachy2_symbolic_ik_amd/csrc/rsik_kernel_state.hpp
@@ -21,7 +21,7 @@
 template <bool MIXED>
 __global__ __launch_bounds__(kBlock) void reach_state_kernel(const StateArgs K) {
     const int64_t i = (int64_t)blockIdx.x * kBlock + threadIdx.x;
-    __shared__ SharedTables lds_tab;
+    SharedTables lds_tab;
     stage_tables<MIXED, (int)offsetof(StateArgs, arms) + (MIXED ? 0 : (int)sizeof(ArmC))>(lds_tab, K.arms);
     if (i >= K.n) return;
     const Acc<MIXED> A = make_acc<MIXED>(K.arms, MIXED ? (K.arm[i] != 0) : false, lds_tab);
@@ -63,7 +63,7 @@
 template <bool MIXED>
 __global__ __launch_bounds__(kBlock) void joints_state_kernel(const StateArgs K) {
     const int64_t i = (int64_t)blockIdx.x * kBlock + threadIdx.x;
-    __shared__ SharedTables lds_tab;
+    SharedTables lds_tab;
     stage_tables<MIXED, (int)offsetof(StateArgs, arms) + (MIXED ? 0 : (int)sizeof(ArmC))>(lds_tab, K.arms);
     if (i >= K.n) return;
     const Acc<MIXED> A = make_acc<MIXED>(K.arms, MIXED ? (K.arm[i] != 0) : false, lds_tab);
@@ -91,7 +91,7 @@
 
 __global__ __launch_bounds__(kBlock) void elbow_state_kernel(const StateArgs K) {
     const int64_t i = (int64_t)blockIdx.x * kBlock + threadIdx.x;
-    stage_sincos_tab();
+    stage_lds_tabs();
     __syncthreads();
     if (i >= K.n) return;
     const double* S = K.solver_state + i * RSIK_SOLVER_STATE_STRIDE;
@@ -117,7 +117,7 @@
 template <bool MIXED>
 __global__ __launch_bounds__(kBlock) void fk_kernel(const FkArgs K) {
     const int64_t i = (int64_t)blockIdx.x * kBlock + threadIdx.x;
-    __shared__ SharedTables lds_tab;
+    SharedTables lds_tab;
     stage_tables<MIXED>(lds_tab, K.arms);
     if (i >= K.n) return;
     const Acc<MIXED> A = make_acc<MIXED>(K.arms, MIXED ? (K.arm[i] != 0) : false, lds_tab);
@@ -152,9 +152,7 @@
 
 __global__ void debug_math_kernel(int op, int64_t n, const double* a, const double* b, double* o0, double* o1) {
     const int64_t i = (int64_t)blockIdx.x * blockDim.x + threadIdx.x;
-    __shared__ double utab[3][kUnitAtanRows];
-    stage_sincos_tab();
-    stage_unit_atan_tab(utab);
+    stage_lds_tabs();
     __syncthreads();
     if (i >= n) return;
     double x = a[i], r0 = 0.0, r1 = 0.0;
@@ -162,7 +160,7 @@
         case 7: {
             const double ss[1] = {x}, cc[1] = {b[i]};
             double o[1];
-            unit_atan2_n<1>((UnitAtanTab)&utab[0][0], ss, cc, o);
+            unit_atan2_n<1>((UnitAtanTab)&g_lds_tab[0], ss, cc, o);
             r0 = o[0];
             break;
         }
diff --git a/reachy2_symbolic_ik_amd/csrc/rsik_kernel_sweep.hpp b/reachy2_symbolic_ik_amd/csrc/rsik_kernel_sweep.hpp
--- a/reachy2_symbolic_ik_amd/csrc/rsik_kernel_sweep.hpp
+++ b/reachy2_symbolic_ik_amd/csrc/rsik_kernel_sweep.hpp
@@ -32,7 +32,7 @@
 #endif
 template <int MIXED, bool TIPZ, bool PREV_ROWS>
 __global__ __launch_bounds__(kBlock, RSIK_SWEEP_MIN_WAVES) void solve_sweep_kernel(const SweepArgs K) {
-    __shared__ SharedTables lds_tab;
+    SharedTables lds_tab;
     __shared__ double lds[kBlock / 64][64 * 10];
     const int lane = threadIdx.x & 63;
     const int wave = __builtin_amdgcn_readfirstlane(threadIdx.x >> 6);
diff --git a/reachy2_symbolic_ik_amd/csrc/rsik_kernel_theta_from_joints.hpp b/reachy2_symbolic_ik_amd/csrc/rsik_kernel_theta_from_joints.hpp
--- a/reachy2_symbolic_ik_amd/csrc/rsik_kernel_theta_from_joints.hpp
+++ b/reachy2_symbolic_ik_amd/csrc/rsik_kernel_theta_from_joints.hpp
@@ -79,7 +79,7 @@
     const bool live = i < K.n;
     const int64_t ii = live ? i : (K.n - 1);
 
-    __shared__ SharedTables lds_tab;
+    SharedTables lds_tab;
     stage_tables<(MIXED != 0), (MIXED == 1 ? 0 : (int)offsetof(ThetaFromJointsArgs, arms) + (int)sizeof(ArmC))>(lds_tab, K.arms);
     const int slot = (MIXED != 0 && K.arm[ii] != 0) ? 1 : 0;
     const AccK<MIXED> A = kernarg_acc<AccK<MIXED>, ThetaFromJointsArgs>(lds_tab, slot);
@@ -127,7 +127,7 @@
 template <bool MIXED>
 __global__ __launch_bounds__(kBlock) void theta_from_joints_state_kernel(const ThetaFromJointsArgs K) {
     const int64_t i = (int64_t)blockIdx.x * kBlock + threadIdx.x;
-    __shared__ SharedTables lds_tab;
+    SharedTables lds_tab;
     stage_tables<MIXED, (int)offsetof(ThetaFromJointsArgs, arms) + (MIXED ? 0 : (int)sizeof(ArmC))>(lds_tab, K.arms);
     if (i >= K.n) return;
     const Acc<MIXED> A = make_acc<MIXED>(K.arms, MIXED ? (K.arm[i] != 0) : false, lds_tab);
diff --git a/reachy2_symbolic_ik_amd/csrc/rsik_math.hpp b/reachy2_symbolic_ik_amd/csrc/rsik_math.hpp
--- a/reachy2_symbolic_ik_amd/csrc/rsik_math.hpp
+++ b/reachy2_symbolic_ik_amd/csrc/rsik_math.hpp
@@ -80,25 +80,40 @@
     return o[0];
 }
 
+__shared__ __attribute__((aligned(16))) double g_lds_tab[kLdsTabBytes / 8];
+static_assert(kLdsAtanSin - kLdsAtanCos > 2040 && kLdsAtanPhi - kLdsAtanSin > 2040 && (kLdsAtanSin - kLdsAtanCos) % 512 != 0 &&
+              (kLdsAtanPhi - kLdsAtanSin) % 512 != 0 && (kLdsAtanPhi - kLdsAtanCos) % 512 != 0 && kLdsSinCosSin - kLdsSinCosCos > 2040 &&
+              (kLdsSinCosSin - kLdsSinCosCos) % 512 != 0, "two columns of one table within reach of a two-address LDS read");
+__device__ __forceinline__ constexpr int lds_slot_unit_atan(int k) {
+    return k < kUnitAtanRows ? kLdsAtanCos / 8 + k : k < 2 * kUnitAtanRows ? kLdsAtanSin / 8 + (k - kUnitAtanRows) : kLdsAtanPhi / 8 + (k - 2 * kUnitAtanRows);
+}
+__device__ __forceinline__ constexpr int lds_slot_sincos(int k) {
+    return k < kSinCosRows ? kLdsSinCosCos / 8 + k : kLdsSinCosSin / 8 + (k - kSinCosRows);
+}
+__device__ __forceinline__ void stage_lds_tabs() {
+    for (int k = threadIdx.x; k < kUnitAtanRows * 3; k += blockDim.x) g_lds_tab[lds_slot_unit_atan(k)] = (&c_unit_atan_tab[0][0])[k];
+    for (int k = threadIdx.x; k < kSinCosRows * 2; k += blockDim.x) g_lds_tab[lds_slot_sincos(k)] = (&c_sincos_tab[0][0])[k];
+}
+
 typedef const __attribute__((address_space(3))) double* UnitAtanTab;
-__device__ __forceinline__ void stage_unit_atan_tab(double (*lds_tab)[kUnitAtanRows]) {
-    for (int k = threadIdx.x; k < kUnitAtanRows * 3; k += blockDim.x) (&lds_tab[0][0])[k] = (&c_unit_atan_tab[0][0])[k];
-}
+static_assert(kUnitAtanIdxBytes == 2 * kUnitAtanCnegBytes, "unit_atan2_n forms 2 i + [c < 0] in one instruction");
 template <int N>
 __device__ __forceinline__ void unit_atan2_n(UnitAtanTab T, const double (&s)[N], const double (&c)[N], double (&out)[N]) {
     double x[N], x2[N], p[N], phi[N];
+    const double scale = unit_atan_scale();
 #pragma unroll
     for (int i = 0; i < N; i++) {
         const double ac = fabs(c[i]), as = fabs(s[i]);
         const double mx = fmax(ac, as), mn = fmin(ac, as);
-        const unsigned idx = (unsigned)(int)fma(mn, (double)kUnitAtanSteps, 0.5);
-        const unsigned cneg = (unsigned)(__builtin_bit_cast(unsigned long long, c[i]) >> 63);
+        const unsigned idx = (unsigned)__builtin_bit_cast(unsigned long long, unit_atan_index(mn, scale));
+        const unsigned chi = (unsigned)(__builtin_bit_cast(unsigned long long, c[i]) >> 32);
+        const unsigned row2 = __builtin_amdgcn_alignbit(idx, chi, 31);
         typedef const __attribute__((address_space(3))) char* LdsBytes;
         const unsigned tb = (unsigned)(size_t)(LdsBytes)T;
-        const unsigned addr = ((idx + (unsigned)kUnitAtanHalf * cneg) << 4) + (as > ac ? tb + 8u : tb);
+        const unsigned addr = row2 * (unsigned)kUnitAtanCnegBytes + (as > ac ? tb + (unsigned)kUnitAtanSwapBytes : tb);
         const LdsBytes Tb = (LdsBytes)(size_t)addr;
-        const double ci = *(UnitAtanTab)Tb, si = *(UnitAtanTab)(Tb + kUnitAtanRows * 8);
-        phi[i] = *(UnitAtanTab)(Tb + 2 * kUnitAtanRows * 8);
+        const double ci = *(UnitAtanTab)(Tb + kLdsAtanCos), si = *(UnitAtanTab)(Tb + kLdsAtanSin);
+        phi[i] = *(UnitAtanTab)(Tb + kLdsAtanPhi);
         x[i] = fma(mn, ci, -(mx * si));
         x2[i] = x[i] * x[i];
     }
@@ -110,20 +125,16 @@
     }
 }
 
-__shared__ __attribute__((aligned(512))) double g_sincos_tab[2][kSinCosRows];
-__device__ __forceinline__ void stage_sincos_tab() {
-    for (int k = threadIdx.x; k < kSinCosRows * 2; k += blockDim.x) (&g_sincos_tab[0][0])[k] = (&c_sincos_tab[0][0])[k];
-}
 template <int N>
 __device__ __forceinline__ void fast_sincos_n(const double (&x)[N], double (&sn)[N], double (&cs)[N]) {
     double r[N], z[N], ps[N], pc[N], ck[N], sk[N];
+    const double scale = sincos_scale();
 #pragma unroll
     for (int i = 0; i < N; i++) {
-        const double k = __builtin_rint(x[i] * 10.185916357881302);
-        const double t = fma(-k, 0.09817477042088285, x[i]);
-        r[i] = fma(-k, 3.79818781656637e-12, t);
-        const int idx = (int)k & (kSinCosRows - 1);
-        ck[i] = g_sincos_tab[0][idx]; sk[i] = g_sincos_tab[1][idx];
+        const double t = sincos_index(x[i], scale);
+        const unsigned idx = (unsigned)__builtin_bit_cast(unsigned long long, t) & (unsigned)(kSinCosRows - 1);
+        r[i] = sincos_reduce(x[i], t);
+        ck[i] = g_lds_tab[kLdsSinCosCos / 8 + idx]; sk[i] = g_lds_tab[kLdsSinCosSin / 8 + idx];
         z[i] = r[i] * r[i];
     }
     horner_sin3<N>(ps, z);
@@ -131,9 +142,9 @@
 #pragma unroll
     for (int i = 0; i < N; i++) {
         const double sr = fma(r[i] * z[i], ps[i], r[i]);
-        const double cm1 = z[i] * pc[i];
-        sn[i] = sk[i] + fma(sk[i], cm1, ck[i] * sr);
-        cs[i] = ck[i] + fma(ck[i], cm1, -(sk[i] * sr));
+        const double cr = fma(z[i], pc[i], 1.0);
+        sn[i] = fma(sk[i], cr, ck[i] * sr);
+        cs[i] = fma(ck[i], cr, -(sk[i] * sr));
     }
 }
 __device__ __forceinline__ void fast_sincos(double x, double* sn, double* cs) {
diff --git a/reachy2_symbolic_ik_amd/csrc/rsik_poly_gen.hpp b/reachy2_symbolic_ik_amd/csrc/rsik_poly_gen.hpp
--- a/reachy2_symbolic_ik_amd/csrc/rsik_poly_gen.hpp
+++ b/reachy2_symbolic_ik_amd/csrc/rsik_poly_gen.hpp
@@ -91,13 +91,22 @@
         : "v"(s[0]), "v"(s[1]), "v"(s[2]), "v"(s[3]), "v"(s[4]), "v"(s[5]), "v"(s[6])
         : "s94", "s95");
 }
+constexpr int kLdsAtanCos = 0;
+constexpr int kLdsSinCosCos = 576;
+constexpr int kLdsArm = 1088;
+constexpr int kLdsAtanSin = 2056;
+constexpr int kLdsSinCosSin = 2632;
+constexpr int kLdsAtanPhi = 4112;
+constexpr int kLdsTabBytes = 4688;
+constexpr int kLdsArmBytes = 968;
+constexpr int kUnitAtanIdxBytes = 16, kUnitAtanCnegBytes = 8, kUnitAtanSwapBytes = 288;
 constexpr int kUnitAtanSteps = 24;
 constexpr int kUnitAtanHalf = 18;
 constexpr int kUnitAtanRows = 4 * kUnitAtanHalf;
 __constant__ double c_unit_atan_tab[3][kUnitAtanRows] = {
     {1.0, -1.0, 0.9991315673568165, -0.9991315673568165, 0.9965217285917831, -0.9965217285917831, 0.9921567416492215, -0.9921567416492215, 0.9860132971832694, -0.9860132971832694, 0.9780578828587919, -0.9780578828587919, 0.9682458365518543, -0.9682458365518543, 0.9565200236040831, -0.9565200236040831, 0.9428090415820634, -0.9428090415820634, 0.9270248108869579, -0.9270248108869579, 0.9090593428863095, -0.9090593428863095, 0.8887803753208976, -0.8887803753208976, 0.8660254037844386, -0.8660254037844386, 0.8405933750763339, -0.8405933750763339, 0.8122328620674136, -0.8122328620674136, 0.7806247497997998, -0.7806247497997998, 0.7453559924999299, -0.7453559924999299, 0.705878097754059, -0.705878097754059, -1.0, 1.0, -0.9991315673568165, 0.9991315673568165, -0.9965217285917831, 0.9965217285917831, -0.9921567416492215, 0.9921567416492215, -0.9860132971832694, 0.9860132971832694, -0.9780578828587919, 0.9780578828587919, -0.9682458365518543, 0.9682458365518543, -0.9565200236040831, 0.9565200236040831, -0.9428090415820634, 0.9428090415820634, -0.9270248108869579, 0.9270248108869579, -0.9090593428863095, 0.9090593428863095, -0.8887803753208976, 0.8887803753208976, -0.8660254037844386, 0.8660254037844386, -0.8405933750763339, 0.8405933750763339, -0.8122328620674136, 0.8122328620674136, -0.7806247497997998, 0.7806247497997998, -0.7453559924999299, 0.7453559924999299, -0.705878097754059, 0.705878097754059},
     {0.0, 0.0, 0.041666666666666664, -0.041666666666666664, 0.08333333333333333, -0.08333333333333333, 0.125, -0.125, 0.16666666666666666, -0.16666666666666666, 0.20833333333333334, -0.20833333333333334, 0.25, -0.25, 0.2916666666666667, -0.2916666666666667, 0.3333333333333333, -0.3333333333333333, 0.375, -0.375, 0.4166666666666667, -0.4166666666666667, 0.4583333333333333, -0.4583333333333333, 0.5, -0.5, 0.5416666666666666, -0.5416666666666666, 0.5833333333333334, -0.5833333333333334, 0.625, -0.625, 0.6666666666666666, -0.6666666666666666, 0.7083333333333334, -0.7083333333333334, 0.0, 0.0, -0.041666666666666664, 0.041666666666666664, -0.08333333333333333, 0.08333333333333333, -0.125, 0.125, -0.16666666666666666, 0.16666666666666666, -0.20833333333333334, 0.20833333333333334, -0.25, 0.25, -0.2916666666666667, 0.2916666666666667, -0.3333333333333333, 0.3333333333333333, -0.375, 0.375, -0.4166666666666667, 0.4166666666666667, -0.4583333333333333, 0.4583333333333333, -0.5, 0.5, -0.5416666666666666, 0.5416666666666666, -0.5833333333333334, 0.5833333333333334, -0.625, 0.625, -0.6666666666666666, 0.6666666666666666, -0.7083333333333334, 0.7083333333333334},
-    {0.0, 1.5707963267948966, 0.041678732422577865, 1.5291175943723188, 0.083430086610615, 1.4873662401842815, 0.1253278311680654, 1.4454684956268313, 0.16744807921968932, 1.4033482475752073, 0.20987059226273777, 1.3609257345321588, 0.25268025514207865, 1.318116071652818, 0.2959688033589313, 1.2748275234359654, 0.3398369094541219, 1.2309594173407747, 0.3843967744956391, 1.1863995522992576, 0.42977543130452767, 1.141020895490369, 0.47611906091179634, 1.0946772658831003, 0.5235987755982989, 1.0471975511965979, 0.5724185720928202, 0.9983777547020763, 0.622826585412003, 0.9479697413828937, 0.6751315329370317, 0.895664793857865, 0.7297276562269663, 0.8410686705679302, 0.7871342779970989, 0.7836620487977977, 3.141592653589793, 1.5707963267948966, 3.0999139211672153, 1.6124750592174746, 3.058162566979178, 1.6542264134055116, 3.0162648224217277, 1.696124157962962, 2.974144574370104, 1.7382444060145859, 2.9317220613270556, 1.7806669190576343, 2.8889123984477147, 1.8234765819369754, 2.845623850230862, 1.866765130153828, 2.8017557441356713, 1.9106332362490186, 2.757195879094154, 1.9551931012905357, 2.7118172222852657, 2.0005717580994244, 2.665473592677997, 2.046915387706693, 2.6179938779914944, 2.0943951023931957, 2.569174081496973, 2.1432148988877167, 2.5187660681777904, 2.1936229122068998, 2.466461120652762, 2.2459278597319283, 2.411864997362827, 2.300523983021863, 2.3544583755926944, 2.3579306047919957},
+    {0.0, 3.141592653589793, 0.041678732422577865, 3.0999139211672153, 0.083430086610615, 3.058162566979178, 0.1253278311680654, 3.0162648224217277, 0.16744807921968932, 2.974144574370104, 0.20987059226273777, 2.9317220613270556, 0.25268025514207865, 2.8889123984477147, 0.2959688033589313, 2.845623850230862, 0.3398369094541219, 2.8017557441356713, 0.3843967744956391, 2.757195879094154, 0.42977543130452767, 2.7118172222852657, 0.47611906091179634, 2.665473592677997, 0.5235987755982989, 2.6179938779914944, 0.5724185720928202, 2.569174081496973, 0.622826585412003, 2.5187660681777904, 0.6751315329370317, 2.466461120652762, 0.7297276562269663, 2.411864997362827, 0.7871342779970989, 2.3544583755926944, 1.5707963267948966, 1.5707963267948966, 1.5291175943723188, 1.6124750592174746, 1.4873662401842815, 1.6542264134055116, 1.4454684956268313, 1.696124157962962, 1.4033482475752073, 1.7382444060145859, 1.3609257345321588, 1.7806669190576343, 1.318116071652818, 1.8234765819369754, 1.2748275234359654, 1.866765130153828, 1.2309594173407747, 1.9106332362490186, 1.1863995522992576, 1.9551931012905357, 1.141020895490369, 2.0005717580994244, 1.0946772658831003, 2.046915387706693, 1.0471975511965979, 2.0943951023931957, 0.9983777547020763, 2.1432148988877167, 0.9479697413828937, 2.1936229122068998, 0.895664793857865, 2.2459278597319283, 0.8410686705679302, 2.300523983021863, 0.7836620487977977, 2.3579306047919957},
 };
 template <int N> __device__ __forceinline__ void horner_asin_p(double (&q)[N], const double (&s)[N]);
 template <> __device__ __forceinline__ void horner_asin_p<1>(double (&q)[1], const double (&s)[1]) {
@@ -129,6 +138,16 @@
         : "=&v"(q[0]), "=&v"(q[1]), "=&v"(q[2]), "=&v"(q[3]), "=&v"(q[4]), "=&v"(q[5]), "=&v"(q[6])
         : "v"(s[0]), "v"(s[1]), "v"(s[2]), "v"(s[3]), "v"(s[4]), "v"(s[5]), "v"(s[6])
         : "s94", "s95");
+}
+__device__ __forceinline__ double unit_atan_scale() {
+    double v;
+    asm("s_mov_b32 s94, 0x00000000\n\ts_mov_b32 s95, 0x40380000\n\tv_mov_b64 %0, s[94:95]" : "=v"(v) : : "s94", "s95");
+    return v;
+}
+__device__ __forceinline__ double unit_atan_index(double x, double scale) {
+    double t;
+    asm("s_mov_b32 s94, 0x00000000\n\ts_mov_b32 s95, 0x43380000\n\tv_fma_f64 %0, %1, %2, s[94:95]" : "=v"(t) : "v"(x), "v"(scale) : "s94", "s95");
+    return t;
 }
 constexpr int kSinCosRows = 64;
 __constant__ double c_sincos_tab[2][kSinCosRows] = {
@@ -185,3 +204,22 @@
         : "v"(s[0]), "v"(s[1]), "v"(s[2]), "v"(s[3])
         : "s94", "s95");
 }
+__device__ __forceinline__ double sincos_scale() {
+    double v;
+    asm("s_mov_b32 s94, 0x6dc9c883\n\ts_mov_b32 s95, 0x40245f30\n\tv_mov_b64 %0, s[94:95]" : "=v"(v) : : "s94", "s95");
+    return v;
+}
+__device__ __forceinline__ double sincos_index(double x, double scale) {
+    double t;
+    asm("s_mov_b32 s94, 0x00000000\n\ts_mov_b32 s95, 0x43380000\n\tv_fma_f64 %0, %1, %2, s[94:95]" : "=v"(t) : "v"(x), "v"(scale) : "s94", "s95");
+    return t;
+}
+__device__ __forceinline__ double sincos_reduce(double x, double t) {
+    double k, r;
+    asm("s_mov_b32 s94, 0x00000000\n\ts_mov_b32 s95, 0x43380000\n\tv_add_f64 %0, %1, -s[94:95]" : "=v"(k) : "v"(t) : "s94", "s95");
+    asm("s_mov_b32 s94, 0x54400000\n\ts_mov_b32 s95, 0xbfb921fb\n\tv_fma_f64 %0, %1, s[94:95], %2\n\ts_mov_b32 s94, 0x1a626331\n\ts_mov_b32 s95, 0xbd90b461\n\tv_fma_f64 %0, %1, s[94:95], %0"
+        : "=&v"(r)
+        : "v"(k), "v"(x)
+        : "s94", "s95");
+    return r;
+}
```

Measured after the change: 34.87 billion. No clear change (-0.8%).
